# tangent-T/FACL

Measured on AMD Instinct MI355X. Metric: contrastive-step clips/sec (B=32,T=24,N=2048) at 1/2/4/8 MI355X, higher is better.
Workload: dtype f32

## Files before the change

### facl_amd/_lib.py

```python
import ctypes
import os

import torch

_HERE = os.path.dirname(os.path.abspath(__file__))
_LIB = None

c_p = ctypes.c_void_p
c_i = ctypes.c_int
c_f = ctypes.c_float
c_d = ctypes.c_double
c_l = ctypes.c_longlong

SIGNATURES = {
    "facl_version": [],
    "facl_fps_f32": [c_p, c_i, c_i, c_i, c_i, c_p, c_p, c_p],
    "facl_fps_f64": [c_p, c_i, c_i, c_i, c_i, c_p, c_p, c_p],
    "facl_fps_reorder": [c_p, c_i, c_i, c_i, c_p, c_i, c_p, c_p],
    "facl_group": [c_p, c_i, c_i, c_i, c_i, c_i, c_f, c_p, c_p, c_p, c_p],
    "facl_group_clips": [c_p, c_i, c_i, c_i, c_i, c_i, c_i, c_f, c_p, c_p, c_p, c_p],
    "facl_gather_rows": [c_p, c_i, c_i, c_i, c_i, c_p, c_i, c_p, c_p, c_i, c_i, c_p],
    "facl_scatter_rows": [c_p, c_i, c_i, c_i, c_i, c_i, c_p, c_i, c_p, c_p],
    "facl_sinkhorn": [c_p, c_i, c_i, c_i, c_p, c_p, c_p],
    "facl_kmeans": [c_p, c_i, c_i, c_i, c_i, c_p, c_p, c_p, c_p],
    "facl_adam_prep": [c_p, c_p, c_f, c_f, c_p, c_p],
    "facl_adam_apply": [c_i, c_p, c_p, c_p, c_p, c_p, c_p, c_f, c_f, c_f, c_p],
    "facl_ws_bytes": [],
    "facl_bn_finalize": [c_p, c_i, c_d, c_p, c_p, c_f, c_f, c_p, c_p, c_p, c_p, c_p, c_p],
    "facl_bn_finalize_after": [c_p, c_i, c_d, c_p, c_p, c_f, c_f, c_p, c_p, c_p, c_p, c_p, c_p, c_i, c_p],
    "facl_bn_eval_consts_after": [c_i, c_p, c_p, c_p, c_p, c_f, c_p, c_p, c_i, c_p],
    "facl_absmax": [c_p, c_l, c_p, c_p],
    "facl_rows_act_amax": [c_p, c_l, c_i, c_p, c_p, c_p, c_p],
    "facl_bn_eval_consts": [c_i, c_p, c_p, c_p, c_p, c_f, c_p, c_p],
    "facl_sa_x_moments": [c_p, c_l, c_i, c_p, c_p, c_p],
    "facl_bn1_sums_from_moments": [c_p, c_d, c_i, c_p, c_p, c_p, c_p],
    "facl_sa_bn1_chain": [c_p, c_d, c_i, c_p, c_p, c_p, c_p, c_f, c_f, c_p, c_p, c_p, c_p, c_p, c_p, c_p],
    "facl_sa_l1tab": [c_p, c_p, c_i, c_p, c_p, c_p, c_p, c_p, c_p],
    "facl_sa_fwd2": [c_p, c_l, c_i, c_p, c_p, c_p, c_p, c_p, c_p, c_p, c_p],
    "facl_sa_fwd3": [c_p, c_l, c_p, c_p, c_p, c_p, c_p, c_p, c_p, c_p, c_p, c_p],
    "facl_sa_fwd3_h3": [c_p, c_l, c_p, c_p, c_p, c_p, c_p, c_p, c_p, c_p, c_p, c_p, c_p],
    "facl_sa_fwd3_f16": [c_p, c_l, c_p, c_p, c_p, c_p, c_p, c_p, c_p, c_p, c_p, c_p],
    "facl_sa_pool": [c_p, c_l, c_i, c_p, c_p, c_p, c_p, c_p],
    "facl_sa_eval": [c_p, c_l, c_i] + [c_p] * 12,
    "facl_rows_stats": [c_p, c_l, c_i, c_p, c_p, c_p],
    "facl_rows_bn_relu": [c_p, c_l, c_i, c_p, c_p, c_p, c_p],
    "facl_rows_segmax": [c_p, c_l, c_i, c_i, c_p, c_p, c_p, c_p],
    "facl_rows_bwd_stats": [c_p, c_p, c_l, c_i, c_p, c_p, c_p, c_p],
    "facl_rows_bwd_apply": [c_p, c_p, c_l, c_i, c_p, c_p, c_p, c_p],
    "facl_rows_bwd_apply_amax": [c_p, c_p, c_l, c_i, c_p, c_p, c_p, c_p, c_p],
    "facl_segmax_bwd_stats": [c_p, c_p, c_p, c_p, c_l, c_i, c_i, c_p, c_p, c_p, c_p],
    "facl_segmax_bwd_stats_ymax": [c_p, c_p, c_p, c_l, c_i, c_p, c_p, c_p, c_p, c_i, c_p],
    "facl_segmax_bwd_apply": [c_p, c_p, c_p, c_p, c_l, c_i, c_i, c_p, c_p, c_p, c_p],
    "facl_segmax_bwd_apply_amax": [c_p, c_p, c_p, c_p, c_l, c_i, c_i, c_p, c_p, c_p, c_p, c_p],
    "facl_gemm_fwd": [c_p, c_l, c_i, c_p, c_i, c_i, c_p, c_p, c_p, c_p, c_p, c_i, c_p, c_p, c_p, c_p],
    "facl_gemm_fwd_segmax": [c_p, c_l, c_i, c_p, c_i, c_i, c_p, c_p, c_p, c_p, c_p, c_p, c_p, c_p],
    "facl_gemm_dgrad": [c_p, c_l, c_i, c_p, c_i, c_i, c_p, c_p],
    "facl_gemm_wgrad": [c_p, c_p, c_l, c_i, c_i, c_i, c_p, c_p, c_i, c_p],
    "facl_gemm_fwd_f16": [c_p, c_l, c_i, c_p, c_i, c_i, c_p, c_p, c_p, c_p, c_p, c_i, c_p, c_p, c_p, c_p],
    "facl_gemm_fwd_segmax_f16": [c_p, c_l, c_i, c_p, c_i, c_i, c_p, c_p, c_p, c_p, c_p, c_p, c_p, c_p],
    "facl_gemm_dgrad_f16": [c_p, c_l, c_i, c_p, c_i, c_i, c_p, c_p],
    "facl_gemm_wgrad_f16": [c_p, c_p, c_l, c_i, c_i, c_i, c_p, c_p, c_i, c_p],
    "facl_gemm_wgrad_pro": [c_p, c_p, c_l, c_i, c_i, c_i, c_p, c_p, c_p, c_p, c_i, c_p],
    "facl_gemm_wgrad_pro_x3": [c_p, c_p, c_l, c_i, c_i, c_i, c_p, c_p, c_p, c_p, c_i, c_p],
    "facl_gemm_wgrad_h3": [c_p, c_p, c_l, c_i, c_i, c_i, c_p, c_p, c_p, c_p, c_p, c_p, c_i, c_p],
    "facl_gemm_rs_wgrad_slices": [c_l, c_i, c_i],
    "facl_gemm_rs_wgrad": [c_p, c_p, c_l, c_i, c_i, c_p, c_p, c_p, c_p, c_p, c_p, c_p],
    "facl_gemm_rs_planes_bytes": [c_i, c_i, c_i],
    "facl_gemm_rs_planes": [c_p, c_i, c_i, c_i, c_i, c_p, c_i, c_i, c_p, c_p],
    "facl_gemm_rs_planes_multi": [c_i, c_p, c_p, c_p, c_p, c_p, c_p, c_p, c_p, c_p, c_p, c_l, c_p, c_p],
    "facl_gemm_rs_supported": [c_l, c_i, c_i],
    "facl_gemm_rs_fwd": [c_p, c_l, c_i, c_p, c_i, c_p, c_i, c_p, c_p, c_p, c_p, c_p, c_p, c_p, c_p, c_p, c_p, c_p],
    "facl_gemm_rs_dgrad": [c_p, c_l, c_i, c_p, c_i, c_p, c_i, c_p, c_p],
    "facl_gemm_rs_dgrad_bnstats": [c_p, c_l, c_i, c_p, c_i, c_p, c_i, c_p, c_p, c_p, c_p, c_p, c_p],
    "facl_gemm_fwd_x3": [c_p, c_l, c_i, c_p, c_i, c_i, c_p, c_p, c_p, c_p, c_p, c_i, c_p, c_p, c_p, c_p],
    "facl_gemm_fwd_segmax_x3": [c_p, c_l, c_i, c_p, c_i, c_i, c_p, c_p, c_p, c_p, c_p, c_p, c_p, c_p],
    "facl_gemm_dgrad_x3": [c_p, c_l, c_i, c_p, c_i, c_i, c_p, c_p],
    "facl_gemm_wgrad_x3": [c_p, c_p, c_l, c_i, c_i, c_i, c_p, c_p, c_i, c_p],
    "facl_sa_fwd3_x3": [c_p, c_l, c_p, c_p, c_p, c_p, c_p, c_p, c_p, c_p, c_p, c_p],
    "facl_contrast": [c_p, c_i, c_i, c_i, c_i, c_i, c_i, c_i, c_p, c_i, c_p, c_p, c_p, c_p],
    "facl_contrast_pair": [c_p, c_i, c_i, c_i, c_i, c_p, c_i, c_p, c_p, c_p, c_p],
    "facl_normalize_map": [c_p, c_l, c_i, c_p, c_i, c_p, c_p, c_p],
    "facl_scale_rows2": [c_p, c_p, c_l, c_l, c_i, c_p, c_p, c_p],
    "facl_build_views_f32": [c_p, c_l, c_i, c_p, c_p, c_p, c_i, c_p, c_p],
    "facl_build_views_f64": [c_p, c_l, c_i, c_p, c_p, c_p, c_i, c_p, c_p],
    "facl_views_temporal_rows_f32": [c_p, c_l, c_i, c_p, c_i, c_p, c_p, c_p, c_p],
    "facl_views_temporal_rows_f64": [c_p, c_l, c_i, c_p, c_i, c_p, c_p, c_p, c_p],
    "facl_build_views_philox_f32": [c_p, c_l, c_i, c_p, c_p, c_p, c_l, c_i, c_i, c_p, c_p, c_p],
    "facl_build_views_philox_f64": [c_p, c_l, c_i, c_p, c_p, c_p, c_l, c_i, c_i, c_p, c_p, c_p],
    "facl_build_views_philox_gp_f32": [c_p, c_l, c_i, c_p, c_p, c_p, c_l, c_i, c_i, c_i, c_i, c_p, c_p, c_p],
    "facl_build_views_philox_gp_f64": [c_p, c_l, c_i, c_p, c_p, c_p, c_l, c_i, c_i, c_i, c_i, c_p, c_p, c_p],
    "facl_resident_temporal_rows_f32": [c_p, c_p, c_p, c_i, c_i, c_p, c_p],
    "facl_resident_temporal_rows_f64": [c_p, c_p, c_p, c_i, c_i, c_p, c_p],
    "facl_build_views_resident_f32": [c_p, c_p, c_p, c_i, c_p, c_i, c_l, c_i, c_p, c_p, c_p, c_p],
    "facl_build_views_resident_f64": [c_p, c_p, c_p, c_i, c_p, c_i, c_l, c_i, c_p, c_p, c_p, c_p],
    "facl_build_views_resident_gp_f32": [c_p, c_p, c_p, c_i, c_p, c_i, c_i, c_i, c_l, c_i, c_p, c_p, c_p, c_p],
    "facl_build_views_resident_gp_f64": [c_p, c_p, c_p, c_i, c_p, c_i, c_i, c_i, c_l, c_i, c_p, c_p, c_p, c_p],
    "facl_build_views_philox_recipe_f32": [c_p, c_l, c_i, c_p, c_p, c_p, c_l, c_i, c_i, c_i, c_i, c_p, c_p, c_p, c_i, c_p, c_p],
    "facl_build_views_philox_recipe_f64": [c_p, c_l, c_i, c_p, c_p, c_p, c_l, c_i, c_i, c_i, c_i, c_p, c_p, c_p, c_i, c_p, c_p],
    "facl_build_views_resident_recipe_f32": [c_p, c_p, c_p, c_i, c_p, c_i, c_i, c_i, c_l, c_i, c_p, c_p, c_p, c_p, c_i, c_p, c_p],
    "facl_build_views_resident_recipe_f64": [c_p, c_p, c_p, c_i, c_p, c_i, c_i, c_i, c_l, c_i, c_p, c_p, c_p, c_p, c_i, c_p, c_p],
    "facl_view_recipe_table": [c_p, c_i, c_p, c_p],
    "facl_sa_bwd0": [c_p, c_p, c_l, c_p, c_p, c_p, c_p, c_p],
    "facl_sa_bwd1": [c_p, c_l, c_p, c_p, c_p, c_p, c_p, c_p, c_p, c_p, c_p, c_p, c_p],
    "facl_sa_bwd_w3": [c_p, c_l, c_p, c_p, c_p, c_p, c_p, c_p, c_p],
    "facl_sa_bwd2": [c_p, c_p, c_p, c_l, c_i, c_p, c_p, c_p, c_p, c_p, c_p, c_p],
    "facl_sa_bwd_consts3": [c_p, c_p, c_p, c_p, c_d, c_p, c_p, c_p],
    "facl_sa_bwd_consts2": [c_p, c_p, c_d, c_p, c_p],
    "facl_bn_bwd_consts": [c_p, c_p, c_i, c_d, c_p, c_p, c_p, c_p],
    "facl_rows_center_wgrad": [c_p, c_p, c_l, c_i, c_p, c_p, c_p],
    "facl_viewmax_fwd": [c_p, c_i, c_i, c_i, c_p, c_p, c_p],
    "facl_viewmax_bwd": [c_p, c_p, c_i, c_i, c_i, c_p, c_p],
    "facl_viewmax_bwd_add": [c_p, c_p, c_i, c_i, c_i, c_p, c_p],
    "facl_sa_bwd_final": [c_p] * 13 + [c_i, c_d] + [c_p] * 9 + [c_p],
    "facl_bn_bwd_consts_frozen": [c_p, c_p, c_i, c_p, c_p, c_p, c_p, c_p],
    "facl_sa_bwd_consts3_frozen": [c_p, c_p, c_p],
    "facl_sa_bwd_consts2_frozen": [c_p, c_p, c_p],
    "facl_sa_bwd_final_frozen": [c_p] * 9 + [c_i] + [c_p] * 12 + [c_p],
    "facl_viewmax_stack": [c_p, c_i, c_i, c_i, c_p, c_p, c_p],
    "facl_fc_bn_stats": [c_p, c_l, c_l, c_i, c_p, c_p, c_p],
    "facl_fc_bn_apply": [c_p, c_l, c_l, c_i, c_p, c_p, c_i, c_i, c_d, c_d, c_p, c_p, c_f, c_f, c_p, c_p, c_p, c_p, c_p],
    "facl_fc_bn_bwd_stats": [c_p, c_p, c_l, c_l, c_i, c_p, c_p, c_p, c_p],
    "facl_fc_bn_bwd_apply": [c_p, c_p, c_l, c_l, c_i, c_p, c_p, c_p, c_d, c_d, c_p, c_p, c_p, c_p, c_p],
    "facl_col_sums": [c_p, c_l, c_i, c_p, c_p],
    "facl_contrast_pair_sum": [c_p, c_i, c_i, c_i, c_i, c_p, c_i, c_p, c_p, c_p, c_p, c_p],
    "facl_gemm_wgrad_acc": [c_p, c_p, c_l, c_i, c_i, c_i, c_p, c_i, c_p],
    "facl_contrast_pair_sum_mask": [c_p, c_i, c_i, c_i, c_i, c_p, c_i, c_i, c_p, c_p, c_p, c_p, c_p],
    "facl_loss_rows_fwd": [c_p, c_l, c_i, c_i, c_f, c_p, c_p, c_p],
    "facl_loss_rows_bwd": [c_p, c_p, c_p, c_l, c_i, c_i, c_f, c_p, c_p],
    "facl_contrast_pair_queue": [c_p, c_p, c_i, c_i, c_i, c_i, c_i, c_p, c_i, c_i, c_p, c_p, c_p, c_p, c_p, c_p, c_p],
    "facl_queue_push": [c_p, c_i, c_i, c_p, c_i, c_p, c_p],
    "facl_ema_apply": [c_i, c_p, c_p, c_p, c_f, c_p],
    "facl_grad_sqnorm": [c_i, c_p, c_p, c_p, c_p],
    "facl_adam_prep_ex": [c_p, c_p, c_f, c_f, c_p, c_i, c_d, c_i, c_i, c_i, c_d, c_p, c_p],
    "facl_adamw_apply": [c_i, c_p, c_p, c_p, c_p, c_p, c_p, c_p, c_f, c_f, c_f, c_f, c_p],
    "facl_mailbox_bytes": [c_i, c_i],
    "facl_mailbox_alloc": [c_l, c_p, c_p],
    "facl_mailbox_open": [c_p, c_p],
    "facl_mailbox_close": [c_p],
    "facl_mailbox_free": [c_p],
    "facl_mailbox_allreduce": [c_p, c_p, c_i, c_i, c_p, c_i, c_i, c_p, c_p, c_p],
    "facl_gen3dv_frames": [c_p, c_i, c_i, c_i, c_p, c_p, c_p, c_p],
    "facl_gen3dv_voxelise": [c_p, c_i, c_i, c_i, c_p, c_p, c_p, c_p, c_i, c_i, c_i, c_l, c_l, c_d, c_p, c_p, c_p, c_p, c_p],
    "facl_gen3dv_volumes": [c_p, c_p, c_p, c_p, c_i, c_i, c_l, c_p, c_p, c_p],
    "facl_gen3dv_filter": [c_p, c_p, c_p, c_i, c_i, c_l, c_i, c_i, c_p, c_p, c_p],
    "facl_gen3dv_compact": [c_p, c_p, c_p, c_p, c_i, c_i, c_l, c_p, c_p, c_p],
    "facl_gen3dv_sample": [c_p, c_p, c_p, c_p, c_p, c_i, c_i, c_l, c_p, c_l, c_i, c_p, c_p, c_p, c_p, c_p, c_p],
    "facl_gen3dv_app": [c_p, c_i, c_i, c_i, c_p, c_p, c_p, c_l, c_p, c_i, c_p, c_l, c_i, c_p, c_p, c_p, c_i, c_i, c_l, c_d,
                        c_p, c_p, c_p, c_p, c_p],
    "facl_knn_ws_bytes": [c_i, c_i, c_i],
    "facl_knn_topk": [c_p, c_i, c_i, c_p, c_i, c_i, c_i, c_i, c_p, c_p, c_p, c_p, c_p],
    "facl_knn_vote": [c_p, c_p, c_p, c_i, c_i, c_i, c_i, c_f, c_p, c_p, c_p],
    "facl_cls_gather_norm_fwd": [c_p, c_i, c_i, c_i, c_p, c_p, c_p],
    "facl_cls_gather_norm_bwd": [c_p, c_p, c_p, c_i, c_i, c_i, c_p, c_p],
    "facl_softmax_ce": [c_p, c_i, c_p, c_i, c_i, c_p, c_p, c_p, c_p, c_p],
    "facl_cls_probs_acc": [c_p, c_i, c_i, c_i, c_p, c_i, c_p],
    "facl_cls_topk": [c_p, c_i, c_i, c_i, c_i, c_p, c_p, c_p, c_p, c_p],
}
RESTYPE_I64 = {"facl_ws_bytes", "facl_gemm_rs_planes_bytes", "facl_mailbox_bytes", "facl_knn_ws_bytes"}


def lib_path():
    return os.environ.get("FACL_LIB") or os.path.join(_HERE, "libfacl_hip.so")


def load_library():
    global _LIB
    if _LIB is not None:
        return _LIB
    path = lib_path()
    if not os.path.exists(path):
        raise RuntimeError(
            f"{path} not found: facl_amd has no CPU/eager fallback. Build it with "
            "`python -m facl_amd.build` (hipcc --offload-arch=gfx950).")
    lib = ctypes.CDLL(path)
    for name, argtypes in SIGNATURES.items():
        fn = getattr(lib, name)
        fn.argtypes = argtypes
        fn.restype = ctypes.c_longlong if name in RESTYPE_I64 else ctypes.c_int
    _LIB = lib
    return lib


_ERR = {-1: "unsupported shape", -2: "NULL pointer", -3: "misaligned pointer", -4: "unsupported configuration"}


def check(rc, what):
    if rc != 0:
        msg = _ERR.get(rc, f"hipError {rc}")
        raise RuntimeError(f"{what} failed: {msg} (code {rc})")


AMAX_WORDS = 2048

VIEW_KINDS = ("raw", "mirror", "key", "key_mirror", "rot", "t4", "t7", "res30", "res10", "jitter", "scale", "tilt_neg", "tilt_pos")
VIEW_POS_MAX = 12
VIEW_NSTRENGTH = 6
VIEW_TABLE_COLS = 8

SA_D_MIN, SA_D_MAX = 3, 8


def sa_l1_cols(D):
    return 8 if D <= 4 else 12


def sa_bwd2_out(D):
    return 64 * 64 + 64 * sa_l1_cols(D)


def amax_buffers(n, device, zero=True):
    if zero:
        return torch.zeros((n, AMAX_WORDS), dtype=torch.int32, device=device)
    return empty((n, AMAX_WORDS), dtype=torch.int32, device=device)


def ptr(t):
    return None if t is None else t.data_ptr()


def stream():
    return torch.cuda.current_stream().cuda_stream


SIDE_STREAM = os.environ.get("FACL_SIDE_STREAM", "0") != "0"
_SIDE = {}


class fork:

    def __init__(self, enabled=True):
        self.on = bool(enabled) and SIDE_STREAM
        self.joined = False

    def __enter__(self):
        if self.on:
            self.main = torch.cuda.current_stream()
            key = (self.main.device.index,)
            if key not in _SIDE:
                _SIDE[key] = torch.cuda.Stream(device=self.main.device)
            self.side = _SIDE[key]
            if self.side.cuda_stream == self.main.cuda_stream:
                self.on = False
                return self
            self.side.wait_stream(self.main)
            self._ctx = torch.cuda.stream(self.side)
            self._ctx.__enter__()
        return self

    def __exit__(self, *exc):
        if self.on:
            self._ctx.__exit__(*exc)
            if exc[0] is not None:
                self.main.wait_stream(self.side)
                self.joined = True
        return False

    def join(self, *tensors):
        if self.on and not self.joined:
            self.main.wait_stream(self.side)
            self.joined = True
            for t in tensors:
# ... 100 lines not shown
```

### facl_amd/csrc/finalize.hip

```cpp
#include "common.h"
#include <stdlib.h>

extern "C" int64_t facl_ws_bytes(void);

namespace {

template <typename T>
__global__ __launch_bounds__(1024) void k_reduce_rows_t1(const T* __restrict__ part, int rows, int V,
                                                         int rows_per_block, double* __restrict__ out) {
    __shared__ double red[16][64];
    const int col = threadIdx.x & 63, rg = threadIdx.x >> 6;
    const int v = blockIdx.x * 64 + col;
    const int r0 = blockIdx.y * rows_per_block;
    const int r1 = r0 + rows_per_block < rows ? r0 + rows_per_block : rows;
    double s0 = 0, s1 = 0;
    if (v < V) {
        int r = r0 + rg;
        for (; r + 16 < r1; r += 32) {
            s0 += (double)part[(size_t)r * V + v];
            s1 += (double)part[(size_t)(r + 16) * V + v];
        }
        if (r < r1) s0 += (double)part[(size_t)r * V + v];
    }
    red[rg][col] = s0 + s1;
// ... 380 lines not shown
    if (!mom || !W1 || !b1 || !sums) return FACL_E_NULL;
    if (D < FACL_SA_D_MIN || D > FACL_SA_D_MAX) return FACL_E_SHAPE;
    hipLaunchKernelGGL(k_bn1_sums_from_moments, dim3(1), dim3(64), 0, (hipStream_t)stream, mom, count, D, W1, b1, 64,
                       sums);
    return facl_launch_status();
}

extern "C" int facl_sa_bn1_chain(const double* mom, double count, int D, const float* W1, const float* b1, const float* gamma,
                                 const float* beta, float eps, float momentum, float* running_mean, float* running_var,
                                 double* sums, float* bnc, uint32_t* aamax, float* l1tab, void* stream) {
    if (!mom || !W1 || !b1 || !gamma || !beta || !sums || !bnc || !l1tab) return FACL_E_NULL;
    if (D < FACL_SA_D_MIN || D > FACL_SA_D_MAX || count < 1) return FACL_E_SHAPE;
    hipLaunchKernelGGL(k_sa_bn1_chain, dim3(1), dim3(64), 0, (hipStream_t)stream, mom, count, D, W1, b1, gamma, beta, eps, momentum,
                       running_mean, running_var, sums, bnc, aamax, l1tab);
    return facl_launch_status();
}

extern "C" int facl_sa_l1tab(const float* W1, const float* b1, int D, const float* scale, const float* shift,
                             float* l1tab, const uint32_t* xamax, uint32_t* a1amax, void* stream) {
    if (!W1 || !b1 || !l1tab || ((xamax == nullptr) != (a1amax == nullptr))) return FACL_E_NULL;
    if (D < FACL_SA_D_MIN || D > FACL_SA_D_MAX) return FACL_E_SHAPE;
    hipLaunchKernelGGL(k_l1tab, dim3(1), dim3(64), 0, (hipStream_t)stream, W1, b1, D, scale, shift, l1tab, xamax, a1amax);
    return facl_launch_status();
}

namespace {

__global__ __launch_bounds__(256) void k_sa_bwd_consts3(const double* __restrict__ sums0, const float* __restrict__ bnc3,
                                                        const float* __restrict__ W3, const float* __restrict__ b3,
                                                        double P, float* __restrict__ G3, float* __restrict__ h3) {
    __shared__ double g[256], hc[256];
    __shared__ double red[3][64];
    const int c = threadIdx.x;
    {
        const double mean = bnc3[c], inv = bnc3[256 + c], sc = bnc3[512 + c];
        const double gg = -(sc * sums0[2 * c + 1] * inv) / P;
        g[c] = gg;
        hc[c] = -(sc * sums0[2 * c]) / P + gg * ((double)b3[c] - mean);
    }
    __syncthreads();
    const int j = threadIdx.x & 63, qt = threadIdx.x >> 6;
    const int k = blockIdx.x;
    double s = 0;
    if (k < 64) {
#pragma unroll 8
        for (int cc = 64 * qt; cc < 64 * qt + 64; ++cc) s += g[cc] * (double)W3[cc * 64 + k] * (double)W3[cc * 64 + j];
    } else {
#pragma unroll 8
        for (int cc = 64 * qt; cc < 64 * qt + 64; ++cc) s += hc[cc] * (double)W3[cc * 64 + j];
    }
    if (qt) red[qt - 1][j] = s;
    __syncthreads();
    if (qt == 0) {
        s += red[0][j]; s += red[1][j]; s += red[2][j];
        if (k < 64) G3[k * 64 + j] = (float)s;
        else h3[j] = (float)s;
    }
}

__global__ void k_sa_bwd_consts2(const double* __restrict__ sums1, const float* __restrict__ bnc2, double P,
                                 float* __restrict__ bw2) {
    const int c = threadIdx.x;
    if (c >= 64) return;
    const double inv = bnc2[64 + c], sc = bnc2[128 + c];
    bw2[c] = (float)sc;
    bw2[64 + c] = (float)(-sc * sums1[2 * c] / P);
    bw2[128 + c] = (float)(-sc * inv * sums1[2 * c + 1] / P);
    bw2[192 + c] = bnc2[c];
}

__global__ __launch_bounds__(256) void k_sa_bwd_final(
    const double* __restrict__ out3, const double* __restrict__ sums0_g, const double* __restrict__ sums0_l,
    const float* __restrict__ bnc3, const float* __restrict__ W3, const float* __restrict__ b3,
    const double* __restrict__ out2, const double* __restrict__ sums1_l, const double* __restrict__ R1_g,
    const double* __restrict__ mom_l, const float* __restrict__ bnc1, const float* __restrict__ W1,
    const float* __restrict__ b1, int D, double P, float* __restrict__ dW3, float* __restrict__ dg3,
    float* __restrict__ dbe3, float* __restrict__ dW2, float* __restrict__ dg2, float* __restrict__ dbe2,
    float* __restrict__ dW1, float* __restrict__ dg1, float* __restrict__ dbe1) {
    const int o = blockIdx.x * 256 + threadIdx.x;
    const double* sparse3 = out3;
    const double* gram2 = out3 + 256 * 64;
    const double* s2 = out3 + 256 * 64 + 64 * 64;
    if (o < 16384) {
        const int c = o >> 6, k = o & 63;
        const double mean = bnc3[c], inv = bnc3[256 + c], sc = bnc3[512 + c];
        double wg = 0;
        for (int j = 0; j < 64; ++j) wg += (double)W3[c * 64 + j] * gram2[j * 64 + k];
        const double yhat_a2 = inv * (wg + ((double)b3[c] - mean) * s2[k]);
        dW3[o] = (float)(sparse3[o] - (sc / P) * (sums0_g[2 * c] * s2[k] + sums0_g[2 * c + 1] * yhat_a2));
        return;
    }
    int r = o - 16384;
    if (r < 256) { dbe3[r] = (float)sums0_l[2 * r]; dg3[r] = (float)sums0_l[2 * r + 1]; return; }
    r -= 256;
    if (r < 4096) { dW2[r] = (float)out2[r]; return; }
    r -= 4096;
    if (r < 64) { dbe2[r] = (float)sums1_l[2 * r]; dg2[r] = (float)sums1_l[2 * r + 1]; return; }
    r -= 64;
    if (r < 64) {
        const int c = r;
        const double* R1_l = out2 + 4096;
        const double mean = bnc1[c], inv = bnc1[64 + c], sc = bnc1[128 + c];
        const double bmm = (double)b1[c] - mean;
        double wr_l = 0, wr_g = 0;
        for (int d = 0; d < D; ++d) {
            wr_l += (double)W1[c * D + d] * R1_l[d * 64 + c];
            wr_g += (double)W1[c * D + d] * R1_g[d * 64 + c];
        }
        const double dbe_l = R1_l[D * 64 + c], dbe_g = R1_g[D * 64 + c];
        const double dg_l = inv * (wr_l + bmm * dbe_l), dg_g = inv * (wr_g + bmm * dbe_g);
        dbe1[c] = (float)dbe_l;
        dg1[c] = (float)dg_l;
        const double* sx = mom_l;
        const double* X2 = mom_l + D;
        for (int d = 0; d < D; ++d) {
            double wx = 0;
            for (int j = 0; j < D; ++j) wx += (double)W1[c * D + j] * X2[j * D + d];
            const double yhat_x = inv * (wx + bmm * sx[d]);
            dW1[c * D + d] = (float)(sc * (R1_l[d * 64 + c] - (dbe_g / P) * sx[d] - (dg_g / P) * yhat_x));
        }
    }
}

}

extern "C" int facl_sa_bwd_consts3(const double* sums0, const float* bnc3, const float* W3, const float* b3, double P,
                                   float* G3, float* h3, void* stream) {
    if (!sums0 || !bnc3 || !W3 || !b3 || !G3 || !h3) return FACL_E_NULL;
    if (P < 1) return FACL_E_SHAPE;
    hipLaunchKernelGGL(k_sa_bwd_consts3, dim3(65), dim3(256), 0, (hipStream_t)stream, sums0, bnc3, W3, b3, P, G3, h3);
    return facl_launch_status();
}

__global__ void k_bn_bwd_consts(const double* __restrict__ sums_l, const double* __restrict__ sums_g, int C, double P,
                                float* __restrict__ dbeta, float* __restrict__ dgamma, float* __restrict__ kk) {
    const int c = blockIdx.x * blockDim.x + threadIdx.x;
    if (c >= C) return;
    dbeta[c] = (float)sums_l[2 * c];
    dgamma[c] = (float)sums_l[2 * c + 1];
    const float inv = (float)(1.0 / P);
    kk[c] = (float)sums_g[2 * c] * inv;
    kk[C + c] = (float)sums_g[2 * c + 1] * inv;
}

extern "C" int facl_bn_bwd_consts(const double* sums_local, const double* sums_global, int C, double P, float* dbeta,
                                  float* dgamma, float* kk, void* stream) {
    if (!sums_local || !sums_global || !dbeta || !dgamma || !kk) return FACL_E_NULL;
    if (C < 1 || P < 1) return FACL_E_SHAPE;
    hipLaunchKernelGGL(k_bn_bwd_consts, dim3((C + 255) / 256), dim3(256), 0, (hipStream_t)stream, sums_local, sums_global,
                       C, P, dbeta, dgamma, kk);
    return facl_launch_status();
}

extern "C" int facl_sa_bwd_consts2(const double* sums1, const float* bnc2, double P, float* bw2, void* stream) {
    if (!sums1 || !bnc2 || !bw2) return FACL_E_NULL;
    if (P < 1) return FACL_E_SHAPE;
    hipLaunchKernelGGL(k_sa_bwd_consts2, dim3(1), dim3(64), 0, (hipStream_t)stream, sums1, bnc2, P, bw2);
    return facl_launch_status();
}

extern "C" int facl_sa_bwd_final(const double* out3, const double* sums0_g, const double* sums0_l, const float* bnc3,
                                 const float* W3, const float* b3, const double* out2, const double* sums1_l,
                                 const double* R1_g, const double* mom_l, const float* bnc1, const float* W1,
                                 const float* b1, int D, double P, float* dW3, float* dg3, float* dbe3, float* dW2,
                                 float* dg2, float* dbe2, float* dW1, float* dg1, float* dbe1, void* stream) {
    if (!out3 || !sums0_g || !sums0_l || !bnc3 || !W3 || !b3 || !out2 || !sums1_l || !R1_g || !mom_l || !bnc1 || !W1 ||
        !b1 || !dW3 || !dg3 || !dbe3 || !dW2 || !dg2 || !dbe2 || !dW1 || !dg1 || !dbe1)
        return FACL_E_NULL;
    if (D < FACL_SA_D_MIN || D > FACL_SA_D_MAX || P < 1) return FACL_E_SHAPE;
    const int total = 16384 + 256 + 4096 + 64 + 64;
    hipLaunchKernelGGL(k_sa_bwd_final, dim3((total + 255) / 256), dim3(256), 0, (hipStream_t)stream, out3, sums0_g,
                       sums0_l, bnc3, W3, b3, out2, sums1_l, R1_g, mom_l, bnc1, W1, b1, D, P, dW3, dg3, dbe3, dW2, dg2,
                       dbe2, dW1, dg1, dbe1);
    return facl_launch_status();
}

namespace {

__global__ void k_bn_bwd_consts_frozen(const double* __restrict__ sums, const float* __restrict__ bnc, int C,
                                       float* __restrict__ dbeta, float* __restrict__ dgamma, float* __restrict__ dbias,
                                       float* __restrict__ kk) {
    const int c = blockIdx.x * blockDim.x + threadIdx.x;
    if (c >= C) return;
    dbeta[c] = (float)sums[2 * c];
    dgamma[c] = (float)sums[2 * c + 1];
    dbias[c] = (float)((double)bnc[2 * C + c] * sums[2 * c]);
    kk[c] = 0.f;
    kk[C + c] = 0.f;
}

__global__ void k_sa_bwd_consts3_frozen(float* __restrict__ G3, float* __restrict__ h3) {
    const int o = blockIdx.x * 256 + threadIdx.x;
    if (o < 4096) G3[o] = 0.f;
    else if (o < 4096 + 64) h3[o - 4096] = 0.f;
}

__global__ void k_sa_bwd_consts2_frozen(const float* __restrict__ bnc2, float* __restrict__ bw2) {
    const int c = threadIdx.x;
    if (c >= 64) return;
    bw2[c] = bnc2[128 + c];
    bw2[64 + c] = 0.f;
    bw2[128 + c] = 0.f;
    bw2[192 + c] = bnc2[c];
}

__global__ __launch_bounds__(256) void k_sa_bwd_final_frozen(
    const double* __restrict__ out3, const double* __restrict__ sums0, const float* __restrict__ bnc3,
    const double* __restrict__ out2, const double* __restrict__ sums1, const float* __restrict__ bnc2,
    const float* __restrict__ bnc1, const float* __restrict__ W1, const float* __restrict__ b1, int D,
    float* __restrict__ dW3, float* __restrict__ dg3, float* __restrict__ dbe3, float* __restrict__ db3,
    float* __restrict__ dW2, float* __restrict__ dg2, float* __restrict__ dbe2, float* __restrict__ db2,
    float* __restrict__ dW1, float* __restrict__ dg1, float* __restrict__ dbe1, float* __restrict__ db1) {
    const int o = blockIdx.x * 256 + threadIdx.x;
    if (o < 16384) { dW3[o] = (float)out3[o]; return; }
    int r = o - 16384;
    if (r < 256) {
        dbe3[r] = (float)sums0[2 * r];
        dg3[r] = (float)sums0[2 * r + 1];
        db3[r] = (float)((double)bnc3[512 + r] * sums0[2 * r]);
        return;
    }
    r -= 256;
    if (r < 4096) { dW2[r] = (float)out2[r]; return; }
    r -= 4096;
    if (r < 64) {
        dbe2[r] = (float)sums1[2 * r];
        dg2[r] = (float)sums1[2 * r + 1];
        db2[r] = (float)((double)bnc2[128 + r] * sums1[2 * r]);
        return;
    }
    r -= 64;
    if (r < 64) {
        const int c = r;
        const double* R1 = out2 + 4096;
        const double mean = bnc1[c], inv = bnc1[64 + c], sc = bnc1[128 + c];
        double wr = 0;
        for (int d = 0; d < D; ++d) wr += (double)W1[c * D + d] * R1[d * 64 + c];
        const double dbe = R1[D * 64 + c];
        dbe1[c] = (float)dbe;
        dg1[c] = (float)(inv * (wr + ((double)b1[c] - mean) * dbe));
        db1[c] = (float)(sc * dbe);
        for (int d = 0; d < D; ++d) dW1[c * D + d] = (float)(sc * R1[d * 64 + c]);
    }
}

}

extern "C" int facl_bn_bwd_consts_frozen(const double* sums, const float* bnc, int C, float* dbeta, float* dgamma,
                                         float* dbias, float* kk, void* stream) {
    if (!sums || !bnc || !dbeta || !dgamma || !dbias || !kk) return FACL_E_NULL;
    if (C < 1) return FACL_E_SHAPE;
    hipLaunchKernelGGL(k_bn_bwd_consts_frozen, dim3((C + 255) / 256), dim3(256), 0, (hipStream_t)stream, sums, bnc, C,
                       dbeta, dgamma, dbias, kk);
    return facl_launch_status();
}

extern "C" int facl_sa_bwd_consts3_frozen(float* G3, float* h3, void* stream) {
    if (!G3 || !h3) return FACL_E_NULL;
    hipLaunchKernelGGL(k_sa_bwd_consts3_frozen, dim3((4096 + 64 + 255) / 256), dim3(256), 0, (hipStream_t)stream, G3, h3);
    return facl_launch_status();
}

extern "C" int facl_sa_bwd_consts2_frozen(const float* bnc2, float* bw2, void* stream) {
    if (!bnc2 || !bw2) return FACL_E_NULL;
    hipLaunchKernelGGL(k_sa_bwd_consts2_frozen, dim3(1), dim3(64), 0, (hipStream_t)stream, bnc2, bw2);
    return facl_launch_status();
}

extern "C" int facl_sa_bwd_final_frozen(const double* out3, const double* sums0, const float* bnc3, const double* out2,
                                        const double* sums1, const float* bnc2, const float* bnc1, const float* W1,
                                        const float* b1, int D, float* dW3, float* dg3, float* dbe3, float* db3, float* dW2,
                                        float* dg2, float* dbe2, float* db2, float* dW1, float* dg1, float* dbe1, float* db1,
                                        void* stream) {
    if (!out3 || !sums0 || !bnc3 || !out2 || !sums1 || !bnc2 || !bnc1 || !W1 || !b1 || !dW3 || !dg3 || !dbe3 || !db3 ||
        !dW2 || !dg2 || !dbe2 || !db2 || !dW1 || !dg1 || !dbe1 || !db1)
        return FACL_E_NULL;
    if (D < FACL_SA_D_MIN || D > FACL_SA_D_MAX) return FACL_E_SHAPE;
    const int total = 16384 + 256 + 4096 + 64 + 64;
    hipLaunchKernelGGL(k_sa_bwd_final_frozen, dim3((total + 255) / 256), dim3(256), 0, (hipStream_t)stream, out3, sums0, bnc3,
                       out2, sums1, bnc2, bnc1, W1, b1, D, dW3, dg3, dbe3, db3, dW2, dg2, dbe2, db2, dW1, dg1, dbe1, db1);
    return facl_launch_status();
}
```

### facl_amd/csrc/gemm_rs.hip

```cpp
#include "rows_common.h"

int facl_reduce_rows(const double* part, int rows, int V, double* out, hipStream_t st);
int facl_sum_slices(const float* slices, int nz, long long n4, float* out, bool par_ok, hipStream_t st);
extern "C" int64_t facl_ws_bytes(void);

namespace {

constexpr int RS_CT = 8;
constexpr int RS_WAVES = 4;
constexpr int RS_WPP = RS_CT * 3 / RS_WAVES;
constexpr int RS_WSLOT = RS_CT * 3 * 1024;
constexpr int RS_ASLOT = 32 * 128;
constexpr int RS_LDS_W = 2 * RS_WSLOT;
constexpr int RS_LDS_A = RS_WAVES * RS_ASLOT;
constexpr int RS_KMAX = 1024;
#ifndef RS_PREP_IN_ODD
#define RS_PREP_IN_ODD 1
#endif
#ifndef RS_H3_AHEAD2
#define RS_H3_AHEAD2 0
#endif
constexpr int RS_KPRO = 512;
constexpr int RS_LDS = RS_LDS_W + RS_LDS_A + 2 * RS_KPRO * 4;

struct RsArgs {
    const float* A = nullptr; int lda = 0; int M = 0; int K = 0;
    const uint4* Wp = nullptr; int NT = 0;
    int N = 0;
    const float* bias = nullptr;
    const float* pscale = nullptr; const float* pshift = nullptr;
    const float* centers = nullptr;
    float* C = nullptr; int ldc = 0;
    double* part = nullptr;
    const float* sgn = nullptr; float* smax = nullptr; int* sarg = nullptr;
    const float* by = nullptr; const float* bbnc = nullptr;
    int h3 = 0;
    const unsigned* amax = nullptr;
    const int* wse = nullptr;
    int phase_ticks = 0;
    int first_round = 0;
};



constexpr int RS_PL_ITEMS = 16;
__device__ __forceinline__ void rs_planes_tile(const float* __restrict__ W, long long so, long long sc, int NO, int NC,
                                               const float* __restrict__ xc, int ldxc, uint4* __restrict__ out, int half,
                                               int* __restrict__ hdr, int ot) {
    __shared__ float red[16];
    const int NT = NO >> 5, nks = NC >> 4, nitems = (nks + (xc ? 1 : 0)) * 64;
    float v[RS_PL_ITEMS][8];
    float m = 0.f;
#pragma unroll
    for (int t = 0; t < RS_PL_ITEMS; ++t) {
        const int item = threadIdx.x + 256 * t;
        const int ln = item & 63, ks = item >> 6;
        const int o = 32 * ot + (ln & 31), hh = ln >> 5;
        if (item < nitems) {
            if (ks < nks) {
#pragma unroll
                for (int j = 0; j < 8; ++j) v[t][j] = W[(long long)o * so + (long long)(16 * ks + 8 * hh + j) * sc];
            } else {
#pragma unroll
                for (int j = 0; j < 8; ++j) v[t][j] = (hh == 0 && j < 3) ? xc[(long long)o * ldxc + j] : 0.f;
            }
        } else {
#pragma unroll
            for (int j = 0; j < 8; ++j) v[t][j] = 0.f;
        }
    }
    float sw = 1.f;
    if (half) {
#pragma unroll
        for (int t = 0; t < RS_PL_ITEMS; ++t)
#pragma unroll
            for (int j = 0; j < 8; ++j) m = fmaxf(m, fabsf(v[t][j]));
#pragma unroll
        for (int o = 32; o > 0; o >>= 1) m = fmaxf(m, __shfl_xor(m, o, 64));
        if ((threadIdx.x & 63) == 0) red[threadIdx.x >> 6] = m;
        __syncthreads();
        m = fmaxf(fmaxf(red[0], red[1]), fmaxf(red[2], red[3]));
        const int se = h3_se(__float_as_uint(m));
        if (threadIdx.x == 0) hdr[ot] = se;
        sw = pow2_biased(se);
    }
#pragma unroll
    for (int t = 0; t < RS_PL_ITEMS; ++t) {
        const int item = threadIdx.x + 256 * t;
        if (item >= nitems) break;
        const int ln = item & 63, ks = item >> 6;
        unsigned hi[4], mi[4], lo[4];
        if (half) {
#pragma unroll
            for (int j = 0; j < 4; ++j) split_pair_h(v[t][2 * j] * sw, v[t][2 * j + 1] * sw, hi[j], lo[j]);
            uint4* d = out + ((long long)(ks * NT + ot) * 2) * 64 + ln;
            d[0] = make_uint4(hi[0], hi[1], hi[2], hi[3]);
            d[64] = make_uint4(lo[0], lo[1], lo[2], lo[3]);
            continue;
        }
#pragma unroll
        for (int j = 0; j < 4; ++j) split_pair(v[t][2 * j], v[t][2 * j + 1], hi[j], mi[j], lo[j]);
        uint4* d = out + ((long long)(ks * NT + ot) * 3) * 64 + ln;
        d[0] = make_uint4(hi[0], hi[1], hi[2], hi[3]);
        d[64] = make_uint4(mi[0], mi[1], mi[2], mi[3]);
        d[128] = make_uint4(lo[0], lo[1], lo[2], lo[3]);
    }
}

__device__ __forceinline__ void rs_absmax_block(const float* __restrict__ x, long long n, unsigned* __restrict__ amax, int b, int nb) {
    float m = 0.f;
    for (long long i = (long long)b * 256 + threadIdx.x; i < n; i += (long long)nb * 256) m = fmaxf(m, fabsf(x[i]));
#pragma unroll
    for (int o = 32; o > 0; o >>= 1) m = fmaxf(m, __shfl_xor(m, o, 64));
    if ((threadIdx.x & 63) == 0)
        atomicMax(amax + ((b * 4 + (threadIdx.x >> 6)) & (FACL_AMAX_SLOTS - 1)) * FACL_AMAX_STRIDE, __float_as_uint(m));
}

__global__ __launch_bounds__(256) void k_rs_planes(const float* __restrict__ W, long long so, long long sc, int NO, int NC,
                                                   const float* __restrict__ xc, int ldxc, uint4* __restrict__ out, int half,
                                                   int* __restrict__ hdr) {
    rs_planes_tile(W, so, sc, NO, NC, xc, ldxc, out, half, hdr, blockIdx.x);
}

constexpr int RS_MAXJOBS = 8;
struct RsPlaneJobs {
    int n;
    const float* W[RS_MAXJOBS]; long long so[RS_MAXJOBS]; long long sc[RS_MAXJOBS]; int NO[RS_MAXJOBS]; int NC[RS_MAXJOBS];
    const float* xc[RS_MAXJOBS]; int ldxc[RS_MAXJOBS]; uint4* out[RS_MAXJOBS]; int* hdr[RS_MAXJOBS]; int first[RS_MAXJOBS + 1];
    int half[RS_MAXJOBS];
    const float* ax; long long an; unsigned* aamax; int anb;
};
__global__ __launch_bounds__(256) void k_rs_planes_multi(RsPlaneJobs jb) {
    if ((int)blockIdx.x >= jb.first[jb.n]) {
        rs_absmax_block(jb.ax, jb.an, jb.aamax, (int)blockIdx.x - jb.first[jb.n], jb.anb);
        return;
    }
    int j = 0;
#pragma unroll
    for (int t = 1; t < RS_MAXJOBS; ++t) j += (t < jb.n && (int)blockIdx.x >= jb.first[t]) ? 1 : 0;
    rs_planes_tile(jb.W[j], jb.so[j], jb.sc[j], jb.NO[j], jb.NC[j], jb.xc[j], jb.ldxc[j], jb.out[j], jb.half[j], jb.hdr[j],
                   (int)blockIdx.x - jb.first[j]);
}

struct RsTile { int x, y; };
__device__ __forceinline__ RsTile rs_tile() {
    const int nbx = gridDim.x;
    const int L = facl_xcd_tile(blockIdx.x + nbx * blockIdx.y, nbx * gridDim.y);
    RsTile t;
    t.x = L % nbx; t.y = L / nbx;
    return t;
}

__device__ __forceinline__ void rs_dma16(const void* gsrc, unsigned lds_dst) {
    unsigned keep;
    asm volatile("s_mov_b32 %0, m0\n\ts_mov_b32 m0, %2\n\ts_nop 0\n\tglobal_load_lds_dwordx4 %1, off\n\ts_mov_b32 m0, %0"
                 : "=&s"(keep) : "v"(gsrc), "s"(lds_dst) : "memory");
}
__device__ __forceinline__ unsigned lds_addr(const void* p) {
    return (unsigned)(uintptr_t)(const __attribute__((address_space(3))) char*)p;
}

template <bool PRO, bool SEG, bool BST, bool H3 = false, int WV = RS_WAVES>
__global__ __launch_bounds__(64 * WV, WV == 8 ? 1 : 2) void k_gemm_rs(RsArgs g) {
    constexpr int NPL = H3 ? 2 : 3;
    constexpr int WPP = RS_CT * NPL / WV;
    extern __shared__ __attribute__((aligned(16))) char lds[];
    if ((int)(blockIdx.x + gridDim.x * blockIdx.y) < g.first_round) facl_phase_wait(g.phase_ticks);
    const int tid = threadIdx.x, lane = tid & 63, h = lane >> 5, q = lane & 31;
    const int wave = __builtin_amdgcn_readfirstlane(tid >> 6);
    char* const wring = lds;
    char* const abuf = lds + RS_LDS_W + wave * RS_ASLOT;
    float* const tab = reinterpret_cast<float*>(lds + RS_LDS_W + WV * RS_ASLOT);
    const unsigned wring_a = __builtin_amdgcn_readfirstlane(lds_addr(wring));
    const unsigned abuf_a = __builtin_amdgcn_readfirstlane(lds_addr(abuf));
    const RsTile tile = rs_tile();
    const int cb = tile.x;
    const int row0 = (tile.y * WV + wave) * 32;
    const int nks = g.K >> 4, nst = g.K >> 5;
    const int nks_all = nks + (g.centers ? 1 : 0);
    int seA = 127;
    if (H3) seA = h3_se_wide_of(g.amax);
    const float sA = pow2_biased(seA);


    const uint4* wsrc = g.Wp + ((size_t)(RS_CT * cb) * NPL + wave * WPP) * 64 + lane;
    const size_t wstep = (size_t)g.NT * NPL * 64;
    auto issueW = [&](int j) {
        if (j < nks_all) {
            const unsigned dst = wring_a + (j & 1) * RS_WSLOT + wave * WPP * 1024;
            const uint4* src = wsrc + (size_t)j * wstep;
#pragma unroll
            for (int p = 0; p < WPP; ++p) rs_dma16(src + p * 64, dst + p * 1024);
        }
    };
    const float* asrc[4];
#pragma unroll
    for (int i = 0; i < 4; ++i) {
        const int r = 8 * i + (lane >> 3);
        int gr = row0 + r;
        gr = gr < g.M ? gr : g.M - 1;
        asrc[i] = g.A + (size_t)gr * g.lda + 4 * ((lane & 7) ^ ((r >> 1) & 7));
    }
    auto issueA = [&](int s) {
        if (s < nst) {
#pragma unroll
            for (int i = 0; i < 4; ++i) rs_dma16(asrc[i] + 32 * s, abuf_a + i * 1024);
        }
    };
    const int akey = (q >> 1) & 7;
    auto read_stage = [&](float4 (&r)[4]) {
        const char* base = abuf + q * 128;
#pragma unroll
        for (int t = 0; t < 2; ++t) {
            const int c = 4 * t + 2 * h;
            r[2 * t] = *reinterpret_cast<const float4*>(base + ((c ^ akey) << 4));
            r[2 * t + 1] = *reinterpret_cast<const float4*>(base + (((c + 1) ^ akey) << 4));
        }
    };
    auto planes_half = [&](int j, const float4& r, unsigned (&pk)[12], int half) {
        float v[4] = {r.x, r.y, r.z, r.w};
        if (PRO) {
            const float4 s4 = *reinterpret_cast<const float4*>(tab + 16 * j + 8 * h + 4 * half);
            const float4 t4 = *reinterpret_cast<const float4*>(tab + RS_KPRO + 16 * j + 8 * h + 4 * half);
            v[0] = relu_nan(fmaf(s4.x, v[0], t4.x)); v[1] = relu_nan(fmaf(s4.y, v[1], t4.y));
            v[2] = relu_nan(fmaf(s4.z, v[2], t4.z)); v[3] = relu_nan(fmaf(s4.w, v[3], t4.w));
        }
        if (H3) {
            split_pair_h(v[0] * sA, v[1] * sA, pk[2 * half], pk[4 + 2 * half]);
            split_pair_h(v[2] * sA, v[3] * sA, pk[2 * half + 1], pk[4 + 2 * half + 1]);
        } else {
            split_pair(v[0], v[1], pk[2 * half], pk[4 + 2 * half], pk[8 + 2 * half]);
            split_pair(v[2], v[3], pk[2 * half + 1], pk[4 + 2 * half + 1], pk[8 + 2 * half + 1]);
        }
    };
    auto frag = [&](const unsigned (&pk)[12], int p) { return as_bf16x8(pk[4 * p], pk[4 * p + 1], pk[4 * p + 2], pk[4 * p + 3]); };

    f32x16 acc[RS_CT];
#pragma unroll
    for (int ct = 0; ct < RS_CT; ++ct)
#pragma unroll
        for (int r = 0; r < 16; ++r) acc[ct][r] = 0.f;
    constexpr int PA[6] = FACL_SB_PA, PB[6] = FACL_SB_PB;
    constexpr int HA[3] = FACL_H3_PA, HB[3] = FACL_H3_PB;
    auto mfma_group = [&](f32x16& c, const bf16x8 (&P)[3], const bf16x8 (&b)[3]) {
        if (H3) {
#pragma unroll
            for (int t = 0; t < 3; ++t)
                c = MFMA_F16(__builtin_bit_cast(f16x8h, P[HA[t]]), __builtin_bit_cast(f16x8h, b[HB[t]]), c);
        } else {
#pragma unroll
            for (int t = 0; t < 6; ++t) c = MFMA_BF16(P[PA[t]], b[PB[t]], c);
        }
    };
    auto mfma_step = [&](int j, const unsigned (&pk)[12], auto&& mid_a, auto&& mid_b) {
        const uint4* ws = reinterpret_cast<const uint4*>(wring + (j & 1) * RS_WSLOT) + lane;
        const bf16x8 P[3] = {frag(pk, 0), frag(pk, 1), frag(pk, H3 ? 1 : 2)};
        if (H3 && RS_H3_AHEAD2) {
            bf16x8 bq[3][3];
#pragma unroll
            for (int p = 0; p < NPL; ++p) { bq[0][p] = __builtin_bit_cast(bf16x8, ws[p * 64]); bq[1][p] = __builtin_bit_cast(bf16x8, ws[(NPL + p) * 64]); }
#pragma unroll
            for (int ct = 0; ct < RS_CT; ++ct) {
                if (ct + 2 < RS_CT) {
#pragma unroll
                    for (int p = 0; p < NPL; ++p) bq[(ct + 2) % 3][p] = __builtin_bit_cast(bf16x8, ws[((ct + 2) * NPL + p) * 64]);
                }
                __builtin_amdgcn_sched_barrier(0);
                if (ct == 2) mid_a();
                if (ct == 4) mid_b();
                mfma_group(acc[ct], P, bq[ct % 3]);
                __builtin_amdgcn_sched_barrier(0);
            }
            return;
        }
        bf16x8 b0[3], b1[3];
#pragma unroll
        for (int p = 0; p < NPL; ++p) b0[p] = __builtin_bit_cast(bf16x8, ws[p * 64]);
#pragma unroll
        for (int ct = 0; ct < RS_CT; ct += 2) {
#pragma unroll
            for (int p = 0; p < NPL; ++p) b1[p] = __builtin_bit_cast(bf16x8, ws[((ct + 1) * NPL + p) * 64]);
            __builtin_amdgcn_sched_barrier(0);
            if (ct == 2) mid_a();
            if (ct == 4) mid_b();
            mfma_group(acc[ct], P, b0);
            __builtin_amdgcn_sched_barrier(0);
            if (ct + 2 < RS_CT) {
#pragma unroll
                for (int p = 0; p < NPL; ++p) b0[p] = __builtin_bit_cast(bf16x8, ws[((ct + 2) * NPL + p) * 64]);
                __builtin_amdgcn_sched_barrier(0);
            }
            mfma_group(acc[ct + 1], P, b1);
            __builtin_amdgcn_sched_barrier(0);
        }
    };
    auto nop = []() {};

    issueA(0); issueW(0);
    if (PRO) {
        for (int i = tid; i < g.K; i += 64 * WV) { tab[i] = g.pscale[i]; tab[RS_KPRO + i] = g.pshift[i]; }
    }
    unsigned P0[12], P1[12];
    float4 raw[4];
    asm volatile("s_waitcnt vmcnt(0)" ::: "memory");
    __syncthreads();
    read_stage(raw);
    planes_half(0, raw[0], P0, 0);
    planes_half(0, raw[1], P0, 1);
    issueW(1);
    for (int j = 0; j + 2 < nks; j += 2) {
        asm volatile("s_waitcnt lgkmcnt(0)" ::: "memory");
        issueA((j >> 1) + 1);
        mfma_step(j, P0, [&]() { planes_half(j + 1, raw[2], P1, 0); }, [&]() { planes_half(j + 1, raw[3], P1, 1); });
        asm volatile("s_waitcnt vmcnt(4)" ::: "memory");
        __builtin_amdgcn_s_barrier();
        issueW(j + 2);
        if (RS_PREP_IN_ODD) {
            mfma_step(j + 1, P1,
                      [&]() { asm volatile("s_waitcnt vmcnt(%0)" :: "n"(WPP) : "memory"); read_stage(raw); },
                      [&]() { planes_half(j + 2, raw[0], P0, 0); planes_half(j + 2, raw[1], P0, 1); });
            asm volatile("s_waitcnt vmcnt(0)" ::: "memory");
            __builtin_amdgcn_s_barrier();
            issueW(j + 3);
            continue;
        }
        mfma_step(j + 1, P1, nop, nop);
        asm volatile("s_waitcnt vmcnt(0)" ::: "memory");
        __builtin_amdgcn_s_barrier();
        issueW(j + 3);
        read_stage(raw);
        planes_half(j + 2, raw[0], P0, 0);
        planes_half(j + 2, raw[1], P0, 1);
    }
    {
        const int j = nks - 2;
        mfma_step(j, P0, [&]() { planes_half(j + 1, raw[2], P1, 0); }, [&]() { planes_half(j + 1, raw[3], P1, 1); });
        asm volatile("s_waitcnt vmcnt(0)" ::: "memory");
        __builtin_amdgcn_s_barrier();
        issueW(j + 2);
        mfma_step(j + 1, P1, nop, nop);
    }
    if (g.centers) {
        float c0 = 0.f, c1 = 0.f, c2 = 0.f;
        if (h == 0) {
            int gr = row0 + q;
            gr = gr < g.M ? gr : g.M - 1;
            c0 = g.centers[(size_t)gr * 3]; c1 = g.centers[(size_t)gr * 3 + 1]; c2 = g.centers[(size_t)gr * 3 + 2];
        }
        unsigned hi[2], mi[2] = {0u, 0u}, lo[2];
        if (H3) {
            split_pair_h(c0 * sA, c1 * sA, hi[0], mi[0]);
            split_pair_h(c2 * sA, 0.f, hi[1], mi[1]);
            lo[0] = lo[1] = 0u;
        } else {
            split_pair(c0, c1, hi[0], mi[0], lo[0]);
            split_pair(c2, 0.f, hi[1], mi[1], lo[1]);
        }
        const unsigned Pc[12] = {hi[0], hi[1], 0u, 0u, mi[0], mi[1], 0u, 0u, lo[0], lo[1], 0u, 0u};
        asm volatile("s_waitcnt vmcnt(0)" ::: "memory");
        __builtin_amdgcn_s_barrier();
        mfma_step(nks, Pc, nop, nop);
    }

    float* const stg = reinterpret_cast<float*>(abuf);
    char* const freeslot = WV == 8 ? lds + RS_LDS_W + WV * RS_ASLOT + 2 * RS_KPRO * 4 : wring + (((nks_all - 1) & 1) ^ 1) * RS_WSLOT;
    float* const wstat = reinterpret_cast<float*>(freeslot + wave * 6144);
    float* const wbest = wstat + 512;
    float* const ystg = wstat + 512;
    const int srow = lane >> 3, schunk = lane & 7;
    float biasv[RS_CT], sgv[RS_CT], unsv[RS_CT];
#pragma unroll
    for (int ct = 0; ct < RS_CT; ++ct) {
        const int n = 256 * cb + 32 * ct + q;
        biasv[ct] = g.bias ? g.bias[n] : 0.f;
        sgv[ct] = SEG ? sgn_of(g.sgn[n]) : 1.f;
        unsv[ct] = H3 ? h3_unscale(seA, g.wse[RS_CT * cb + ct]) : 1.f;
    }
    struct YTile { float4 y0, y1, y2, y3; float mean, inv, sc, sh; };
    auto fetch_y = [&](int ct) -> YTile {
        YTile t;
        const int n_ = 256 * cb + 32 * ct + q;
        t.mean = g.bbnc[n_]; t.inv = g.bbnc[g.N + n_]; t.sc = g.bbnc[2 * g.N + n_]; t.sh = g.bbnc[3 * g.N + n_];
        const float* base = g.by + 256 * cb + 32 * ct + 4 * schunk;
        int r0_ = row0 + srow, r1_ = row0 + 8 + srow, r2_ = row0 + 16 + srow, r3_ = row0 + 24 + srow;
        r0_ = r0_ < g.M ? r0_ : g.M - 1; r1_ = r1_ < g.M ? r1_ : g.M - 1; r2_ = r2_ < g.M ? r2_ : g.M - 1; r3_ = r3_ < g.M ? r3_ : g.M - 1;
        t.y0 = *reinterpret_cast<const float4*>(base + (size_t)r0_ * g.N);
        t.y1 = *reinterpret_cast<const float4*>(base + (size_t)r1_ * g.N);
        t.y2 = *reinterpret_cast<const float4*>(base + (size_t)r2_ * g.N);
        t.y3 = *reinterpret_cast<const float4*>(base + (size_t)r3_ * g.N);
        return t;
    };
    YTile ycur = {}, ynxt = {};
    if (BST) ycur = fetch_y(0);
#pragma unroll
    for (int ct = 0; ct < RS_CT; ++ct) {
        const float bias = biasv[ct], sg = sgv[ct], uns = unsv[ct];
        float s = 0.f, sq = 0.f, best = 0.f;
        int bp = 0;
        float bmean = 0.f, binv = 0.f, bsc = 0.f, bsh = 0.f;
        if (BST) {
            bmean = ycur.mean; binv = ycur.inv; bsc = ycur.sc; bsh = ycur.sh;
            *reinterpret_cast<float4*>(ystg + (srow) * 32 + ((schunk ^ ((srow >> 1) & 7)) << 2)) = ycur.y0;
            *reinterpret_cast<float4*>(ystg + (8 + srow) * 32 + ((schunk ^ (((8 + srow) >> 1) & 7)) << 2)) = ycur.y1;
            *reinterpret_cast<float4*>(ystg + (16 + srow) * 32 + ((schunk ^ (((16 + srow) >> 1) & 7)) << 2)) = ycur.y2;
            *reinterpret_cast<float4*>(ystg + (24 + srow) * 32 + ((schunk ^ (((24 + srow) >> 1) & 7)) << 2)) = ycur.y3;
            asm volatile("s_waitcnt lgkmcnt(0)" ::: "memory");
            if (ct + 1 < RS_CT) ynxt = fetch_y(ct + 1);
        }
        float q4[4] = {0.f, 0.f, 0.f, 0.f}, g4[4] = {0.f, 0.f, 0.f, 0.f};
#pragma unroll
        for (int r = 0; r < 16; ++r) {
            const int p = rowmap(r, h);
            const float v = H3 ? fmaf(acc[ct][r], uns, bias) : acc[ct][r] + bias;
            stg[p * 32 + (((q >> 2) ^ ((p >> 1) & 7)) << 2) + (q & 3)] = v;
            if (row0 + p < g.M) {
                if (BST) {
                    const float yy = ystg[p * 32 + (((q >> 2) ^ ((p >> 1) & 7)) << 2) + (q & 3)];
                    const float d = bn_relu_dz(bsc, yy, bsh, v);
                    q4[r >> 2] += d;
                    g4[r >> 2] = fmaf(d, bn_yhat(yy, bmean, binv), g4[r >> 2]);
                } else {
                    s += v; sq = fmaf(v, v, sq);
                }
            }
            if (SEG) {
                const float sv = sg * v;
                if (r == 0 || sv > best) { best = sv; bp = rowmap(r, 0); }
            }
        }
        asm volatile("s_waitcnt lgkmcnt(0)" ::: "memory");
#pragma unroll
        for (int t = 0; t < 4; ++t) {
            const int row = 8 * t + srow;
            const float4 v4 = *reinterpret_cast<const float4*>(stg + row * 32 + ((schunk ^ ((row >> 1) & 7)) << 2));
            if (row0 + row < g.M)
                *reinterpret_cast<float4*>(g.C + (size_t)(row0 + row) * g.ldc + 256 * cb + 32 * ct + 4 * schunk) = v4;
        }
        asm volatile("" ::: "memory");
        if (BST) { s = (q4[0] + q4[1]) + (q4[2] + q4[3]); sq = (g4[0] + g4[1]) + (g4[2] + g4[3]); }
        if (g.part) {
            const float st = s + __shfl_xor(s, 32, 64), sqt = sq + __shfl_xor(sq, 32, 64);
            if (h == 0) { wstat[2 * (32 * ct + q)] = st; wstat[2 * (32 * ct + q) + 1] = sqt; }
        }
        if (SEG) {
            bp += 4 * h;
            const float ob = __shfl_xor(best, 32, 64);
            const int op = __shfl_xor(bp, 32, 64);
            if (ob > best || (ob == best && op < bp)) { best = ob; bp = op; }
            const float stp = s + __shfl_xor(s, 32, 64);
            best += stp - stp;
            if (wave & 1) {
                if (h == 0) { wbest[2 * (32 * ct + q)] = best; wbest[2 * (32 * ct + q) + 1] = __int_as_float(bp); }
            } else {
                acc[ct][0] = best; acc[ct][1] = __int_as_float(bp);
            }
        }
        if (BST) ycur = ynxt;
    }
    if (!g.part && !SEG) return;
    __syncthreads();
    if (SEG && !(wave & 1) && h == 0) {
        const float* pb = reinterpret_cast<const float*>(freeslot + (wave + 1) * 6144) + 512;
        const int cloud = row0 >> 6;
        if (row0 < g.M) {
#pragma unroll
            for (int ct = 0; ct < RS_CT; ++ct) {
                float best = acc[ct][0];
                int bp = __float_as_int(acc[ct][1]);
                const float ob = pb[2 * (32 * ct + q)];
                if (ob > best) { best = ob; bp = 32 + __float_as_int(pb[2 * (32 * ct + q) + 1]); }
                best += ob - ob;
                const size_t o = (size_t)cloud * g.N + 256 * cb + 32 * ct + q;
                g.smax[o] = best;
                g.sarg[o] = bp;
            }
        }
    }
    if (g.part && tid < 256) {
        double s = 0.0, sq = 0.0;
#pragma unroll
        for (int w = 0; w < WV; ++w) {
            const float* ps = reinterpret_cast<const float*>(freeslot + w * 6144);
            s += (double)ps[2 * tid]; sq += (double)ps[2 * tid + 1];
        }
        double* pr = g.part + ((size_t)tile.y * g.N + 256 * cb + tid) * 2;
        pr[0] = s; pr[1] = sq;
    }
}


constexpr int WG_WAVES = 8;
struct WgArgs {
    const float* dy; const float* y; int M, N, K;
    const float* pscale; const float* pshift;
    float* slices; int rows_per_slice;
    const unsigned* amax;
    const unsigned* amax_b;
};

constexpr int WG_TP = 68;
template <bool PRO, bool H3, bool WIDE = false>
__global__ __launch_bounds__(64 * WG_WAVES) void k_wgrad_rs(WgArgs g) {
    constexpr int NPL = H3 ? 2 : 3;
    constexpr int BRING_U4 = 2 * (2 * 4 * NPL * 64);
    constexpr int WSTG_F = WIDE ? 32 * WG_TP : 32 * 32;
    extern __shared__ __attribute__((aligned(16))) char wg_lds[];
    uint4 (*bring)[2 * 4 * NPL * 64] = reinterpret_cast<uint4 (*)[2 * 4 * NPL * 64]>(wg_lds);
    float* const stg_base = reinterpret_cast<float*>(wg_lds + BRING_U4 * 16);
    const int tid = threadIdx.x, lane = tid & 63, h = lane >> 5, q = lane & 31;
    const int wave = __builtin_amdgcn_readfirstlane(tid >> 6);
    const int gx = gridDim.x, gy = gridDim.y;
    const int L = facl_xcd_tile(blockIdx.x + gx * (blockIdx.y + gy * blockIdx.z), gx * gy * gridDim.z);
    const int bx = L % gx, by = (L / gx) % gy, bz = L / (gx * gy);
    const int k0 = bx * 128, n0 = by * 512 + wave * 64;
    const int p0 = bz * g.rows_per_slice;
    const int p1 = p0 + g.rows_per_slice < g.M ? p0 + g.rows_per_slice : g.M;
    const int nst = (p1 - p0 + 31) >> 5;
    float sD = 1.f, sB = 1.f, uns = 1.f;
    if (H3) {
        const int seD = h3_se_wide_of(g.amax), seB = h3_se_of(g.amax_b);
        sD = pow2_biased(seD); sB = pow2_biased(seB); uns = h3_unscale(seD, seB);
    }

    const int ks_b = tid >> 8, kt_b = (tid >> 6) & 3, lb = tid & 63;
    const int kb = k0 + 32 * kt_b + (lb & 31), hb = lb >> 5;
    const float ps = PRO ? g.pscale[kb] : 1.f, pt = PRO ? g.pshift[kb] : 0.f;
    const float* ysrc = g.y + kb;
    const float* dsrc = g.dy + n0 + q;
    auto load_b = [&](int s, float (&r)[8]) {
#pragma unroll
        for (int e = 0; e < 8; ++e) {
            int p = p0 + 32 * s + 16 * ks_b + 8 * hb + e;
            p = p < p1 ? p : p1 - 1;
            r[e] = ysrc[(size_t)p * g.K];
        }
    };
    auto store_b = [&](int s, const float (&r)[8]) {
        float v[8];
#pragma unroll
        for (int e = 0; e < 8; ++e) v[e] = PRO ? fmaxf(fmaf(ps, r[e], pt), 0.f) : r[e];
        unsigned hi[4], mi[4], lo[4];
        uint4* d = &bring[s & 1][((ks_b * 4 + kt_b) * NPL) * 64 + lb];
        if (H3) {
#pragma unroll
            for (int e = 0; e < 4; ++e) split_pair_h(v[2 * e] * sB, v[2 * e + 1] * sB, hi[e], mi[e]);
        } else {
#pragma unroll
            for (int e = 0; e < 4; ++e) split_pair(v[2 * e], v[2 * e + 1], hi[e], mi[e], lo[e]);
            d[128] = make_uint4(lo[0], lo[1], lo[2], lo[3]);
        }
        d[0] = make_uint4(hi[0], hi[1], hi[2], hi[3]);
        d[64] = make_uint4(mi[0], mi[1], mi[2], mi[3]);
    };
    auto load_a = [&](int s, float (&r)[2][2][8]) {
#pragma unroll
        for (int ks = 0; ks < 2; ++ks)
#pragma unroll
            for (int e = 0; e < 8; ++e) {
                const int p = p0 + 32 * s + 16 * ks + 8 * h + e;
                const bool in = p < p1;
                const size_t o = (size_t)(in ? p : p1 - 1) * g.N;
#pragma unroll
                for (int nt = 0; nt < 2; ++nt) {
                    const float v = dsrc[o + 32 * nt];
                    r[ks][nt][e] = in ? v : 0.f;
                }
            }
    };

    float* const dimg = stg_base + wave * WSTG_F;
    const float* dsrc4 = g.dy + n0 + 4 * (lane & 15);
    auto load_raw = [&](int s, float4 (&r)[8]) {
#pragma unroll
        for (int i = 0; i < 8; ++i) {
            const int p = p0 + 32 * s + 4 * i + (lane >> 4);
            const bool in = p < p1;
            const float4 v = *reinterpret_cast<const float4*>(dsrc4 + (size_t)(in ? p : p1 - 1) * g.N);
            r[i] = in ? v : make_float4(0.f, 0.f, 0.f, 0.f);
        }
    };
    auto raw_to_frags = [&](const float4 (&r)[8], float (&f)[2][2][8]) {
#pragma unroll
        for (int i = 0; i < 8; ++i)
            *reinterpret_cast<float4*>(dimg + (4 * i + (lane >> 4)) * WG_TP + 4 * (lane & 15)) = r[i];
        asm volatile("s_waitcnt lgkmcnt(0)" ::: "memory");
#pragma unroll
        for (int ks = 0; ks < 2; ++ks)
#pragma unroll
            for (int e = 0; e < 8; ++e)
#pragma unroll
                for (int nt = 0; nt < 2; ++nt) f[ks][nt][e] = dimg[(16 * ks + 8 * h + e) * WG_TP + 32 * nt + q];
    };

    f32x16 acc[2][4];
#pragma unroll
    for (int a = 0; a < 2; ++a)
#pragma unroll
        for (int b = 0; b < 4; ++b)
#pragma unroll
            for (int r = 0; r < 16; ++r) acc[a][b][r] = 0.f;
    constexpr int PA[6] = FACL_SB_PA, PB[6] = FACL_SB_PB;
    constexpr int HA[3] = FACL_H3_PA, HB[3] = FACL_H3_PB;

    float rb[8], ra[2][2][8];
    float4 raw[8];
    load_b(0, rb);
    if (WIDE) { load_raw(0, raw); raw_to_frags(raw, ra); }
    else load_a(0, ra);
    store_b(0, rb);
    if (nst > 1) load_b(1, rb);
    __syncthreads();
    for (int s = 0; s < nst; ++s) {
        float ran[2][2][8];
        if (s + 1 < nst) {
            if (WIDE) load_raw(s + 1, raw);
            else load_a(s + 1, ran);
        }
        const uint4* bs = &bring[s & 1][lane];
        auto split_a = [&](int ks, bf16x8 (&af)[2][NPL]) {
#pragma unroll
            for (int nt = 0; nt < 2; ++nt) {
                unsigned hi[4], mi[4], lo[4];
                if (H3) {
#pragma unroll
                    for (int e = 0; e < 4; ++e) split_pair_h(ra[ks][nt][2 * e] * sD, ra[ks][nt][2 * e + 1] * sD, hi[e], mi[e]);
                } else {
#pragma unroll
                    for (int e = 0; e < 4; ++e) split_pair(ra[ks][nt][2 * e], ra[ks][nt][2 * e + 1], hi[e], mi[e], lo[e]);
                    af[nt][NPL - 1] = as_bf16x8(lo[0], lo[1], lo[2], lo[3]);
                }
                af[nt][0] = as_bf16x8(hi[0], hi[1], hi[2], hi[3]);
                af[nt][1] = as_bf16x8(mi[0], mi[1], mi[2], mi[3]);
            }
        };
        auto mfma_ks = [&](int ks, const bf16x8 (&af)[2][NPL]) {
#pragma unroll
            for (int kt = 0; kt < 4; ++kt) {
                bf16x8 bf[NPL];
#pragma unroll
                for (int p = 0; p < NPL; ++p) bf[p] = __builtin_bit_cast(bf16x8, bs[((ks * 4 + kt) * NPL + p) * 64]);
                if (H3) {
#pragma unroll
                    for (int t = 0; t < 3; ++t) {
                        acc[0][kt] = MFMA_F16(__builtin_bit_cast(f16x8h, af[0][HA[t]]), __builtin_bit_cast(f16x8h, bf[HB[t]]), acc[0][kt]);
                        acc[1][kt] = MFMA_F16(__builtin_bit_cast(f16x8h, af[1][HA[t]]), __builtin_bit_cast(f16x8h, bf[HB[t]]), acc[1][kt]);
                    }
                } else {
#pragma unroll
                    for (int t = 0; t < 6; ++t) {
                        acc[0][kt] = MFMA_BF16(af[0][PA[t]], bf[PB[t]], acc[0][kt]);
                        acc[1][kt] = MFMA_BF16(af[1][PA[t]], bf[PB[t]], acc[1][kt]);
                    }
                }
            }
        };
        {
            bf16x8 af0[2][NPL], af1[2][NPL];
            split_a(0, af0);
            mfma_ks(0, af0);
            split_a(1, af1);
            if (WIDE && s + 1 < nst) raw_to_frags(raw, ra);
            mfma_ks(1, af1);
        }
        if (s + 1 < nst) {
            store_b(s + 1, rb);
            if (s + 2 < nst) load_b(s + 2, rb);
            if (!WIDE) {
#pragma unroll
                for (int ks = 0; ks < 2; ++ks)
#pragma unroll
                    for (int nt = 0; nt < 2; ++nt)
#pragma unroll
                        for (int e = 0; e < 8; ++e) ra[ks][nt][e] = ran[ks][nt][e];
            }
        }
        __syncthreads();
    }

    float* const stg = stg_base + wave * WSTG_F;
    float* const out = g.slices + (size_t)bz * g.N * g.K;
    const int srow = lane >> 3, schunk = lane & 7;
#pragma unroll
    for (int nt = 0; nt < 2; ++nt)
#pragma unroll
        for (int kt = 0; kt < 4; ++kt) {
#pragma unroll
            for (int r = 0; r < 16; ++r) {
                const int p = rowmap(r, h);
                stg[p * 32 + (((q >> 2) ^ ((p >> 1) & 7)) << 2) + (q & 3)] = H3 ? acc[nt][kt][r] * uns : acc[nt][kt][r];
            }
            asm volatile("s_waitcnt lgkmcnt(0)" ::: "memory");
#pragma unroll
            for (int t = 0; t < 4; ++t) {
                const int row = 8 * t + srow;
                const float4 v4 = *reinterpret_cast<const float4*>(stg + row * 32 + ((schunk ^ ((row >> 1) & 7)) << 2));
                *reinterpret_cast<float4*>(out + (size_t)(n0 + 32 * nt + row) * g.K + k0 + 32 * kt + 4 * schunk) = v4;
            }
            asm volatile("" ::: "memory");
        }
}

template <bool PRO, bool H3, bool WIDE>
int wg_launch_k(const WgArgs& g, dim3 grid, hipStream_t st) {
    constexpr int lds = 2 * (2 * 4 * (H3 ? 2 : 3) * 64) * 16 + WG_WAVES * 32 * (WIDE ? WG_TP : 32) * 4;
    return facl_launch_dynamic_lds<k_wgrad_rs<PRO, H3, WIDE>>(grid, dim3(64 * WG_WAVES), lds, st, g);
}

constexpr int RS_LDS8 = RS_LDS_W + 8 * RS_ASLOT + 2 * RS_KPRO * 4 + 8 * 6144;

int rs_waves(int h3) {
    static const int w8 = facl_env_int("FACL_RS_W8", 0);
    return (h3 && w8) ? 8 : RS_WAVES;
}

template <bool PRO, bool SEG, bool BST, bool H3, int WV>
int rs_launch_k(const RsArgs& g, hipStream_t st) {
    const dim3 grid(g.N / 256, (g.M + 32 * WV - 1) / (32 * WV));
    return facl_launch_dynamic_lds<k_gemm_rs<PRO, SEG, BST, H3, WV>>(grid, dim3(64 * WV), WV == 8 ? RS_LDS8 : RS_LDS, st, g);
}
template <bool H3, int WV>
int rs_launch_form(const RsArgs& g, hipStream_t st) {
    if (g.by) return rs_launch_k<false, false, true, H3, WV>(g, st);
    if (g.pscale && g.smax) return rs_launch_k<true, true, false, H3, WV>(g, st);
    if (g.pscale) return rs_launch_k<true, false, false, H3, WV>(g, st);
    if (g.smax) return rs_launch_k<false, true, false, H3, WV>(g, st);
    return rs_launch_k<false, false, false, H3, WV>(g, st);
}

int rs_launch(const RsArgs& g0, hipStream_t st) {
    RsArgs g = g0;
    {
        static const int per_ks = facl_env_int("FACL_RS_PHASE", 30);
        const long long wgs = (long long)(g.N / 256) * ((g.M + 32 * rs_waves(g.h3) - 1) / (32 * rs_waves(g.h3)));
        g.first_round = 512;
        g.phase_ticks = (per_ks > 0 && wgs > g.first_round && rs_waves(g.h3) == RS_WAVES) ? per_ks * (g.K >> 4) + 500 : 0;
    }
    if (rs_waves(g.h3) == 8) return rs_launch_form<true, 8>(g, st);
    return g.h3 ? rs_launch_form<true, RS_WAVES>(g, st) : rs_launch_form<false, RS_WAVES>(g, st);
}

}

static int64_t rs_planes_only_bytes(int N, int K, int with_centers) {
    return (int64_t)(K / 16 + (with_centers ? 1 : 0)) * (N / 32) * 3 * 64 * 16;
}
extern "C" int64_t facl_gemm_rs_planes_bytes(int N, int K, int with_centers) {
    if (N < 32 || K < 16) return 0;
    return rs_planes_only_bytes(N, K, with_centers) + (((int64_t)(N / 32) * 4 + 255) / 256) * 256;
}

extern "C" int facl_gemm_rs_planes(const float* W, int ldw, int N, int K, int transposed, const float* Wc, int ldwc,
                                   int half, void* planes, void* stream) {
    if (!W || !planes) return FACL_E_NULL;
    if (N < 1 || K < 1 || ldw < K) return FACL_E_SHAPE;
    const int NO = transposed ? K : N, NC = transposed ? N : K;
    if ((NO & 31) || (NC & 15) || (transposed && Wc) || NC / 16 + (Wc ? 1 : 0) > RS_PL_ITEMS * 4) return FACL_E_SHAPE;
    const long long so = transposed ? 1 : ldw, sc = transposed ? ldw : 1;
    int* hdr = (int*)((char*)planes + rs_planes_only_bytes(NO, NC, Wc ? 1 : 0));
    hipLaunchKernelGGL(k_rs_planes, dim3(NO / 32), dim3(256), 0, (hipStream_t)stream, W, so, sc, NO, NC, Wc, ldwc, (uint4*)planes,
                       half ? 1 : 0, hdr);
    return facl_launch_status();
}

extern "C" int facl_gemm_rs_planes_multi(int n, const float* const* W, const int* ldw, const int* N, const int* K,
                                         const int* transposed, const float* const* Wc, const int* ldwc, const int* half,
                                         void* const* planes, const float* absmax_x, int64_t absmax_n, uint32_t* absmax_amax,
                                         void* stream) {
    if (!W || !ldw || !N || !K || !transposed || !Wc || !ldwc || !half || !planes) return FACL_E_NULL;
    if ((absmax_x == nullptr) != (absmax_amax == nullptr)) return FACL_E_NULL;
    if (n < 1 || n > RS_MAXJOBS || (absmax_x && absmax_n < 1)) return FACL_E_SHAPE;
    RsPlaneJobs jb;
    jb.n = n;
    jb.first[0] = 0;
    for (int j = 0; j < RS_MAXJOBS; ++j) {
        if (j >= n) { jb.W[j] = nullptr; jb.xc[j] = nullptr; jb.out[j] = nullptr; jb.hdr[j] = nullptr; jb.so[j] = jb.sc[j] = 0; jb.NO[j] = jb.NC[j] = 32; jb.ldxc[j] = 0; jb.half[j] = 0; jb.first[j + 1] = jb.first[j]; continue; }
        if (!W[j] || !planes[j]) return FACL_E_NULL;
        if (N[j] < 1 || K[j] < 1 || ldw[j] < K[j]) return FACL_E_SHAPE;
        const int NO = transposed[j] ? K[j] : N[j], NC = transposed[j] ? N[j] : K[j];
        if ((NO & 31) || (NC & 15) || (transposed[j] && Wc[j]) || NC / 16 + (Wc[j] ? 1 : 0) > RS_PL_ITEMS * 4) return FACL_E_SHAPE;
        jb.W[j] = W[j]; jb.so[j] = transposed[j] ? 1 : ldw[j]; jb.sc[j] = transposed[j] ? ldw[j] : 1;
        jb.NO[j] = NO; jb.NC[j] = NC; jb.xc[j] = Wc[j]; jb.ldxc[j] = ldwc[j]; jb.out[j] = (uint4*)planes[j];
        jb.hdr[j] = (int*)((char*)planes[j] + rs_planes_only_bytes(NO, NC, Wc[j] ? 1 : 0));
        jb.half[j] = half[j] ? 1 : 0;
        jb.first[j + 1] = jb.first[j] + NO / 32;
    }
    jb.ax = absmax_x; jb.an = absmax_n; jb.aamax = absmax_amax;
    jb.anb = absmax_x ? (int)((absmax_n + 4095) / 4096 < 16 ? (absmax_n + 4095) / 4096 : 16) : 0;
    hipLaunchKernelGGL(k_rs_planes_multi, dim3(jb.first[n] + jb.anb), dim3(256), 0, (hipStream_t)stream, jb);
    return facl_launch_status();
}

extern "C" int facl_gemm_rs_supported(int64_t M, int K, int N) {
    return (M >= 2048 && M <= 0x7fffffff && K >= 64 && K <= RS_KMAX && !(K & 31) && N >= 256 && !(N & 255)) ? 1 : 0;
}

extern "C" int facl_gemm_rs_fwd(const float* a, int64_t M, int K, const void* planes, int half, const uint32_t* amax_a, int N,
                                const float* bias, const float* pscale, const float* pshift, const float* centers, float* y,
                                double* sums, const float* sgn, float* ymax, int32_t* arg, void* ws, void* stream) {
    if (!a || !planes || !y || (sums && !ws) || (half && !amax_a)) return FACL_E_NULL;
    if (!facl_gemm_rs_supported(M, K, N)) return FACL_E_SHAPE;
    if ((pscale == nullptr) != (pshift == nullptr)) return FACL_E_NULL;
    if (pscale && K > RS_KPRO) return FACL_E_SHAPE;
    if ((sgn == nullptr) != (ymax == nullptr) || (sgn == nullptr) != (arg == nullptr)) return FACL_E_NULL;
    if (sgn && (M & 63)) return FACL_E_SHAPE;
    if (((uintptr_t)a | (uintptr_t)planes) & 15) return FACL_E_ALIGN;
    const int rpw = 32 * rs_waves(half ? 1 : 0);
    const int prow = (int)((M + rpw - 1) / rpw);
    if (sums && (size_t)prow * N * 2 * sizeof(double) > ((size_t)facl_ws_bytes() - FACL_WS_TICKET_BYTES)) return FACL_E_SHAPE;
    hipStream_t st = (hipStream_t)stream;
    const int* wse = (const int*)((const char*)planes + rs_planes_only_bytes(N, K, centers ? 1 : 0));
    RsArgs g{a, K, (int)M, K, (const uint4*)planes, N / 32, N};
    g.C = y; g.ldc = N;
    g.bias = bias; g.pscale = pscale; g.pshift = pshift; g.centers = centers;
    g.part = sums ? (double*)ws : nullptr;
    g.sgn = sgn; g.smax = ymax; g.sarg = arg;
    g.h3 = half ? 1 : 0; g.amax = amax_a; g.wse = wse;
    int rc = rs_launch(g, st);
    if (rc || !sums) return rc;
    return facl_reduce_rows((const double*)ws, prow, 2 * N, sums, st);
}

extern "C" int facl_gemm_rs_dgrad(const float* dy, int64_t M, int N, const void* planes, int half, const uint32_t* amax,
                                  int K, float* da, void* stream) {
    if (!dy || !planes || !da || (half && !amax)) return FACL_E_NULL;
    if (!facl_gemm_rs_supported(M, N, K)) return FACL_E_SHAPE;
    if (((uintptr_t)dy | (uintptr_t)planes) & 15) return FACL_E_ALIGN;
    const int* wse = (const int*)((const char*)planes + rs_planes_only_bytes(K, N, 0));
    RsArgs g{dy, N, (int)M, N, (const uint4*)planes, K / 32, K};
    g.C = da; g.ldc = K;
    g.h3 = half ? 1 : 0; g.amax = amax; g.wse = wse;
    return rs_launch(g, (hipStream_t)stream);
}

extern "C" int facl_gemm_rs_dgrad_bnstats(const float* dy, int64_t M, int N, const void* planes, int half,
                                          const uint32_t* amax, int K, float* da, const float* y, const float* bnc,
                                          double* sums, void* ws, void* stream) {
    if (!dy || !planes || !da || !y || !bnc || !sums || !ws || (half && !amax)) return FACL_E_NULL;
    if (!facl_gemm_rs_supported(M, N, K)) return FACL_E_SHAPE;
    if (((uintptr_t)dy | (uintptr_t)planes) & 15) return FACL_E_ALIGN;
    const int rpw = 32 * rs_waves(half ? 1 : 0);
    const int prow = (int)((M + rpw - 1) / rpw);
    if ((size_t)prow * K * 2 * sizeof(double) > ((size_t)facl_ws_bytes() - FACL_WS_TICKET_BYTES)) return FACL_E_SHAPE;
    hipStream_t st = (hipStream_t)stream;
    const int* wse = (const int*)((const char*)planes + rs_planes_only_bytes(K, N, 0));
    RsArgs g{dy, N, (int)M, N, (const uint4*)planes, K / 32, K};
    g.C = da; g.ldc = K;
    g.part = (double*)ws; g.by = y; g.bbnc = bnc;
    g.h3 = half ? 1 : 0; g.amax = amax; g.wse = wse;
    int rc = rs_launch(g, st);
    if (rc) return rc;
    return facl_reduce_rows((const double*)ws, prow, 2 * K, sums, st);
}

extern "C" int facl_gemm_rs_wgrad_slices(int64_t M, int N, int K) {
    if (M < 4096 || N < 512 || (N & 511) || K < 128 || (K & 127)) return 0;
    const int tiles = (N / 512) * (K / 128);
    if (tiles < 8) return 0;
    int nz = 256 / tiles;
    if (nz < 1) nz = 1;
    int rps = (int)((M + nz - 1) / nz);
    rps = (rps + 31) / 32 * 32;
    return (int)((M + rps - 1) / rps);
}
extern "C" int facl_gemm_rs_wgrad(const float* dy, const float* y, int64_t M, int N, int K, const float* pscale,
                                  const float* pshift, const uint32_t* amax, const uint32_t* amax_b, float* dW, float* slices,
                                  void* stream) {
    if (!dy || !y || !dW || !slices || (amax && !amax_b)) return FACL_E_NULL;
    if ((pscale == nullptr) != (pshift == nullptr)) return FACL_E_NULL;
    if (M > 0x7fffffff) return FACL_E_SHAPE;
    const int nz = facl_gemm_rs_wgrad_slices(M, N, K);
    if (nz < 1) return FACL_E_CONFIG;
    if (((uintptr_t)slices | (uintptr_t)dW) & 15) return FACL_E_ALIGN;
    const int tiles = (N / 512) * (K / 128);
    int nz0 = 256 / tiles;
    if (nz0 < 1) nz0 = 1;
    int rps = (int)((M + nz0 - 1) / nz0);
    rps = (rps + 31) / 32 * 32;
    hipStream_t st = (hipStream_t)stream;
    WgArgs g{dy, y, (int)M, N, K, pscale, pshift, slices, rps, amax, amax_b};
    const dim3 grid(K / 128, N / 512, nz);
    static const int wide_env = facl_env_int("FACL_WGRAD_WIDE", 1);
    const int wide = wide_env && !(((uintptr_t)dy) & 15);
    int rc;
    if (pscale && amax && wide) rc = wg_launch_k<true, true, true>(g, grid, st);
    else if (amax && wide) rc = wg_launch_k<false, true, true>(g, grid, st);
    else if (pscale && amax) rc = wg_launch_k<true, true, false>(g, grid, st);
    else if (pscale) rc = wg_launch_k<true, false, false>(g, grid, st);
    else if (amax) rc = wg_launch_k<false, true, false>(g, grid, st);
    else rc = wg_launch_k<false, false, false>(g, grid, st);
    if (rc) return rc;
    return facl_sum_slices(slices, nz, (long long)N * K / 4, dW, false, st);
}
```

### facl_amd/csrc/rows.hip

```cpp
#include "rows_common.h"
#include <algorithm>

int facl_reduce_rows(const double* part, int rows, int V, double* out, hipStream_t st);

namespace {

constexpr int ROWS_BLOCKS = 1024;


__global__ __launch_bounds__(256) void k_rows_stats(const float* __restrict__ y, int R, int C,
                                                    double* __restrict__ part) {
    const int c = blockIdx.x * 256 + threadIdx.x;
    if (c >= C) return;
    double s = 0, q = 0;
    for (int r = blockIdx.y; r < R; r += gridDim.y) {
        const float v = y[(size_t)r * C + c];
        s += (double)v;
        q += (double)v * (double)v;
    }
    part[(size_t)blockIdx.y * 2 * C + 2 * c] = s;
    part[(size_t)blockIdx.y * 2 * C + 2 * c + 1] = q;
}

__global__ void k_rows_bn_relu(const float* __restrict__ y, long long n4, int C4, const float* __restrict__ scale,
                               const float* __restrict__ shift, float* __restrict__ out) {
    const long long stride = (long long)gridDim.x * blockDim.x;
    const long long i0 = (long long)blockIdx.x * blockDim.x + threadIdx.x;
    int c4 = (int)(i0 % C4);
    const int dc = (int)(stride % C4);
    for (long long i = i0; i < n4; i += stride, c4 = c4 + dc >= C4 ? c4 + dc - C4 : c4 + dc)
        reinterpret_cast<float4*>(out)[i] = lane_map<4>(bn_relu, reinterpret_cast<const float4*>(scale)[c4],
                                                        reinterpret_cast<const float4*>(y)[i], reinterpret_cast<const float4*>(shift)[c4]);
}

__global__ __launch_bounds__(256) void k_rows_segmax(const float* __restrict__ y, int S, int C,
                                                     const float* __restrict__ bnc, float* __restrict__ out,
                                                     int* __restrict__ arg) {
    const int c = blockIdx.x * 256 + threadIdx.x;
    const int m = blockIdx.y;
    if (c >= C) return;
    const float scale = bnc[2 * C + c], shift = bnc[3 * C + c], sgn = bnc[4 * C + c];
    const float* base = y + (size_t)m * S * C + c;
    float best = sgn * base[0];
    int bi = 0;
    for (int s = 1; s < S; ++s) first_max_wins(best, bi, sgn * base[(size_t)s * C], s);
    out[(size_t)m * C + c] = bn_relu(fabsf(scale), best, shift);
    arg[(size_t)m * C + c] = bi;
}

__global__ __launch_bounds__(256) void k_rows_bwd_stats(const float* __restrict__ dout, const float* __restrict__ y,
                                                        int R, int C, const float* __restrict__ bnc,
                                                        double* __restrict__ part) {
    const int c = blockIdx.x * 256 + threadIdx.x;
    if (c >= C) return;
    double acc[2] = {};
    bn_bwd_stats_rows<1>(dout, y, C, c, bnc, blockIdx.y, R, gridDim.y, acc);
    part[(size_t)blockIdx.y * 2 * C + 2 * c] = acc[0];
    part[(size_t)blockIdx.y * 2 * C + 2 * c + 1] = acc[1];
}

__global__ __launch_bounds__(256) void k_rows_bwd_stats4(const float* __restrict__ dout, const float* __restrict__ y,
                                                         int R, int C4, const float* __restrict__ bnc,
                                                         double* __restrict__ part) {
    __shared__ double red[3][64][8];
    const int lane = threadIdx.x & 63, ph = threadIdx.x >> 6;
    const int c4 = blockIdx.x * 64 + lane;
    const int C = 4 * C4;
    double acc[8] = {0, 0, 0, 0, 0, 0, 0, 0};
    if (c4 < C4) {
        const BnLanes<4> q = bn_lanes<4>(bnc, C, c4);
        for (int r = blockIdx.y * 4 + ph; r < R; r += gridDim.y * 4) {
            const size_t o = (size_t)r * C4 + c4;
            const float4 v = reinterpret_cast<const float4*>(y)[o], g = reinterpret_cast<const float4*>(dout)[o];
            const float d0 = bn_relu_dz(q.scale.x, v.x, q.shift.x, g.x), d1 = bn_relu_dz(q.scale.y, v.y, q.shift.y, g.y);
            const float d2 = bn_relu_dz(q.scale.z, v.z, q.shift.z, g.z), d3 = bn_relu_dz(q.scale.w, v.w, q.shift.w, g.w);
            acc[0] += (double)d0; acc[1] += (double)d0 * (double)bn_yhat(v.x, q.mean.x, q.inv.x);
            acc[2] += (double)d1; acc[3] += (double)d1 * (double)bn_yhat(v.y, q.mean.y, q.inv.y);
            acc[4] += (double)d2; acc[5] += (double)d2 * (double)bn_yhat(v.z, q.mean.z, q.inv.z);
            acc[6] += (double)d3; acc[7] += (double)d3 * (double)bn_yhat(v.w, q.mean.w, q.inv.w);
        }
    }
    if (phase_sum(acc, red, lane, ph, c4 < C4)) {
        double* pr = part + (size_t)blockIdx.y * 2 * C + 8 * c4;
#pragma unroll
        for (int e = 0; e < 8; ++e) pr[e] = acc[e];
    }
}

__global__ void k_rows_bwd_apply(const float* __restrict__ dout, const float* __restrict__ y, long long n, int C,
                                 const float* __restrict__ bnc, const float* __restrict__ kk,
                                 float* __restrict__ dy) {
    const long long stride = (long long)gridDim.x * blockDim.x;
    const long long i0 = (long long)blockIdx.x * blockDim.x + threadIdx.x;
    int c = (int)(i0 % C);
    const int dc = (int)(stride % C);
    for (long long i = i0; i < n; i += stride, c = c + dc >= C ? c + dc - C : c + dc)
        dy[i] = bn_relu_bwd(dout[i], y[i], bnc[c], bnc[C + c], bnc[2 * C + c], bnc[3 * C + c], kk[c], kk[C + c]);
}

__global__ __launch_bounds__(256) void k_rows_bwd_apply4(const float* __restrict__ dout, const float* __restrict__ y,
                                                         int R, int C4, const float* __restrict__ bnc,
                                                         const float* __restrict__ kk, float* __restrict__ dy,
                                                         unsigned* __restrict__ amax) {
    const int c4 = blockIdx.x * 256 + threadIdx.x;
    if (c4 >= C4) return;
    float mx = 0.f;
    unsigned* const slot = amax ? abs_max_slot(amax) : nullptr;
    const unsigned seen = amax ? *slot : 0u;
    const BnLanes<4> q = bn_lanes<4>(bnc, 4 * C4, c4);
    const KkLanes<4> k = kk_lanes<4>(kk, 4 * C4, c4);
    for (int r = blockIdx.y; r < R; r += gridDim.y) {
        const size_t o = (size_t)r * C4 + c4;
        const float4 out = lane_map<4>(bn_relu_bwd, reinterpret_cast<const float4*>(dout)[o], reinterpret_cast<const float4*>(y)[o],
                                       q.mean, q.inv, q.scale, q.shift, k.k1, k.k2);
        reinterpret_cast<float4*>(dy)[o] = out;
        mx = abs_max4(mx, out);
    }
    if (amax) publish_abs_max(slot, seen, mx);
}

__global__ __launch_bounds__(256) void k_segmax_bwd_stats(const float* __restrict__ dxpre, const float* __restrict__ xpre,
                                                          const float* __restrict__ y, const int* __restrict__ arg,
                                                          int Mrows, int S, int C, const float* __restrict__ bnc,
                                                          double* __restrict__ part) {
    const int c = blockIdx.x * 256 + threadIdx.x;
    if (c >= C) return;
    const float mean = bnc[c], inv = bnc[C + c];
    double s = 0, g = 0;
    for (int m = blockIdx.y; m < Mrows; m += gridDim.y) {
        const size_t o = (size_t)m * C + c;
        const float d = xpre[o] > 0.f ? dxpre[o] : 0.f;
        const float v = y[((size_t)m * S + arg[o]) * C + c];
        s += (double)d;
        g += (double)d * (double)bn_yhat(v, mean, inv);
    }
    part[(size_t)blockIdx.y * 2 * C + 2 * c] = s;
    part[(size_t)blockIdx.y * 2 * C + 2 * c + 1] = g;
}

__global__ __launch_bounds__(256) void k_segmax_bwd_stats_ymax(const float* __restrict__ dxpre, const float* __restrict__ xpre,
                                                               const float* __restrict__ ymax, int Mrows, int C,
                                                               const float* __restrict__ bnc, double* __restrict__ part,
                                                               unsigned* __restrict__ zamax, int zwords) {
    if (zamax && blockIdx.x == 0 && blockIdx.y == 0)
        for (int i = threadIdx.x; i < zwords; i += 256) zamax[i] = 0u;
    const int c = blockIdx.x * 256 + threadIdx.x;
    if (c >= C) return;
    const float mean = bnc[c], inv = bnc[C + c], sg = bnc[4 * C + c];
    double s = 0, g = 0;
    for (int m = blockIdx.y; m < Mrows; m += gridDim.y) {
        const size_t o = (size_t)m * C + c;
        const float d = xpre[o] > 0.f ? dxpre[o] : 0.f;
        s += (double)d;
        g += (double)d * (double)bn_yhat(sg * ymax[o], mean, inv);
    }
    part[(size_t)blockIdx.y * 2 * C + 2 * c] = s;
    part[(size_t)blockIdx.y * 2 * C + 2 * c + 1] = g;
}

template <int W>
__global__ __launch_bounds__(256) void k_segmax_bwd_apply(const float* __restrict__ dxpre, const float* __restrict__ xpre,
                                                          const float* __restrict__ y, const int* __restrict__ arg,
                                                          int S, int CW, const float* __restrict__ bnc,
                                                          const float* __restrict__ kk, float* __restrict__ dy,
                                                          unsigned* __restrict__ amax) {
    using F = typename lanes<W>::F;
    const int cw = blockIdx.x * 256 + threadIdx.x;
    const int m = blockIdx.y;
    if (cw >= CW) return;
    float mx = 0.f;
    unsigned* const slot = amax ? abs_max_slot(amax) : nullptr;
    const unsigned seen = amax ? *slot : 0u;
    const BnLanes<W> q = bn_lanes<W>(bnc, W * CW, cw);
    const KkLanes<W> k = kk_lanes<W>(kk, W * CW, cw);
    const size_t o = (size_t)m * CW + cw;
    const F d = lane_map<W>([](float xp, float dx) { return xp > 0.f ? dx : 0.f; }, reinterpret_cast<const F*>(xpre)[o],
                            reinterpret_cast<const F*>(dxpre)[o]);
    const typename lanes<W>::I a = reinterpret_cast<const typename lanes<W>::I*>(arg)[o];
    const F* yb = reinterpret_cast<const F*>(y) + (size_t)m * S * CW + cw;
    F* db = reinterpret_cast<F*>(dy) + (size_t)m * S * CW + cw;
    for (int s = 0; s < S; ++s) {
        const F out = lane_map<W>([s](int a, float d, float v, float mean, float inv, float scale, float k1, float k2) {
            return bn_bwd_dy(scale, s == a ? d : 0.f, k1, bn_yhat(v, mean, inv), k2);
        }, a, d, yb[(size_t)s * CW], q.mean, q.inv, q.scale, k.k1, k.k2);
        db[(size_t)s * CW] = out;
        if constexpr (W == 4) mx = abs_max4(mx, out);
    }
    if (amax) publish_abs_max(slot, seen, mx);
}

__global__ __launch_bounds__(256) void k_rows_center_wgrad(const float* __restrict__ dy, const float* __restrict__ ctr,
                                                           int R, int C4, double* __restrict__ part) {
    __shared__ double red[3][64][12];
    const int lane = threadIdx.x & 63, ph = threadIdx.x >> 6;
    const int c4 = blockIdx.x * 64 + lane;
    double acc[12] = {};
    if (c4 < C4) {
        for (int r = blockIdx.y * 4 + ph; r < R; r += gridDim.y * 4) {
            const float x0 = ctr[(size_t)r * 3], x1 = ctr[(size_t)r * 3 + 1], x2 = ctr[(size_t)r * 3 + 2];
            lane_each<4>([&](int e, float g) {
                acc[3 * e] += (double)g * (double)x0;
                acc[3 * e + 1] += (double)g * (double)x1;
                acc[3 * e + 2] += (double)g * (double)x2;
            }, reinterpret_cast<const float4*>(dy)[(size_t)r * C4 + c4]);
        }
    }
    if (phase_sum(acc, red, lane, ph, c4 < C4)) {
        double* pr = part + (size_t)blockIdx.y * 12 * C4 + 12 * c4;
#pragma unroll
        for (int e = 0; e < 12; ++e) pr[e] = acc[e];
    }
}

__global__ __launch_bounds__(256) void k_viewmax_fwd(const float* __restrict__ x, int G, int B, int C4,
                                                     float* __restrict__ out, int* __restrict__ arg) {
    const int i = blockIdx.x * 256 + threadIdx.x;
    if (i >= B * C4) return;
    const int b = i / C4, c4 = i - b * C4;
    float4 best = reinterpret_cast<const float4*>(x)[(size_t)b * C4 + c4];
    int4 bi = make_int4(0, 0, 0, 0);
    for (int g = 1; g < G; ++g) first_max_wins(best, bi, reinterpret_cast<const float4*>(x)[((size_t)g * B + b) * C4 + c4], g);
    reinterpret_cast<float4*>(out)[i] = best;
    reinterpret_cast<int4*>(arg)[i] = bi;
}

__global__ __launch_bounds__(256) void k_viewmax_bwd(const float* __restrict__ dout, const int* __restrict__ arg, int G,
                                                     int B, int C4, float* __restrict__ dx) {
    const int i = blockIdx.x * 256 + threadIdx.x;
    if (i >= B * C4) return;
    const int b = i / C4, c4 = i - b * C4;
    const float4 d = reinterpret_cast<const float4*>(dout)[i];
    const int4 a = reinterpret_cast<const int4*>(arg)[i];
    for (int g = 0; g < G; ++g)
        reinterpret_cast<float4*>(dx)[((size_t)g * B + b) * C4 + c4] =
            make_float4(a.x == g ? d.x : 0.f, a.y == g ? d.y : 0.f, a.z == g ? d.z : 0.f, a.w == g ? d.w : 0.f);
}

__global__ __launch_bounds__(256) void k_normalize_map(const float* __restrict__ x, int C, const float* __restrict__ Wm,
                                                       int K, float* __restrict__ xn, float* __restrict__ code) {
    __shared__ __attribute__((aligned(16))) float row[4096];
    __shared__ float red[4];
    const size_t m = blockIdx.x;
    const float4* xr = reinterpret_cast<const float4*>(x + m * C);
    const int C4 = C >> 2;
    float ss = 0.f;
    for (int i = threadIdx.x; i < C4; i += 256) {
        const float4 v = xr[i];
        reinterpret_cast<float4*>(row)[i] = v;
        ss = fmaf(v.x, v.x, ss); ss = fmaf(v.y, v.y, ss); ss = fmaf(v.z, v.z, ss); ss = fmaf(v.w, v.w, ss);
    }
    ss = wave_sum_f32(ss);
    if (lane_id() == 0) red[threadIdx.x >> 6] = ss;
    __syncthreads();
    const float nrm = sqrtf((red[0] + red[1]) + (red[2] + red[3]));
    const float inv = 1.f / fmaxf(nrm, 1e-12f);
    float4* xo = reinterpret_cast<float4*>(xn + m * C);
    for (int i = threadIdx.x; i < C4; i += 256) {
        float4 v = reinterpret_cast<float4*>(row)[i];
        v.x *= inv; v.y *= inv; v.z *= inv; v.w *= inv;
        reinterpret_cast<float4*>(row)[i] = v;
        xo[i] = v;
    }
    __syncthreads();
    const int qtr = threadIdx.x & 3, q4 = C4 >> 2;
    for (int k = threadIdx.x >> 2; k < K; k += 64) {
        const float4* w = reinterpret_cast<const float4*>(Wm + (size_t)k * C) + qtr * q4;
        const float4* r = reinterpret_cast<const float4*>(row) + qtr * q4;
        float acc = 0.f;
        for (int i = 0; i < q4; ++i) {
            const float4 a = r[i], b = w[i];
            acc = fmaf(a.x, b.x, acc); acc = fmaf(a.y, b.y, acc); acc = fmaf(a.z, b.z, acc); acc = fmaf(a.w, b.w, acc);
        }
        acc += __shfl_xor(acc, 1, 64);
        acc += __shfl_xor(acc, 2, 64);
        if (qtr == 0) code[m * K + k] = acc;
    }
}

template <int KPW, int NI>
__global__ __launch_bounds__(256) void k_normalize_map4(const float* __restrict__ x, int M, const float* __restrict__ Wm,
                                                        float* __restrict__ xn, float* __restrict__ code) {
    static_assert(KPW * 4 == 64, "the butterfly leaves one total per lane");
    constexpr int K = 4 * KPW, C4 = 64 * NI, C = 4 * C4;
    __shared__ __attribute__((aligned(16))) float rows[4][C];
    const int wave = threadIdx.x >> 6, lane = threadIdx.x & 63;
    const int m0 = blockIdx.x * 4;
    const float4* w4 = reinterpret_cast<const float4*>(Wm) + (size_t)wave * C4 + lane;
    float4 b[NI][KPW];
#pragma unroll
    for (int t = 0; t < NI; ++t)
#pragma unroll
        for (int kk = 0; kk < KPW; ++kk) b[t][kk] = w4[(size_t)(4 * kk) * C4 + 64 * t];
    {
        const int m = m0 + wave;
        float4 v[NI];
        float ss = 0.f;
#pragma unroll
        for (int t = 0; t < NI; ++t) {
            const int i = lane + 64 * t;
            v[t] = make_float4(0.f, 0.f, 0.f, 0.f);
            if (m < M && i < C4) v[t] = reinterpret_cast<const float4*>(x + (size_t)m * C)[i];
            ss = fmaf(v[t].x, v[t].x, ss); ss = fmaf(v[t].y, v[t].y, ss); ss = fmaf(v[t].z, v[t].z, ss); ss = fmaf(v[t].w, v[t].w, ss);
        }
        ss = wave_sum_f32(ss);
        const float inv = 1.f / fmaxf(sqrtf(ss), 1e-12f);
#pragma unroll
        for (int t = 0; t < NI; ++t) {
            const int i = lane + 64 * t;
            if (i < C4) {
                const float4 o = make_float4(v[t].x * inv, v[t].y * inv, v[t].z * inv, v[t].w * inv);
                reinterpret_cast<float4*>(rows[wave])[i] = o;
                if (m < M) reinterpret_cast<float4*>(xn + (size_t)m * C)[i] = o;
            }
        }
    }
    __syncthreads();
    float a[64];
#pragma unroll
    for (int j = 0; j < 64; ++j) a[j] = 0.f;
#pragma unroll
    for (int t = 0; t < NI; ++t) {
        float4 r[4];
#pragma unroll
        for (int q = 0; q < 4; ++q) r[q] = reinterpret_cast<const float4*>(rows[q])[lane + 64 * t];
#pragma unroll
        for (int kk = 0; kk < KPW; ++kk)
#pragma unroll
            for (int q = 0; q < 4; ++q) {
                float u = a[4 * kk + q];
                u = fmaf(r[q].x, b[t][kk].x, u); u = fmaf(r[q].y, b[t][kk].y, u); u = fmaf(r[q].z, b[t][kk].z, u); u = fmaf(r[q].w, b[t][kk].w, u);
                a[4 * kk + q] = u;
            }
    }
#pragma unroll
    for (int o = 32; o > 0; o >>= 1) {
        const bool hi = (lane & o) != 0;
#pragma unroll
        for (int j = 0; j < o; ++j) {
            const float keep = hi ? a[j + o] : a[j], send = hi ? a[j] : a[j + o];
            a[j] = keep + __shfl_xor(send, o, 64);
        }
    }
    const int kk = lane >> 2, q = lane & 3;
    if (m0 + q < M) code[(size_t)(m0 + q) * K + wave + 4 * kk] = a[0];
}

__global__ __launch_bounds__(256) void k_viewmax_bwd_add(const float* __restrict__ dout, const int* __restrict__ arg,
                                                         int B, int C4, float* __restrict__ dx) {
    const int i = blockIdx.x * 256 + threadIdx.x;
    if (i >= B * C4) return;
    const int b = i / C4, c4 = i - b * C4;
    const float4 d = reinterpret_cast<const float4*>(dout)[i];
    const int4 a = reinterpret_cast<const int4*>(arg)[i];
    const size_t C = (size_t)C4 * 4, col = (size_t)c4 * 4;
    dx[((size_t)a.x * B + b) * C + col + 0] += d.x;
    dx[((size_t)a.y * B + b) * C + col + 1] += d.y;
    dx[((size_t)a.z * B + b) * C + col + 2] += d.z;
    dx[((size_t)a.w * B + b) * C + col + 3] += d.w;
}

dim3 rows_grid(int64_t R, int C) {
    const int gx = (C + 255) / 256;
    return dim3(gx, (int)std::max<int64_t>(1, std::min<int64_t>(ROWS_BLOCKS / gx, R)));
}
dim3 phase_grid(int64_t R, int CW) {
    const int gx = (CW + 63) / 64;
    return dim3(gx, (int)std::max<int64_t>(1, std::min<int64_t>(ROWS_BLOCKS / gx, (R + 3) / 4)));
}

template <class... KA, class... A>
int launch_partials(void (*kern)(KA...), dim3 grid, int V, double* out, void* ws, hipStream_t st, A... args) {
    hipLaunchKernelGGL(kern, grid, dim3(256), 0, st, args...);
    if (int rc = facl_launch_status()) return rc;
    return facl_reduce_rows((const double*)ws, (int)grid.y, V, out, st);
}

}

extern "C" int facl_rows_stats(const float* y, int64_t R, int C, double* sums, void* ws, void* stream) {
    if (!y || !sums || !ws) return FACL_E_NULL;
    if (R < 1 || R > 0x7fffffff || C < 1 || 2 * C > 4608) return FACL_E_SHAPE;
    return launch_partials(k_rows_stats, rows_grid(R, C), 2 * C, sums, ws, (hipStream_t)stream, y, (int)R, C, (double*)ws);
}

extern "C" int facl_rows_bn_relu(const float* y, int64_t R, int C, const float* scale, const float* shift, float* out,
                                 void* stream) {
    if (!y || !scale || !shift || !out) return FACL_E_NULL;
    if (R < 1 || C < 4 || (C & 3)) return FACL_E_SHAPE;
    const long long n4 = R * (long long)(C / 4);
    const int grid = (int)((n4 + 255) / 256 < 4096 ? (n4 + 255) / 256 : 4096);
    hipLaunchKernelGGL(k_rows_bn_relu, dim3(grid), dim3(256), 0, (hipStream_t)stream, y, n4, C / 4, scale, shift, out);
    return facl_launch_status();
}

extern "C" int facl_rows_segmax(const float* y, int64_t M, int S, int C, const float* bnc, float* out, int32_t* arg,
                                void* stream) {
    if (!y || !bnc || !out || !arg) return FACL_E_NULL;
    if (M < 1 || M > 65535 || S < 1 || C < 1) return FACL_E_SHAPE;
    hipLaunchKernelGGL(k_rows_segmax, dim3((C + 255) / 256, (int)M), dim3(256), 0, (hipStream_t)stream, y, S, C, bnc,
                       out, arg);
    return facl_launch_status();
}

extern "C" int facl_rows_bwd_stats(const float* dout, const float* y, int64_t R, int C, const float* bnc, double* sums,
                                   void* ws, void* stream) {
    if (!dout || !y || !bnc || !sums || !ws) return FACL_E_NULL;
    if (R < 1 || R > 0x7fffffff || C < 1 || 2 * C > 4608) return FACL_E_SHAPE;
    const bool quads = !(C & 3) && aligned16(dout, y, bnc);
    return launch_partials(quads ? k_rows_bwd_stats4 : k_rows_bwd_stats, quads ? phase_grid(R, C / 4) : rows_grid(R, C), 2 * C, sums, ws,
                           (hipStream_t)stream, dout, y, (int)R, quads ? C / 4 : C, bnc, (double*)ws);
}

extern "C" int facl_rows_bwd_apply(const float* dout, const float* y, int64_t R, int C, const float* bnc,
                                   const float* kk, float* dy, void* stream) {
    return facl_rows_bwd_apply_amax(dout, y, R, C, bnc, kk, dy, nullptr, stream);
}

extern "C" int facl_rows_bwd_apply_amax(const float* dout, const float* y, int64_t R, int C, const float* bnc,
                                        const float* kk, float* dy, uint32_t* amax, void* stream) {
    if (!dout || !y || !bnc || !kk || !dy) return FACL_E_NULL;
    if (R < 1 || C < 1) return FACL_E_SHAPE;
    if (!(C & 3) && R <= 0x7fffffff && aligned16(dout, y, dy, bnc, kk)) {
        const int gx = (C / 4 + 255) / 256;
        int gy = 4096 / gx;
        if (gy > R) gy = (int)R;
        hipLaunchKernelGGL(k_rows_bwd_apply4, dim3(gx, gy), dim3(256), 0, (hipStream_t)stream, dout, y, (int)R, C / 4, bnc, kk, dy, amax);
        return facl_launch_status();
    }
    if (amax) return FACL_E_ALIGN;
    const long long n = R * (long long)C;
    const int grid = (int)((n + 255) / 256 < 8192 ? (n + 255) / 256 : 8192);
    hipLaunchKernelGGL(k_rows_bwd_apply, dim3(grid), dim3(256), 0, (hipStream_t)stream, dout, y, n, C, bnc, kk, dy);
    return facl_launch_status();
}

extern "C" int facl_segmax_bwd_stats(const float* dxpre, const float* xpre, const float* y, const int32_t* arg,
                                     int64_t M, int S, int C, const float* bnc, double* sums, void* ws, void* stream) {
    if (!dxpre || !xpre || !y || !arg || !bnc || !sums || !ws) return FACL_E_NULL;
    if (M < 1 || M > 0x7fffffff || S < 1 || C < 1 || 2 * C > 4608) return FACL_E_SHAPE;
    return launch_partials(k_segmax_bwd_stats, rows_grid(M, C), 2 * C, sums, ws, (hipStream_t)stream, dxpre, xpre, y, arg, (int)M, S,
                           C, bnc, (double*)ws);
}

extern "C" int facl_segmax_bwd_stats_ymax(const float* dxpre, const float* xpre, const float* ymax, int64_t M, int C,
                                          const float* bnc, double* sums, void* ws, uint32_t* zamax, int zwords, void* stream) {
    if (!dxpre || !xpre || !ymax || !bnc || !sums || !ws) return FACL_E_NULL;
    if (M < 1 || M > 0x7fffffff || C < 1 || 2 * C > 4608 || zwords < 0) return FACL_E_SHAPE;
    return launch_partials(k_segmax_bwd_stats_ymax, rows_grid(M, C), 2 * C, sums, ws, (hipStream_t)stream, dxpre, xpre, ymax, (int)M,
                           C, bnc, (double*)ws, zamax, zwords);
}

extern "C" int facl_segmax_bwd_apply(const float* dxpre, const float* xpre, const float* y, const int32_t* arg,
                                     int64_t M, int S, int C, const float* bnc, const float* kk, float* dy,
                                     void* stream) {
    return facl_segmax_bwd_apply_amax(dxpre, xpre, y, arg, M, S, C, bnc, kk, dy, nullptr, stream);
}

extern "C" int facl_segmax_bwd_apply_amax(const float* dxpre, const float* xpre, const float* y, const int32_t* arg,
                                          int64_t M, int S, int C, const float* bnc, const float* kk, float* dy,
                                          uint32_t* amax, void* stream) {
    if (!dxpre || !xpre || !y || !arg || !bnc || !kk || !dy) return FACL_E_NULL;
    if (M < 1 || M > 65535 || S < 1 || C < 1) return FACL_E_SHAPE;
    const bool quads = !(C & 3) && aligned16(dxpre, xpre, y, arg, dy, bnc, kk);
    if (!quads && amax) return FACL_E_ALIGN;
    const int CW = quads ? C / 4 : C;
    hipLaunchKernelGGL(quads ? k_segmax_bwd_apply<4> : k_segmax_bwd_apply<1>, dim3((CW + 255) / 256, (int)M), dim3(256), 0,
                       (hipStream_t)stream, dxpre, xpre, y, arg, S, CW, bnc, kk, dy, amax);
    return facl_launch_status();
}

extern "C" int facl_rows_center_wgrad(const float* dy, const float* centers, int64_t R, int C, double* dWc, void* ws,
                                      void* stream) {
    if (!dy || !centers || !dWc || !ws) return FACL_E_NULL;
    if (R < 1 || R > 0x7fffffff || C < 4 || (C & 3) || 3 * C > 4608) return FACL_E_SHAPE;
    if (!aligned16(dy)) return FACL_E_ALIGN;
    return launch_partials(k_rows_center_wgrad, phase_grid(R, C / 4), 3 * C, dWc, ws, (hipStream_t)stream, dy, centers, (int)R, C / 4,
                           (double*)ws);
}

extern "C" int facl_viewmax_fwd(const float* x, int G, int B, int C, float* out, int32_t* arg, void* stream) {
    if (!x || !out || !arg) return FACL_E_NULL;
    if (G < 1 || B < 1 || C < 4 || (C & 3)) return FACL_E_SHAPE;
    if (!aligned16(x, out, arg)) return FACL_E_ALIGN;
    const int n = B * (C / 4);
    hipLaunchKernelGGL(k_viewmax_fwd, dim3((n + 255) / 256), dim3(256), 0, (hipStream_t)stream, x, G, B, C / 4, out, arg);
    return facl_launch_status();
}

extern "C" int facl_viewmax_bwd(const float* dout, const int32_t* arg, int G, int B, int C, float* dx, void* stream) {
    if (!dout || !arg || !dx) return FACL_E_NULL;
    if (G < 1 || B < 1 || C < 4 || (C & 3)) return FACL_E_SHAPE;
    if (!aligned16(dout, dx, arg)) return FACL_E_ALIGN;
    const int n = B * (C / 4);
    hipLaunchKernelGGL(k_viewmax_bwd, dim3((n + 255) / 256), dim3(256), 0, (hipStream_t)stream, dout, arg, G, B, C / 4, dx);
    return facl_launch_status();
}

extern "C" int facl_normalize_map(const float* x, int64_t M, int C, const float* Wm, int K, float* x_nor, float* code,
                                  void* stream) {
    if (!x || !Wm || !x_nor || !code) return FACL_E_NULL;
    if (M < 0 || M > 0x7fffffff || C < 16 || (C & 15) || C > 4096 || K < 1 || K > 256) return FACL_E_SHAPE;
    if (!aligned16(x, Wm, x_nor)) return FACL_E_ALIGN;
    if (M == 0) return 0;
    static const int four = facl_env_int("FACL_NORMMAP4", 1);
    if (four && C == 512 && K == 64)
        hipLaunchKernelGGL((k_normalize_map4<16, 2>), dim3((unsigned)((M + 3) / 4)), dim3(256), 0, (hipStream_t)stream, x, (int)M, Wm,
                           x_nor, code);
    else if (four && C == 256 && K == 64)
        hipLaunchKernelGGL((k_normalize_map4<16, 1>), dim3((unsigned)((M + 3) / 4)), dim3(256), 0, (hipStream_t)stream, x, (int)M, Wm,
                           x_nor, code);
    else
        hipLaunchKernelGGL(k_normalize_map, dim3((unsigned)M), dim3(256), 0, (hipStream_t)stream, x, C, Wm, K, x_nor, code);
    return facl_launch_status();
}

extern "C" int facl_viewmax_bwd_add(const float* dout, const int32_t* arg, int G, int B, int C, float* dx, void* stream) {
    if (!dout || !arg || !dx) return FACL_E_NULL;
    if (G < 1 || B < 1 || C < 4 || (C & 3)) return FACL_E_SHAPE;
    if (!aligned16(dout, arg)) return FACL_E_ALIGN;
    const int n = B * (C / 4);
    hipLaunchKernelGGL(k_viewmax_bwd_add, dim3((n + 255) / 256), dim3(256), 0, (hipStream_t)stream, dout, arg, B, C / 4, dx);
    return facl_launch_status();
}
```

### facl_amd/tail.py

```python
import os
import threading

import torch

from . import _lib
from .sa_mlp import BN_EPS, BN_MOMENTUM, _Workspace, _bn_eval, _bn_finalize, act_amax_eval


PRECISIONS = ("f32", "f16", "x3", "x3b")
_SUFFIX = {"f32": "", "f16": "_f16", "x3": "_x3", "x3b": ""}
_LABEL = {"f32": "", "f16": " f16", "x3": " x3", "x3b": ""}
_SCOPE = threading.local()


class precision:

    def __init__(self, p):
        if p not in PRECISIONS:
            raise ValueError("precision must be one of %s" % (PRECISIONS,))
        self.p = p

    def __enter__(self):
        stack = _SCOPE.__dict__.setdefault("stack", [])
        stack.append(self.p)
        return self

    def __exit__(self, *exc):
        _SCOPE.stack.pop()
        return False


def current_precision():
    stack = getattr(_SCOPE, "stack", None)
    return stack[-1] if stack else "f32"


def backward_precision(p):
    return "x3" if p == "x3b" else p


def _fn(lib, name, prec):
    return getattr(lib, name + _SUFFIX[prec])


def _env_on(name, default="1"):
    return os.environ.get(name, default) != "0"


def gemm_fwd(a, W, bias, want_stats=False, centers=None, Wc=None, prec=None):
    lib = _lib.load_library()
    M, K = a.shape
    N = W.shape[0]
    y = _lib.empty((M, N), dtype=torch.float32, device=a.device)
    sums = _lib.empty((N, 2), dtype=torch.float64, device=a.device) if want_stats else None
    ws = _Workspace.get(a.device)
    prec = current_precision() if prec is None else prec
    with _lib.timed("facl_gemm_fwd %dx%dx%d%s" % (M, K, N, _LABEL[prec])):
        _lib.check(_fn(lib, "facl_gemm_fwd", prec)(_lib.ptr(a), M, K, _lib.ptr(W), W.stride(0), N, _lib.ptr(bias), None, None,
                                     _lib.ptr(centers), _lib.ptr(Wc), 3 if Wc is not None else 0, _lib.ptr(y),
                                     _lib.ptr(sums), _lib.ptr(ws), _lib.stream()), "facl_gemm_fwd")
    return y, sums


def gemm_dgrad(dy, W, prec=None):
    lib = _lib.load_library()
    M, N = dy.shape
    K = W.shape[1]
    da = _lib.empty((M, K), dtype=torch.float32, device=dy.device)
    prec = current_precision() if prec is None else prec
    with _lib.timed("facl_gemm_dgrad %dx%dx%d%s" % (M, N, K, _LABEL[prec])):
        _lib.check(_fn(lib, "facl_gemm_dgrad", prec)(_lib.ptr(dy), M, N, W.data_ptr(), W.stride(0), K, _lib.ptr(da), _lib.stream()),
                   "facl_gemm_dgrad")
    return da


def _wgrad_slices(M, N, K):
    tiles = ((N + 127) // 128) * ((K + 127) // 128)
    return max(1, min((M + 255) // 256, 512 // tiles))


def _wgrad_h3(dy, a, bnc, amax, amax_b, dW, slices, nz):
    lib = _lib.load_library()
    M, N = dy.shape
    K = a.shape[1]
    ps, pt = (bnc[2], bnc[3]) if bnc is not None else (None, None)
    with _lib.timed("facl_gemm_wgrad %dx%dx%d h3" % (M, N, K)):
        rc = lib.facl_gemm_wgrad_h3(_lib.ptr(dy), _lib.ptr(a), M, N, K, a.stride(0), _lib.ptr(ps), _lib.ptr(pt), _lib.ptr(amax),
                                    _lib.ptr(amax_b), _lib.ptr(dW), _lib.ptr(slices), nz, _lib.stream())
    if rc == -4:
        return False
    _lib.check(rc, "facl_gemm_wgrad_h3")
    return True


def gemm_wgrad(dy, a, prec=None, amax=None, amax_b=None):
    lib = _lib.load_library()
    M, N = dy.shape
    K = a.shape[1]
    nz = _wgrad_slices(M, N, K)
    dW = _lib.empty((N, K), dtype=torch.float32, device=dy.device)
    slices = _lib.empty(nz * N * K, dtype=torch.float32, device=dy.device)
    prec = current_precision() if prec is None else prec
    if amax is not None and amax_b is not None and prec == "f32" and _wgrad_h3(dy, a, None, amax, amax_b, dW, slices, nz):
        return dW
    with _lib.timed("facl_gemm_wgrad %dx%dx%d%s" % (M, N, K, _LABEL[prec])):
        _lib.check(_fn(lib, "facl_gemm_wgrad", prec)(_lib.ptr(dy), _lib.ptr(a), M, N, K, a.stride(0), _lib.ptr(dW), _lib.ptr(slices), nz,
                                       _lib.stream()), "facl_gemm_wgrad")
    return dW


def _stats(y, ws):
    lib = _lib.load_library()
    R, C = y.shape
    sums = _lib.empty((C, 2), dtype=torch.float64, device=y.device)
    _lib.check(lib.facl_rows_stats(_lib.ptr(y), R, C, _lib.ptr(sums), _lib.ptr(ws), _lib.stream()), "facl_rows_stats")
    return sums


def _bn_bwd_consts(sums, C, count, reduce_fn):
    lib = _lib.load_library()
    f32 = dict(dtype=torch.float32, device=sums.device)
    dbeta, dgamma, kk = _lib.empty(C, **f32), _lib.empty(C, **f32), _lib.empty((2, C), **f32)
    sums_g = reduce_fn(sums.clone()) if reduce_fn is not None else sums
    _lib.check(lib.facl_bn_bwd_consts(_lib.ptr(sums), _lib.ptr(sums_g), C, float(count), _lib.ptr(dbeta), _lib.ptr(dgamma),
                                      _lib.ptr(kk), _lib.stream()), "facl_bn_bwd_consts")
    return dbeta, dgamma, kk


def _bn_bwd_consts_mode(sums, bnc, C, count, reduce_fn, training):
    if training:
        return _bn_bwd_consts(sums, C, count, reduce_fn) + (None,)
    lib = _lib.load_library()
    f32 = dict(dtype=torch.float32, device=sums.device)
    dbeta, dgamma, dbias, kk = _lib.empty(C, **f32), _lib.empty(C, **f32), _lib.empty(C, **f32), _lib.empty((2, C), **f32)
    _lib.check(lib.facl_bn_bwd_consts_frozen(_lib.ptr(sums), _lib.ptr(bnc), C, _lib.ptr(dbeta), _lib.ptr(dgamma), _lib.ptr(dbias),
                                             _lib.ptr(kk), _lib.stream()), "facl_bn_bwd_consts_frozen")
    return dbeta, dgamma, kk, dbias


def _bn_relu_backward(da, y, bnc, count, reduce_fn, ws, sums=None, amax=None, training=True):
    lib = _lib.load_library()
    R, C = y.shape
    if sums is None:
        sums = _lib.empty((C, 2), dtype=torch.float64, device=y.device)
        _lib.check(lib.facl_rows_bwd_stats(_lib.ptr(da), _lib.ptr(y), R, C, _lib.ptr(bnc), _lib.ptr(sums), _lib.ptr(ws),
                                           _lib.stream()), "facl_rows_bwd_stats")
    dbeta, dgamma, kk, dbias = _bn_bwd_consts_mode(sums, bnc, C, count, reduce_fn, training)
    dy = _lib.empty_like(y)
    _lib.check(lib.facl_rows_bwd_apply_amax(_lib.ptr(da), _lib.ptr(y), R, C, _lib.ptr(bnc), _lib.ptr(kk), _lib.ptr(dy),
                                            _lib.ptr(amax), _lib.stream()), "facl_rows_bwd_apply_amax")
    return dy, dgamma, dbeta, dbias


def _first_layer_wgrad(dy, h, centers, ws, prec, amax=None, amax_b=None):
    lib = _lib.load_library()
    R, C = dy.shape
    dWh = gemm_wgrad(dy, h, prec=prec, amax=amax, amax_b=amax_b)
    dWc = _lib.empty((C, 3), dtype=torch.float64, device=dy.device)
    _lib.check(lib.facl_rows_center_wgrad(_lib.ptr(dy), _lib.ptr(centers), R, C, _lib.ptr(dWc), _lib.ptr(ws), _lib.stream()),
               "facl_rows_center_wgrad")
    return torch.cat((dWc.float(), dWh), dim=1)


def _forward_bn_consts(y, bn, training, reduce_fn, ws, sums=None, aamax=None):
    R, C = y.shape
    if not training:
        bnc = _bn_eval(C, bn.weight.detach(), bn.bias.detach(), bn.running_mean, bn.running_var)
        if aamax is not None:
            act_amax_eval(y, bnc, aamax)
        return bnc, float(R)
    if sums is None:
        sums = _stats(y, ws)
    count = float(R)
    if reduce_fn is not None:
        reduce_fn(sums)
        count = count * reduce_fn.world_size
    bnc = _bn_finalize(sums, C, count, bn.weight.detach(), bn.bias.detach(), bn.running_mean, bn.running_var, aamax=aamax)
    bn.count_batch()
    return bnc, count


class _LinearBNReLU(torch.autograd.Function):

    @staticmethod
    def forward(ctx, h, W, b, gamma, beta, bn, training, reduce_fn, centers=None):
        ctx.prec = current_precision()
        lib = _lib.load_library()
        _lib.require_cuda(h)
        ws = _Workspace.get(h.device)
        h = h.contiguous()
        if centers is not None:
            Wc, Wh = W[:, :3].contiguous(), W[:, 3:].contiguous()
            centers = centers.contiguous()
        else:
            Wc, Wh = None, W.contiguous()
        y, sums = gemm_fwd(h, Wh, b, want_stats=training, centers=centers, Wc=Wc, prec=ctx.prec)
        bnc, count = _forward_bn_consts(y, bn, training, reduce_fn, ws, sums)
        ctx.centers = centers
        ctx.Wh = Wh
        R, C = y.shape
        a = _lib.empty_like(y)
        _lib.check(lib.facl_rows_bn_relu(_lib.ptr(y), R, C, _lib.ptr(bnc[2]), _lib.ptr(bnc[3]), _lib.ptr(a),
                                         _lib.stream()), "facl_rows_bn_relu")
        _lib.tap_relu("relu_t%d" % (1 if centers is not None else 2), a=a)
        ctx.save_for_backward(h, W, y, bnc)
        ctx.count, ctx.reduce_fn, ctx.training = count, reduce_fn, training
        return a

    @staticmethod
    def backward(ctx, da):
        bp = backward_precision(ctx.prec)
        h, W, y, bnc = ctx.saved_tensors
        ws = _Workspace.get(y.device)
        dy, dgamma, dbeta, db = _bn_relu_backward(da.contiguous(), y, bnc, ctx.count, ctx.reduce_fn, ws, training=ctx.training)
        dW = gemm_wgrad(dy, h, prec=bp) if ctx.centers is None else _first_layer_wgrad(dy, h, ctx.centers, ws, bp)
        dh = gemm_dgrad(dy, ctx.Wh, prec=bp) if ctx.needs_input_grad[0] else None
        return dh, dW, db, dgamma, dbeta, None, None, None, None


class _LinearBNSegmax(torch.autograd.Function):

    @staticmethod
    def forward(ctx, h, W, b, gamma, beta, bn, training, reduce_fn, S):
        ctx.prec = current_precision()
        lib = _lib.load_library()
        _lib.require_cuda(h)
        ws = _Workspace.get(h.device)
        h = h.contiguous()
        W = W.contiguous()
        R, C = h.shape[0], W.shape[0]
        M = R // S
        xpre = _lib.empty((M, C), dtype=torch.float32, device=h.device)
        arg = _lib.empty((M, C), dtype=torch.int32, device=h.device)
        fused = False
        if S == 64 and R % 64 == 0:
            sgn = gamma.detach()
            y = _lib.empty((R, C), dtype=torch.float32, device=h.device)
            sums = _lib.empty((C, 2), dtype=torch.float64, device=h.device) if training else None
            ymax = _lib.empty((M, C), dtype=torch.float32, device=h.device)
            with _lib.timed("facl_gemm_fwd %dx%dx%d%s" % (R, h.shape[1], C, _LABEL[ctx.prec])):
                rc = _fn(lib, "facl_gemm_fwd_segmax", ctx.prec)(_lib.ptr(h), R, h.shape[1], _lib.ptr(W), W.stride(0), C, _lib.ptr(b),
                                              _lib.ptr(sgn), _lib.ptr(y), _lib.ptr(sums), _lib.ptr(ymax), _lib.ptr(arg),
                                              _lib.ptr(ws), _lib.stream())
            if rc == 0:
                fused = True
                bnc, count = _forward_bn_consts(y, bn, training, reduce_fn, ws, sums)
                _lib.check(lib.facl_sa_pool(_lib.ptr(ymax), M, C, _lib.ptr(bnc[2]), _lib.ptr(bnc[3]), _lib.ptr(xpre), None,
                                            _lib.stream()), "facl_sa_pool")
            elif rc != -4:
                _lib.check(rc, "facl_gemm_fwd_segmax")
        if not fused:
            y, sums = gemm_fwd(h, W, b, want_stats=training, prec=ctx.prec)
            bnc, count = _forward_bn_consts(y, bn, training, reduce_fn, ws, sums)
            _lib.check(lib.facl_rows_segmax(_lib.ptr(y), M, S, C, _lib.ptr(bnc), _lib.ptr(xpre), _lib.ptr(arg),
                                            _lib.stream()), "facl_rows_segmax")
        _lib.tap("seg_arg", arg)
        _lib.tap_relu("relu_t3", a=xpre)
        ctx.save_for_backward(h, W, y, bnc, xpre, arg)
        ctx.count, ctx.reduce_fn, ctx.training, ctx.S = count, reduce_fn, training, S
        ctx.mark_non_differentiable(arg)
        return xpre, arg

    @staticmethod
    def backward(ctx, dxpre, _darg):
        bp = backward_precision(ctx.prec)
        lib = _lib.load_library()
        h, W, y, bnc, xpre, arg = ctx.saved_tensors
        ws = _Workspace.get(y.device)
        R, C = y.shape
        S = ctx.S
        M = R // S
        dxpre = dxpre.contiguous()
        sums = _lib.empty((C, 2), dtype=torch.float64, device=y.device)
        _lib.check(lib.facl_segmax_bwd_stats(_lib.ptr(dxpre), _lib.ptr(xpre), _lib.ptr(y), _lib.ptr(arg), M, S, C,
                                             _lib.ptr(bnc), _lib.ptr(sums), _lib.ptr(ws), _lib.stream()),
                   "facl_segmax_bwd_stats")
        dbeta, dgamma, kk, db = _bn_bwd_consts_mode(sums, bnc, C, ctx.count, ctx.reduce_fn, ctx.training)
        dy = _lib.empty_like(y)
        _lib.check(lib.facl_segmax_bwd_apply(_lib.ptr(dxpre), _lib.ptr(xpre), _lib.ptr(y), _lib.ptr(arg), M, S, C,
                                             _lib.ptr(bnc), _lib.ptr(kk), _lib.ptr(dy), _lib.stream()),
                   "facl_segmax_bwd_apply")
        dW = gemm_wgrad(dy, h, prec=bp)
        dh = gemm_dgrad(dy, W, prec=bp)
        return dh, dW, db, dgamma, dbeta, None, None, None, None


def linear_bn_relu(h, affine, bn, training, reduce_fn=None, centers=None):
    W = affine.weight.view(affine.weight.shape[0], -1)
    return _LinearBNReLU.apply(h, W, affine.bias, bn.weight, bn.bias, bn, training, reduce_fn, centers)


class _Linear(torch.autograd.Function):

    @staticmethod
    def forward(ctx, h, W, b):
        ctx.prec = current_precision()
        h, W = h.contiguous(), W.contiguous()
        y, _ = gemm_fwd(h, W, b, prec=ctx.prec)
        ctx.save_for_backward(h, W)
        return y

    @staticmethod
    def backward(ctx, dy):
        bp = backward_precision(ctx.prec)
        h, W = ctx.saved_tensors
        dy = dy.contiguous()
        return gemm_dgrad(dy, W, prec=bp), gemm_wgrad(dy, h, prec=bp), dy.sum(0)


_FC_FUSED = _env_on("FACL_FC_FUSED")


class _FCHead(torch.autograd.Function):

    @staticmethod
    def forward(ctx, x_pre, G, W1, b1, gamma, beta, bn, W2, b2, training, reduce_fn):
        ctx.prec = current_precision()
        lib = _lib.load_library()
        _lib.require_cuda(x_pre)
        ws = _Workspace.get(x_pre.device)
        x_pre = x_pre.contiguous()
        M, Cin = x_pre.shape
        B = M // G
        h = _lib.empty((M + B, Cin), dtype=torch.float32, device=x_pre.device)
        arg = _lib.empty((B, Cin), dtype=torch.int32, device=x_pre.device)
        _lib.check(lib.facl_viewmax_stack(_lib.ptr(x_pre), G, B, Cin, _lib.ptr(h), _lib.ptr(arg), _lib.stream()), "facl_viewmax_stack")
        _lib.tap("view_arg", arg)
        W1, W2 = W1.contiguous(), W2.contiguous()
        R, C = M + B, W1.shape[0]
        segs = ((0, M), (M, R))
# ... 106 lines not shown
                    part = (dbe[i], dga[i], kk[i], None)
                _lib.check(lib.facl_rows_bwd_apply(_lib.ptr(dact[r0:r1]), _lib.ptr(y[r0:r1]), r1 - r0, C, _lib.ptr(bnc),
                                                   _lib.ptr(part[2]), _lib.ptr(dy[r0:r1]), _lib.stream()), "facl_rows_bwd_apply")
                parts.append(part)
            dgamma, dbeta = parts[0][1] + parts[1][1], parts[0][0] + parts[1][0]
            if frozen:
                db1 = parts[0][3] + parts[1][3]
        with _lib.fork(enabled=side) as f1:
            dW1 = gemm_wgrad(dy, h, prec=bp)
        dh = gemm_dgrad(dy, W1, prec=bp)
        _lib.check(lib.facl_viewmax_bwd_add(dh[M:].data_ptr(), _lib.ptr(arg), ctx.G, B, dh.shape[1], _lib.ptr(dh), _lib.stream()),
                   "facl_viewmax_bwd_add")
        f2.join(dW2, db2)
        f1.join(dW1)
        return dh[:M], None, dW1, db1, dgamma, dbeta, None, dW2, db2, None, None


def fc_head(x_pre, G, affine1, bn, affine2, training, reduce_fn=None):
    return _FCHead.apply(x_pre, G, affine1.weight, affine1.bias, bn.weight, bn.bias, bn, affine2.weight, affine2.bias,
                         training, reduce_fn)


class _NormalizeMap(torch.autograd.Function):

    @staticmethod
    def forward(ctx, x, Wm, lazy=False):
        lib = _lib.load_library()
        _lib.require_cuda(x)
        x, Wm = x.contiguous(), Wm.contiguous()
        M, C = x.shape
        K = Wm.shape[0]
        xn = _lib.empty_like(x)
        code = _lib.empty((M, K), dtype=torch.float32, device=x.device)
        with _lib.fork(enabled=lazy) as f:
            _lib.check(lib.facl_normalize_map(_lib.ptr(x), M, C, _lib.ptr(Wm), K, _lib.ptr(xn), _lib.ptr(code), _lib.stream()),
                       "facl_normalize_map")
        if f.on:
            _lib._PENDING.append((f, (xn, code)))
        ctx.save_for_backward(x, xn, Wm)
        return xn, code

    @staticmethod
    def backward(ctx, dxn, dcode):
        x, xn, Wm = ctx.saved_tensors
        dxn_t = dcode @ Wm if dxn is None else dxn + dcode @ Wm
        dWm = dcode.t() @ xn
        nrm = x.norm(dim=1, keepdim=True).clamp_min(1e-12)
        dx = (dxn_t - xn * (dxn_t * xn).sum(1, keepdim=True)) / nrm
        return dx, dWm, None


def normalize_map(x, mapping_weight, lazy=False):
    return _NormalizeMap.apply(x, mapping_weight, lazy)


class _ViewMax(torch.autograd.Function):

    @staticmethod
    def forward(ctx, x_pre, G):
        lib = _lib.load_library()
        _lib.require_cuda(x_pre)
        x_pre = x_pre.contiguous()
        B, C = x_pre.shape[0] // G, x_pre.shape[1]
        out = _lib.empty((B, C), dtype=torch.float32, device=x_pre.device)
        arg = _lib.empty((B, C), dtype=torch.int32, device=x_pre.device)
        _lib.check(lib.facl_viewmax_fwd(_lib.ptr(x_pre), G, B, C, _lib.ptr(out), _lib.ptr(arg), _lib.stream()), "facl_viewmax_fwd")
        ctx.save_for_backward(arg)
        ctx.G = G
        return out

    @staticmethod
    def backward(ctx, dout):
        lib = _lib.load_library()
        arg, = ctx.saved_tensors
        B, C = arg.shape
        dout = dout.contiguous()
        dx = _lib.empty((ctx.G * B, C), dtype=torch.float32, device=dout.device)
        _lib.check(lib.facl_viewmax_bwd(_lib.ptr(dout), _lib.ptr(arg), ctx.G, B, C, _lib.ptr(dx), _lib.stream()), "facl_viewmax_bwd")
        return dx, None


def view_max(x_pre, G):
    return _ViewMax.apply(x_pre, G)


def linear(h, affine):
    return _Linear.apply(h, affine.weight, affine.bias)


def linear_bn_relu_segmax(h, affine, bn, training, S, reduce_fn=None):
    W = affine.weight.view(affine.weight.shape[0], -1)
    xpre, _ = _LinearBNSegmax.apply(h, W, affine.bias, bn.weight, bn.bias, bn, training, reduce_fn, S)
    return xpre


def rs_planes(W, transposed, centers_cols=None, half=False):
    lib = _lib.load_library()
    N, K = W.shape
    nb = lib.facl_gemm_rs_planes_bytes(K if transposed else N, N if transposed else K, 0 if centers_cols is None else 1)
    planes = _lib.empty(nb, dtype=torch.uint8, device=W.device)
    _lib.check(lib.facl_gemm_rs_planes(W.data_ptr(), W.stride(0), N, K, 1 if transposed else 0,
                                       None if centers_cols is None else centers_cols.data_ptr(),
                                       0 if centers_cols is None else centers_cols.stride(0), 1 if half else 0,
                                       _lib.ptr(planes), _lib.stream()), "facl_gemm_rs_planes")
    return planes


def rs_planes_multi(jobs, absmax=None):
    jobs = [(j + (False,))[:4] for j in jobs]
    import ctypes
    lib = _lib.load_library()
    n = len(jobs)
    outs = []
    for W, tr, xc, _h in jobs:
        N, K = W.shape
        nb = lib.facl_gemm_rs_planes_bytes(K if tr else N, N if tr else K, 0 if xc is None else 1)
        outs.append(_lib.empty(nb, dtype=torch.uint8, device=W.device))
    vp, ip = ctypes.c_void_p * n, ctypes.c_int * n
    _lib.check(lib.facl_gemm_rs_planes_multi(
        n, vp(*[j[0].data_ptr() for j in jobs]), ip(*[j[0].stride(0) for j in jobs]), ip(*[j[0].shape[0] for j in jobs]),
        ip(*[j[0].shape[1] for j in jobs]), ip(*[1 if j[1] else 0 for j in jobs]),
        vp(*[None if j[2] is None else j[2].data_ptr() for j in jobs]),
        ip(*[0 if j[2] is None else j[2].stride(0) for j in jobs]), ip(*[1 if j[3] else 0 for j in jobs]),
        vp(*[o.data_ptr() for o in outs]), None if absmax is None else _lib.ptr(absmax[0]),
        0 if absmax is None else absmax[0].numel(), None if absmax is None else _lib.ptr(absmax[1]), _lib.stream()),
        "facl_gemm_rs_planes_multi")
    return outs


FWD_H3 = _env_on("FACL_FWD_H3")
BWD_H3 = _env_on("FACL_BWD_H3")


def _rs_fwd(a, planes, N, bias, pro, centers, want_stats, seg_sgn, ws, half=False, amax_a=None):
    lib = _lib.load_library()
    M, K = a.shape
    y = _lib.empty((M, N), dtype=torch.float32, device=a.device)
    sums = _lib.empty((N, 2), dtype=torch.float64, device=a.device) if want_stats else None
    ymax = arg = None
    if seg_sgn is not None:
        ymax = _lib.empty((M // 64, N), dtype=torch.float32, device=a.device)
        arg = _lib.empty((M // 64, N), dtype=torch.int32, device=a.device)
    ps, pt = (pro[2], pro[3]) if pro is not None else (None, None)
    with _lib.timed("facl_gemm_rs_fwd %dx%dx%d%s" % (M, K, N, " h3" if half else "")):
        _lib.check(lib.facl_gemm_rs_fwd(_lib.ptr(a), M, K, _lib.ptr(planes), 1 if half else 0, _lib.ptr(amax_a), N, _lib.ptr(bias), _lib.ptr(ps), _lib.ptr(pt),
                                        _lib.ptr(centers), _lib.ptr(y), _lib.ptr(sums), _lib.ptr(seg_sgn), _lib.ptr(ymax),
                                        _lib.ptr(arg), _lib.ptr(ws), _lib.stream()), "facl_gemm_rs_fwd")
    return y, sums, ymax, arg


_FUSE_BNSTATS = _env_on("FACL_RS_BNSTATS")


def _rs_dgrad(dy, W, prec, planes=None, bn_y=None, bn_c=None, ws=None, amax=None):
    if prec != "f32":
        return gemm_dgrad(dy, W, prec=prec), None
    lib = _lib.load_library()
    M, N = dy.shape
    K = W.shape[1]
    half = 0 if amax is None else 1
    if planes is None:
        planes = rs_planes(W, True, half=bool(half))
    da = _lib.empty((M, K), dtype=torch.float32, device=dy.device)
    sums = None
    with _lib.timed("facl_gemm_rs_dgrad %dx%dx%d%s" % (M, N, K, " h3" if half else "")):
        if bn_y is not None and _FUSE_BNSTATS:
            sums = _lib.empty((K, 2), dtype=torch.float64, device=dy.device)
            _lib.check(lib.facl_gemm_rs_dgrad_bnstats(_lib.ptr(dy), M, N, _lib.ptr(planes), half, _lib.ptr(amax), K, _lib.ptr(da),
                                                      _lib.ptr(bn_y), _lib.ptr(bn_c), _lib.ptr(sums), _lib.ptr(ws), _lib.stream()),
                       "facl_gemm_rs_dgrad_bnstats")
        else:
            _lib.check(lib.facl_gemm_rs_dgrad(_lib.ptr(dy), M, N, _lib.ptr(planes), half, _lib.ptr(amax), K, _lib.ptr(da),
                                              _lib.stream()), "facl_gemm_rs_dgrad")
    return da, sums


_WGRAD_RS = _env_on("FACL_WGRAD_RS")


def _wgrad_pro(dy, y, bnc, prec, amax=None, amax_b=None):
    lib = _lib.load_library()
    M, N = dy.shape
    K = y.shape[1]
    dW = _lib.empty((N, K), dtype=torch.float32, device=dy.device)
    nzr = lib.facl_gemm_rs_wgrad_slices(M, N, K) if (prec == "f32" and _WGRAD_RS and y.is_contiguous()) else 0
    if nzr > 0:
        slices = _lib.empty(nzr * N * K, dtype=torch.float32, device=dy.device)
        with _lib.timed("facl_gemm_rs_wgrad %dx%dx%d%s" % (M, N, K, "" if amax is None else " h3")):
            _lib.check(lib.facl_gemm_rs_wgrad(_lib.ptr(dy), _lib.ptr(y), M, N, K, _lib.ptr(bnc[2]), _lib.ptr(bnc[3]),
                                              _lib.ptr(amax), _lib.ptr(amax_b), _lib.ptr(dW), _lib.ptr(slices), _lib.stream()),
                       "facl_gemm_rs_wgrad")
        return dW
    nz = _wgrad_slices(M, N, K)
    slices = _lib.empty(nz * N * K, dtype=torch.float32, device=dy.device)
    if amax is not None and prec == "f32" and _wgrad_h3(dy, y, bnc, amax, amax_b, dW, slices, nz):
        return dW
    fn = lib.facl_gemm_wgrad_pro_x3 if prec == "x3" else lib.facl_gemm_wgrad_pro
    with _lib.timed("facl_gemm_wgrad %dx%dx%d%s" % (M, N, K, _LABEL[prec])):
        rc = fn(_lib.ptr(dy), _lib.ptr(y), M, N, K, y.stride(0), _lib.ptr(bnc[2]), _lib.ptr(bnc[3]), _lib.ptr(dW),
                _lib.ptr(slices), nz, _lib.stream())
    if rc == -4:
        a = _lib.empty_like(y)
        _lib.check(lib.facl_rows_bn_relu(_lib.ptr(y), M, K, _lib.ptr(bnc[2]), _lib.ptr(bnc[3]), _lib.ptr(a), _lib.stream()),
                   "facl_rows_bn_relu")
        return gemm_wgrad(dy, a, prec=prec)
    _lib.check(rc, "facl_gemm_wgrad_pro")
    return dW


def net3dv3_supported(P, widths, S, prec):
    if not _env_on("FACL_TAIL_RS") or prec not in ("f32", "x3b") or S != 64 or P % 64:
        return False
    lib = _lib.load_library()
    c0, c1, c2, c3 = widths
    return all(lib.facl_gemm_rs_supported(P, k, n) == 1 for k, n in ((c0, c1), (c1, c2), (c2, c3))) and max(c1, c2) <= 512 \
        and all(lib.facl_gemm_rs_supported(P, n, k) == 1 for k, n in ((c0, c1), (c1, c2), (c2, c3)))


class _Net3DV3(torch.autograd.Function):

    @staticmethod
    def forward(ctx, pooled, centers, S, training, reduce_fn, bns, pooled_amax, W1, b1, g1, be1, W2, b2, g2, be2, W3, b3, g3, be3):
        ctx.prec = current_precision()
        lib = _lib.load_library()
        _lib.require_cuda(pooled)
        ws = _Workspace.get(pooled.device)
        pooled, centers = pooled.contiguous(), centers.contiguous()
        W1, W2, W3 = W1.contiguous(), W2.contiguous(), W3.contiguous()
        P = pooled.shape[0]
        h3 = FWD_H3
        jobs = [(W1[:, 3:], False, W1[:, :3], h3), (W2, False, None, h3), (W3, False, None, h3)]
        want_bwd = (training or any(ctx.needs_input_grad)) and backward_precision(ctx.prec) == "f32"
        if want_bwd:
            jobs += [(W3, True, None, BWD_H3), (W2, True, None, BWD_H3), (W1[:, 3:], True, None, BWD_H3)]
        amax = _lib.amax_buffers(3, pooled.device, zero=(not training) or pooled_amax is None)
        if pooled_amax is not None:
            a0 = pooled_amax
        else:
            a0 = amax[0]
            _lib.check(lib.facl_absmax(_lib.ptr(pooled), pooled.numel(), _lib.ptr(a0), _lib.stream()), "facl_absmax")
        pl = rs_planes_multi(jobs, absmax=(centers, a0))
        ctx.bwd_planes = pl[3:] if want_bwd else None
        ctx.bwd_h3 = want_bwd and BWD_H3
        y1, sums1, _, _ = _rs_fwd(pooled, pl[0], W1.shape[0], b1, None, centers, training, None, ws, h3, a0)
        bnc1, count = _forward_bn_consts(y1, bns[0], training, reduce_fn, ws, sums1, aamax=amax[1])
        y2, sums2, _, _ = _rs_fwd(y1, pl[1], W2.shape[0], b2, bnc1, None, training, None, ws, h3, amax[1])
        bnc2, _ = _forward_bn_consts(y2, bns[1], training, reduce_fn, ws, sums2, aamax=amax[2])
        y3, sums3, ymax, arg = _rs_fwd(y2, pl[2], W3.shape[0], b3, bnc2, None, training, g3.detach(), ws, h3, amax[2])
        ctx.act_amax = (a0, amax[1], amax[2])
        bnc3, _ = _forward_bn_consts(y3, bns[2], training, reduce_fn, ws, sums3)
        M, C = P // S, W3.shape[0]
        xpre = _lib.empty((M, C), dtype=torch.float32, device=pooled.device)
        _lib.check(lib.facl_sa_pool(_lib.ptr(ymax), M, C, _lib.ptr(bnc3[2]), _lib.ptr(bnc3[3]), _lib.ptr(xpre), None, _lib.stream()),
                   "facl_sa_pool")
        _lib.tap("seg_arg", arg)
        _lib.tap_relu("relu_t1", y1, bnc1[2], bnc1[3])
        _lib.tap_relu("relu_t2", y2, bnc2[2], bnc2[3])
        _lib.tap_relu("relu_t3", a=xpre)
        ctx.save_for_backward(pooled, centers, W1, W2, W3, y1, y2, y3, bnc1, bnc2, bnc3, xpre, arg, ymax)
        ctx.count, ctx.reduce_fn, ctx.training, ctx.S = count, reduce_fn, training, S
        return xpre

    @staticmethod
    def backward(ctx, dxpre):
        bp = backward_precision(ctx.prec)
        lib = _lib.load_library()
        pooled, centers, W1, W2, W3, y1, y2, y3, bnc1, bnc2, bnc3, xpre, arg, ymax = ctx.saved_tensors
        ws = _Workspace.get(y1.device)
        st = _lib.stream()
        P, S = y1.shape[0], ctx.S
        M = P // S
        f64 = dict(dtype=torch.float64, device=y1.device)
        C3 = y3.shape[1]
        dxpre = dxpre.contiguous()
        sums = _lib.empty((C3, 2), **f64)
        h3 = ctx.bwd_h3 and bp == "f32"
        amax = _lib.empty((3, _lib.AMAX_WORDS), dtype=torch.int32, device=y1.device) if h3 else None
        _lib.check(lib.facl_segmax_bwd_stats_ymax(_lib.ptr(dxpre), _lib.ptr(xpre), _lib.ptr(ymax), M, C3, _lib.ptr(bnc3),
                                                  _lib.ptr(sums), _lib.ptr(ws), _lib.ptr(amax), 3 * _lib.AMAX_WORDS if h3 else 0, st),
                   "facl_segmax_bwd_stats")
        dbe3, dga3, kk, db3 = _bn_bwd_consts_mode(sums, bnc3, C3, ctx.count, ctx.reduce_fn, ctx.training)
        dy = _lib.empty_like(y3)
        am = (lambda i: amax[i]) if h3 else (lambda i: None)
        _lib.check(lib.facl_segmax_bwd_apply_amax(_lib.ptr(dxpre), _lib.ptr(xpre), _lib.ptr(y3), _lib.ptr(arg), M, S, C3,
                                                  _lib.ptr(bnc3), _lib.ptr(kk), _lib.ptr(dy), _lib.ptr(am(0)), st),
                   "facl_segmax_bwd_apply")
        bpl = ctx.bwd_planes if ctx.bwd_planes is not None else (None, None, None)
        a0b, a1b, a2b = ctx.act_amax
        dW3 = _wgrad_pro(dy, y2, bnc2, bp, am(0), a2b)
        da, sums = _rs_dgrad(dy, W3, bp, bpl[0], y2, bnc2, ws, am(0))
        grads = []
        for li, (y, bnc, yin, bnc_in, W) in enumerate(((y2, bnc2, y1, bnc1, W2), (y1, bnc1, None, None, W1)), 1):
            dy, dga, dbe, db = _bn_relu_backward(da, y, bnc, ctx.count, ctx.reduce_fn, ws, sums, am(li), training=ctx.training)
            if yin is not None:
                dW = _wgrad_pro(dy, yin, bnc_in, bp, am(li), a1b)
                da, sums = _rs_dgrad(dy, W, bp, bpl[1], yin, bnc_in, ws, am(li))
            else:
                dW = _first_layer_wgrad(dy, pooled, centers, ws, bp, am(li), a0b)
                da = _rs_dgrad(dy, W[:, 3:], bp, bpl[2], amax=am(li))[0] if ctx.needs_input_grad[0] else None
            grads.append((dW, db, dga, dbe))
        (dW2, db2, dga2, dbe2), (dW1, db1, dga1, dbe1) = grads
        return (da, None, None, None, None, None, None, dW1, db1, dga1, dbe1, dW2, db2, dga2, dbe2, dW3, db3, dga3, dbe3)


def net3dv3(pooled, centers, net, training, S, reduce_fn=None, pooled_amax=None):
    view = lambda a: a.weight.view(a.weight.shape[0], -1)
    return _Net3DV3.apply(pooled, centers, S, training, reduce_fn, (net[1], net[4], net[7]), pooled_amax,
                          view(net[0]), net[0].bias, net[1].weight, net[1].bias,
                          view(net[3]), net[3].bias, net[4].weight, net[4].bias,
                          view(net[6]), net[6].bias, net[7].weight, net[7].bias)
```

### include/facl_hip.h

```cpp
#ifndef FACL_HIP_H
#define FACL_HIP_H

#include <stdint.h>

#ifdef __cplusplus
extern "C" {
#endif

#define FACL_E_SHAPE  (-1)
#define FACL_E_NULL   (-2)
#define FACL_E_ALIGN  (-3)
#define FACL_E_CONFIG (-4)

int facl_version(void);

int facl_fps_f32(const float* xyz, int M, int N, int ld, int m, const int32_t* start,
                 int32_t* out_idx, void* stream);
int facl_fps_f64(const double* xyz, int M, int N, int ld, int m, const int32_t* start,
                 int32_t* out_idx, void* stream);

int facl_fps_reorder(const float* points, int M, int N, int D, const int32_t* picks, int m,
                     float* out, void* stream);

int facl_group(const float* points, int M, int N, int D, int S, int K, float r2,
               int32_t* idx, float* xt, float* yt, void* stream);
int facl_group_clips(const float* clips, int B, int G, int N, int D, int S, int K, float r2, int32_t* idx,
                     float* xt, float* yt, void* stream);

int64_t facl_ws_bytes(void);
int facl_bn_finalize(const double* sums, int C, double count, const float* gamma, const float* beta,
                     float eps, float momentum, float* running_mean, float* running_var, float* bnc,
                     uint32_t* aamax, uint32_t* zamax, void* stream);
int facl_bn_eval_consts(int C, const float* gamma, const float* beta, const float* running_mean,
                        const float* running_var, float eps, float* bnc, void* stream);
int facl_bn_finalize_after(const double* sums, int C, double count, const float* gamma, const float* beta,
                           float eps, float momentum, float* running_mean, float* running_var, float* bnc,
                           uint32_t* aamax, uint32_t* zamax, const float* prev, int nprev, void* stream);
int facl_bn_eval_consts_after(int C, const float* gamma, const float* beta, const float* running_mean,
                              const float* running_var, float eps, float* bnc, const float* prev, int nprev, void* stream);

#define FACL_SA_D_MIN 3
#define FACL_SA_D_MAX 8
#define FACL_SA_L1_COLS(D) ((D) <= 4 ? 8 : 12)
#define FACL_SA_BWD2_OUT(D) (64 * 64 + 64 * FACL_SA_L1_COLS(D))
int facl_sa_x_moments(const float* x, int64_t P, int D, double* mom, void* ws, void* stream);
int facl_bn1_sums_from_moments(const double* mom, double count, int D, const float* W1, const float* b1,
                               double* sums, void* stream);
int facl_sa_bn1_chain(const double* mom, double count, int D, const float* W1, const float* b1, const float* gamma,
                      const float* beta, float eps, float momentum, float* running_mean, float* running_var,
                      double* sums, float* bnc, uint32_t* aamax, float* l1tab, void* stream);
int facl_sa_l1tab(const float* W1, const float* b1, int D, const float* scale, const float* shift,
                  float* l1tab, const uint32_t* xamax, uint32_t* a1amax, void* stream);
int facl_sa_fwd2(const float* x, int64_t nunits, int D, const float* l1tab, const float* W2,
                 const float* b2, float* y2f, double* sums2, void* ws, const uint32_t* a1amax, void* stream);
int facl_sa_fwd3(const float* y2f, int64_t nunits, const float* scale2, const float* shift2,
                 const float* W3, const float* b3, const float* sgn3, float* ymax, uint8_t* arg,
                 double* sums3, void* ws, void* stream);
int facl_sa_fwd3_f16(const float* y2f, int64_t nunits, const float* scale2, const float* shift2, const float* W3,
                     const float* b3, const float* sgn3, float* ymax, uint8_t* arg, double* sums3, void* ws,
                     void* stream);
int facl_sa_fwd3_h3(const float* y2f, int64_t nunits, const float* scale2, const float* shift2, const float* W3,
                    const float* b3, const float* sgn3, float* ymax, uint8_t* arg, double* sums3, void* ws,
                    const uint32_t* a2amax, void* stream);
int facl_sa_pool(const float* ymax, int64_t rows, int C, const float* scale, const float* shift,
                 float* pooled, uint32_t* amax, void* stream);
int facl_sa_eval(const float* x, int64_t nunits, int D, const float* l1tab, const float* W2, const float* b2,
                 const float* scale2, const float* shift2, const float* W3, const float* b3, const float* scale3,
                 const float* shift3, float* pooled, const uint32_t* a1amax, void* stream);
int facl_absmax(const float* x, int64_t n, uint32_t* amax, void* stream);
int facl_rows_act_amax(const float* y, int64_t R, int C, const float* scale, const float* shift, uint32_t* amax, void* stream);

int facl_sa_bwd0(const float* dpooled, const float* ymax, int64_t rows, const float* bnc3, float* coef,
                 double* sums, void* ws, void* stream);
int facl_sa_bwd1(const float* y2f, int64_t nunits, const float* bnc2, const float* G3, const float* h3,
                 const float* W3, const float* coef, const uint8_t* arg, float* dz2f, double* sums,
                 void* ws, const uint32_t* a2amax, void* stream);
int facl_sa_bwd_w3(const float* y2f, int64_t nunits, const float* bnc2, const float* coef,
                   const uint8_t* arg, double* out, void* ws, const uint32_t* a2amax, void* stream);
int facl_sa_bwd2(const float* dz2f, const float* y2f, const float* x, int64_t nunits, int D,
                 const float* bw2, const float* W2, const float* l1tab, double* out, void* ws,
                 const uint32_t* a1amax, void* stream);
int facl_bn_bwd_consts(const double* sums_local, const double* sums_global, int C, double P, float* dbeta,
                       float* dgamma, float* kk, void* stream);
int facl_sa_bwd_consts3(const double* sums0, const float* bnc3, const float* W3, const float* b3, double P,
                        float* G3, float* h3, void* stream);
int facl_sa_bwd_consts2(const double* sums1, const float* bnc2, double P, float* bw2, void* stream);
int facl_sa_bwd_final(const double* out3, const double* sums0_g, const double* sums0_l, const float* bnc3,
                      const float* W3, const float* b3, const double* out2, const double* sums1_l,
                      const double* R1_g, const double* mom_l, const float* bnc1, const float* W1,
                      const float* b1, int D, double P, float* dW3, float* dg3, float* dbe3, float* dW2,
                      float* dg2, float* dbe2, float* dW1, float* dg1, float* dbe1, void* stream);
int facl_bn_bwd_consts_frozen(const double* sums, const float* bnc, int C, float* dbeta, float* dgamma, float* dbias,
                              float* kk, void* stream);
int facl_sa_bwd_consts3_frozen(float* G3, float* h3, void* stream);
int facl_sa_bwd_consts2_frozen(const float* bnc2, float* bw2, void* stream);
int facl_sa_bwd_final_frozen(const double* out3, const double* sums0, const float* bnc3, const double* out2,
                             const double* sums1, const float* bnc2, const float* bnc1, const float* W1, const float* b1,
                             int D, float* dW3, float* dg3, float* dbe3, float* db3, float* dW2, float* dg2, float* dbe2,
                             float* db2, float* dW1, float* dg1, float* dbe1, float* db1, void* stream);

int facl_rows_stats(const float* y, int64_t R, int C, double* sums, void* ws, void* stream);
int facl_rows_bn_relu(const float* y, int64_t R, int C, const float* scale, const float* shift, float* out,
                      void* stream);
int facl_rows_segmax(const float* y, int64_t M, int S, int C, const float* bnc, float* out, int32_t* arg,
                     void* stream);
int facl_rows_bwd_stats(const float* dout, const float* y, int64_t R, int C, const float* bnc, double* sums,
                        void* ws, void* stream);
int facl_viewmax_fwd(const float* x, int G, int B, int C, float* out, int32_t* arg, void* stream);
int facl_viewmax_bwd(const float* dout, const int32_t* arg, int G, int B, int C, float* dx, void* stream);
int facl_viewmax_bwd_add(const float* dout, const int32_t* arg, int G, int B, int C, float* dx, void* stream);
int facl_viewmax_stack(const float* x, int G, int B, int C, float* h, int32_t* arg, void* stream);

int facl_fc_bn_stats(const float* y, int64_t M, int64_t R, int C, double* sums2, void* ws, void* stream);
int facl_fc_bn_apply(const float* y, int64_t M, int64_t R, int C, const double* sums2, const double* part, int nslices_a,
                     int nslices_b, double count_a, double count_b, const float* gamma, const float* beta, float eps,
                     float momentum, float* running_mean, float* running_var, float* bnc2, float* a_out, void* stream);
int facl_fc_bn_bwd_stats(const float* dact, const float* y, int64_t M, int64_t R, int C, const float* bnc2, double* sums2,
                         void* ws, void* stream);
int facl_fc_bn_bwd_apply(const float* dact, const float* y, int64_t M, int64_t R, int C, const float* bnc2,
                         const double* sums2_g, const void* ws, double count_a, double count_b, float* dgamma, float* dbeta,
                         float* kk2, float* dy, void* stream);
int facl_col_sums(const float* x, int64_t R, int C, float* out, void* stream);
int facl_rows_center_wgrad(const float* dy, const float* centers, int64_t R, int C, double* dWc, void* ws,
                           void* stream);
int facl_rows_bwd_apply(const float* dout, const float* y, int64_t R, int C, const float* bnc,
                        const float* kk, float* dy, void* stream);
int facl_segmax_bwd_stats(const float* dxpre, const float* xpre, const float* y, const int32_t* arg,
                          int64_t M, int S, int C, const float* bnc, double* sums, void* ws, void* stream);
int facl_segmax_bwd_stats_ymax(const float* dxpre, const float* xpre, const float* ymax, int64_t M, int C,
                               const float* bnc, double* sums, void* ws, uint32_t* zamax, int zwords, void* stream);
int facl_segmax_bwd_apply(const float* dxpre, const float* xpre, const float* y, const int32_t* arg,
                          int64_t M, int S, int C, const float* bnc, const float* kk, float* dy, void* stream);
#define FACL_AMAX_WORDS 2048
int facl_rows_bwd_apply_amax(const float* dout, const float* y, int64_t R, int C, const float* bnc, const float* kk,
                             float* dy, uint32_t* amax, void* stream);
int facl_segmax_bwd_apply_amax(const float* dxpre, const float* xpre, const float* y, const int32_t* arg, int64_t M, int S,
                               int C, const float* bnc, const float* kk, float* dy, uint32_t* amax, void* stream);

int facl_gemm_fwd(const float* a, int64_t M, int K, const float* W, int ldw, int N, const float* bias,
                  const float* pscale, const float* pshift, const float* centers, const float* Wc,
                  int ldwc, float* y, double* sums, void* ws, void* stream);
int facl_gemm_fwd_segmax(const float* a, int64_t M, int K, const float* W, int ldw, int N, const float* bias,
                         const float* sgn, float* y, double* sums, float* ymax, int32_t* arg, void* ws,
                         void* stream);
int facl_gemm_dgrad(const float* dy, int64_t M, int N, const float* W, int ldw, int K, float* da,
                    void* stream);
int facl_gemm_wgrad(const float* dy, const float* a, int64_t M, int N, int K, int lda, float* dW,
                    float* slices, int nz, void* stream);
int facl_gemm_wgrad_acc(const float* dy, const float* a, int64_t M, int N, int K, int lda, float* dW, int prec, void* stream);
int facl_gemm_fwd_f16(const float* a, int64_t M, int K, const float* W, int ldw, int N, const float* bias,
                      const float* pscale, const float* pshift, const float* centers, const float* Wc, int ldwc,
                      float* y, double* sums, void* ws, void* stream);
int facl_gemm_fwd_segmax_f16(const float* a, int64_t M, int K, const float* W, int ldw, int N, const float* bias,
                             const float* sgn, float* y, double* sums, float* ymax, int32_t* arg, void* ws,
                             void* stream);
int facl_gemm_dgrad_f16(const float* dy, int64_t M, int N, const float* W, int ldw, int K, float* da,
                        void* stream);
int facl_gemm_wgrad_f16(const float* dy, const float* a, int64_t M, int N, int K, int lda, float* dW,
                        float* slices, int nz, void* stream);
int facl_gemm_wgrad_pro(const float* dy, const float* y, int64_t M, int N, int K, int ldy, const float* pscale,
                        const float* pshift, float* dW, float* slices, int nz, void* stream);
int facl_gemm_wgrad_pro_x3(const float* dy, const float* y, int64_t M, int N, int K, int ldy, const float* pscale,
                           const float* pshift, float* dW, float* slices, int nz, void* stream);
int facl_gemm_wgrad_h3(const float* dy, const float* y, int64_t M, int N, int K, int ldy, const float* pscale,
                       const float* pshift, const uint32_t* amax, const uint32_t* amax_b, float* dW, float* slices, int nz,
                       void* stream);
int facl_gemm_rs_wgrad_slices(int64_t M, int N, int K);
int facl_gemm_rs_wgrad(const float* dy, const float* y, int64_t M, int N, int K, const float* pscale, const float* pshift,
                       const uint32_t* amax, const uint32_t* amax_b, float* dW, float* slices, void* stream);
int64_t facl_gemm_rs_planes_bytes(int N, int K, int with_centers);
int facl_gemm_rs_planes(const float* W, int ldw, int N, int K, int transposed, const float* Wc, int ldwc, int half,
                        void* planes, void* stream);
int facl_gemm_rs_planes_multi(int n, const float* const* W, const int* ldw, const int* N, const int* K,
                              const int* transposed, const float* const* Wc, const int* ldwc, const int* half,
                              void* const* planes, const float* absmax_x, int64_t absmax_n, uint32_t* absmax_amax,
                              void* stream);
int facl_gemm_rs_supported(int64_t M, int K, int N);
int facl_gemm_rs_fwd(const float* a, int64_t M, int K, const void* planes, int half, const uint32_t* amax_a, int N,
                     const float* bias, const float* pscale, const float* pshift, const float* centers, float* y, double* sums,
                     const float* sgn, float* ymax, int32_t* arg, void* ws, void* stream);
int facl_gemm_rs_dgrad(const float* dy, int64_t M, int N, const void* planes, int half, const uint32_t* amax, int K,
                       float* da, void* stream);
int facl_gemm_rs_dgrad_bnstats(const float* dy, int64_t M, int N, const void* planes, int half, const uint32_t* amax, int K,
                               float* da, const float* y, const float* bnc, double* sums, void* ws, void* stream);
int facl_gemm_fwd_x3(const float* a, int64_t M, int K, const float* W, int ldw, int N, const float* bias,
                     const float* pscale, const float* pshift, const float* centers, const float* Wc, int ldwc,
                     float* y, double* sums, void* ws, void* stream);
int facl_gemm_fwd_segmax_x3(const float* a, int64_t M, int K, const float* W, int ldw, int N, const float* bias,
                            const float* sgn, float* y, double* sums, float* ymax, int32_t* arg, void* ws,
                            void* stream);
int facl_gemm_dgrad_x3(const float* dy, int64_t M, int N, const float* W, int ldw, int K, float* da,
                       void* stream);
int facl_gemm_wgrad_x3(const float* dy, const float* a, int64_t M, int N, int K, int lda, float* dW,
                       float* slices, int nz, void* stream);
int facl_sa_fwd3_x3(const float* y2f, int64_t nunits, const float* scale2, const float* shift2, const float* W3,
                    const float* b3, const float* sgn3, float* ymax, uint8_t* arg, double* sums3, void* ws,
                    void* stream);

int facl_gather_rows(const float* feat, int ldf, int M, int S1, int C, const int32_t* idx, int rows_per_cloud,
                     const float* xyz, float* out, int ldo, int col_off, void* stream);
int facl_scatter_rows(const float* drows, int ldd, int col_off, int M, int S1, int C, const int32_t* idx,
                      int rows_per_cloud, float* dfeat, void* stream);

int facl_contrast(const float* sim, int R, int J, int B, int Bk, int nA, int nS, int slot_rows,
                  const int32_t* poscol, int clip_offset, float* dsim, double* loss, void* ws, void* stream);
int facl_contrast_pair(const float* sim, int G, int B, int Bk, int J, const int64_t* order, int clip_offset,
                       float* dsim, double* losses, void* ws, void* stream);
int facl_contrast_pair_sum(const float* sim, int G, int B, int Bk, int J, const int64_t* order, int clip_offset,
                           float* dsim, double* losses, float* losses32, void* ws, void* stream);
int facl_contrast_pair_sum_mask(const float* sim, int G, int B, int Bk, int J, const int64_t* order, int clip_offset,
                                int mask_mode, float* dsim, double* losses, float* losses32, void* ws, void* stream);
int facl_loss_rows_fwd(const float* x, int64_t R, int C, int normalize, float s, float* n, float* inv_norm, void* stream);
int facl_loss_rows_bwd(const float* dn, const float* n, const float* inv_norm, int64_t R, int C, int normalize, float s,
                       float* dx, void* stream);
int facl_contrast_pair_queue(const float* sim, const float* sim_q, int G, int B, int Bk, int J, int L, const int64_t* order,
                             int clip_offset, int mask_mode, const int32_t* qstate, float* dsim, float* dsim_q, double* losses,
                             float* losses32, void* ws, void* stream);
int facl_queue_push(const float* rows, int P, int C, float* queue, int L, int32_t* qstate, void* stream);
int facl_scale_rows2(const float* src, float* dst, int64_t R1, int64_t R, int J, const float* g1, const float* g2,
                     void* stream);

int facl_normalize_map(const float* x, int64_t M, int C, const float* Wm, int K, float* x_nor, float* code,
                       void* stream);

int64_t facl_mailbox_bytes(int R, int n_max);
int facl_mailbox_alloc(int64_t bytes, void** ptr, void* handle64);
int facl_mailbox_open(const void* handle64, void** ptr);
int facl_mailbox_close(void* ptr);
int facl_mailbox_free(void* ptr);
int facl_mailbox_allreduce(const double* in, double* out, int n, int n_max, void* const* boxes, int rank, int R, uint64_t* seq,
                           uint32_t* err, void* stream);

int facl_adam_prep(const float* lr, float* step, float b1, float b2, float* consts, void* stream);
int facl_adam_apply(int nt, float* const* p, const float* const* g, float* const* m, float* const* v, const int* n,
                    const float* consts, float b1, float b2, float eps, void* stream);
int facl_ema_apply(int nt, float* const* pk, const float* const* p, const int* n, float m, void* stream);

#define FACL_LR_STEP   0
#define FACL_LR_COSINE 1
int facl_grad_sqnorm(int nt, const float* const* g, const int* n, double* partial, void* stream);
int facl_adam_prep_ex(const float* lr, float* step, float b1, float b2, const double* partial, int npartial, double max_norm,
                      int schedule, int warmup_steps, int decay_steps, double lr_min, float* consts, void* stream);
int facl_adamw_apply(int nt, float* const* p, const float* const* g, float* const* m, float* const* v, const int* n,
                     const int* decay, const float* consts, float b1, float b2, float eps, float wd, void* stream);

int facl_sinkhorn(const float* Q, int R, int C, int iters, float* scratch, float* out, void* stream);
int facl_kmeans(const float* x, int N, int D, int K, int iters, int32_t* labels, float* cent, int32_t* counts,
                void* stream);

int facl_build_views_f32(const float* src, int64_t rows, int C, const int32_t* idx, const double* noise,
                         const double* cossin, int B, float* out, void* stream);
int facl_build_views_f64(const double* src, int64_t rows, int C, const int32_t* idx, const double* noise,
                         const double* cossin, int B, float* out, void* stream);

int facl_views_temporal_rows_f32(const float* src, int64_t rows, int C, const int32_t* meta, int B, int32_t* list,
                                 int32_t* counts, int32_t* err, void* stream);
int facl_views_temporal_rows_f64(const double* src, int64_t rows, int C, const int32_t* meta, int B, int32_t* list,
                                 int32_t* counts, int32_t* err, void* stream);
int facl_build_views_philox_f32(const float* src, int64_t rows, int C, const int32_t* meta, const int32_t* list,
                                const int32_t* counts, int64_t seed, int epoch, int B, float* out, int32_t* idx_out,
                                void* stream);
int facl_build_views_philox_f64(const double* src, int64_t rows, int C, const int32_t* meta, const int32_t* list,
                                const int32_t* counts, int64_t seed, int epoch, int B, float* out, int32_t* idx_out,
                                void* stream);
int facl_build_views_philox_gp_f32(const float* src, int64_t rows, int C, const int32_t* meta, const int32_t* list,
                                   const int32_t* counts, int64_t seed, int epoch, int B, int G, int P, float* out,
                                   int32_t* idx_out, void* stream);
int facl_build_views_philox_gp_f64(const double* src, int64_t rows, int C, const int32_t* meta, const int32_t* list,
                                   const int32_t* counts, int64_t seed, int epoch, int B, int G, int P, float* out,
                                   int32_t* idx_out, void* stream);

#define FACL_RESIDENT_REC 12
int facl_resident_temporal_rows_f32(const float* src, int64_t* table, int32_t* lists, int first, int count, int32_t* err,
                                    void* stream);
int facl_resident_temporal_rows_f64(const double* src, int64_t* table, int32_t* lists, int first, int count, int32_t* err,
                                    void* stream);
int facl_build_views_resident_f32(const float* src, const int64_t* table, const int32_t* lists, int n_clips,
                                  const int32_t* sel, int B, int64_t seed, int epoch, float* out, int64_t* idx_out,
                                  int32_t* err, void* stream);
int facl_build_views_resident_f64(const double* src, const int64_t* table, const int32_t* lists, int n_clips,
                                  const int32_t* sel, int B, int64_t seed, int epoch, float* out, int64_t* idx_out,
                                  int32_t* err, void* stream);
int facl_build_views_resident_gp_f32(const float* src, const int64_t* table, const int32_t* lists, int n_clips,
                                     const int32_t* sel, int B, int G, int P, int64_t seed, int epoch, float* out,
                                     int64_t* idx_out, int32_t* err, void* stream);
int facl_build_views_resident_gp_f64(const double* src, const int64_t* table, const int32_t* lists, int n_clips,
                                     const int32_t* sel, int B, int G, int P, int64_t seed, int epoch, float* out,
                                     int64_t* idx_out, int32_t* err, void* stream);

#define FACL_VIEW_RAW        0
#define FACL_VIEW_MIRROR     1
#define FACL_VIEW_KEY        2
#define FACL_VIEW_KEY_MIRROR 3
#define FACL_VIEW_ROT        4
#define FACL_VIEW_T4         5
#define FACL_VIEW_T7         6
#define FACL_VIEW_RES30      7
#define FACL_VIEW_RES10      8
#define FACL_VIEW_JITTER     9
#define FACL_VIEW_SCALE      10
#define FACL_VIEW_TILT_NEG   11
#define FACL_VIEW_TILT_POS   12
#define FACL_VIEW_NKINDS     13
#define FACL_VIEW_POS_MAX    12
#define FACL_VIEW_NSTRENGTH  6
#define FACL_VIEW_TABLE_COLS 8
int facl_build_views_philox_recipe_f32(const float* src, int64_t rows, int C, const int32_t* meta, const int32_t* list,
                                       const int32_t* counts, int64_t seed, int epoch, int B, int G, int P, float* out,
                                       int32_t* idx_out, const int32_t* kinds, int n_kinds, const double* strengths,
                                       void* stream);
int facl_build_views_philox_recipe_f64(const double* src, int64_t rows, int C, const int32_t* meta, const int32_t* list,
                                       const int32_t* counts, int64_t seed, int epoch, int B, int G, int P, float* out,
                                       int32_t* idx_out, const int32_t* kinds, int n_kinds, const double* strengths,
                                       void* stream);
int facl_build_views_resident_recipe_f32(const float* src, const int64_t* table, const int32_t* lists, int n_clips,
                                         const int32_t* sel, int B, int G, int P, int64_t seed, int epoch, float* out,
                                         int64_t* idx_out, int32_t* err, const int32_t* kinds, int n_kinds,
                                         const double* strengths, void* stream);
int facl_build_views_resident_recipe_f64(const double* src, const int64_t* table, const int32_t* lists, int n_clips,
                                         const int32_t* sel, int B, int G, int P, int64_t seed, int epoch, float* out,
                                         int64_t* idx_out, int32_t* err, const int32_t* kinds, int n_kinds,
                                         const double* strengths, void* stream);
int facl_view_recipe_table(const int32_t* kinds, int n_kinds, int32_t* table, int32_t* stride);

#define FACL_GEN3DV_MAX_FRAMES        64
#define FACL_GEN3DV_MAX_FRAMES_TOTAL  (1 << 16)
#define FACL_GEN3DV_MAX_PIXELS        (1 << 22)
#define FACL_GEN3DV_MAX_CLIPS         4096
#define FACL_GEN3DV_MAX_VOXELS        (1 << 24)
#define FACL_GEN3DV_MAX_VOXELS_TOTAL  (1 << 27)
int facl_gen3dv_frames(const uint16_t* frames, int NF, int H, int W, int32_t* fbox, int32_t* fcount, double* fext,
                       void* stream);
int facl_gen3dv_voxelise(const uint16_t* frames, int NF, int H, int W, const int32_t* fbox, const int32_t* fmeta,
                         const double* cmin, const int32_t* cgrid, int B, int maxF, int maxvox, int64_t NV, int64_t NP,
                         double voxel, uint64_t* occ, uint64_t* mocc, int32_t* pix, int32_t* err, void* stream);
int facl_gen3dv_volumes(const uint64_t* occ, const uint64_t* mocc, const int32_t* wtab, const int32_t* cgrid, int B,
                        int maxvox, int64_t NV, int32_t* vol, int32_t* key, void* stream);
// ... 38 lines not shown
```

Measured before the change: 10970.

## Fuse segmax BN backward apply into the layer-3 dgrad and wgrad GEMM prologues

Removes the separate segmax backward apply kernel that wrote a full dy tensor for the last SA layer. The dgrad and wgrad GEMMs now rebuild dy on the fly from y3 as an affine per-channel term plus a sparse routed term, using per-cloud routing words (sd, arg) held in LDS or registers. The fp16x3 amax bound for the split is computed analytically in a new consts kernel, with forward-time absmax tracking added for it. This saves a full M×C write and reread of dy. In exchange it adds extra ALU work and LDS pressure in the GEMM inner loops and relies on a conservative amax bound.

```diff
diff --git a/facl_amd/_lib.py b/facl_amd/_lib.py
--- a/facl_amd/_lib.py
+++ b/facl_amd/_lib.py
@@ -50,6 +50,7 @@
     "facl_rows_bwd_apply_amax": [c_p, c_p, c_l, c_i, c_p, c_p, c_p, c_p, c_p],
     "facl_segmax_bwd_stats": [c_p, c_p, c_p, c_p, c_l, c_i, c_i, c_p, c_p, c_p, c_p],
     "facl_segmax_bwd_stats_ymax": [c_p, c_p, c_p, c_l, c_i, c_p, c_p, c_p, c_p, c_i, c_p],
+    "facl_segmax_bwd_stats_ymax_dmax": [c_p, c_p, c_p, c_l, c_i, c_p, c_p, c_p, c_p, c_i, c_p, c_p],
     "facl_segmax_bwd_apply": [c_p, c_p, c_p, c_p, c_l, c_i, c_i, c_p, c_p, c_p, c_p],
     "facl_segmax_bwd_apply_amax": [c_p, c_p, c_p, c_p, c_l, c_i, c_i, c_p, c_p, c_p, c_p, c_p],
     "facl_gemm_fwd": [c_p, c_l, c_i, c_p, c_i, c_i, c_p, c_p, c_p, c_p, c_p, c_i, c_p, c_p, c_p, c_p],
@@ -72,6 +73,8 @@
     "facl_gemm_rs_fwd": [c_p, c_l, c_i, c_p, c_i, c_p, c_i, c_p, c_p, c_p, c_p, c_p, c_p, c_p, c_p, c_p, c_p, c_p],
     "facl_gemm_rs_dgrad": [c_p, c_l, c_i, c_p, c_i, c_p, c_i, c_p, c_p],
     "facl_gemm_rs_dgrad_bnstats": [c_p, c_l, c_i, c_p, c_i, c_p, c_i, c_p, c_p, c_p, c_p, c_p, c_p],
+    "facl_gemm_rs_dgrad_dz3_bnstats": [c_p, c_l, c_i, c_p, c_p, c_p, c_p, c_p, c_i, c_p, c_p, c_p, c_p, c_p, c_p],
+    "facl_gemm_rs_wgrad_dz3": [c_p, c_p, c_l, c_i, c_i, c_p, c_p, c_p, c_p, c_p, c_p, c_p, c_p, c_p, c_p],
     "facl_gemm_fwd_x3": [c_p, c_l, c_i, c_p, c_i, c_i, c_p, c_p, c_p, c_p, c_p, c_i, c_p, c_p, c_p, c_p],
     "facl_gemm_fwd_segmax_x3": [c_p, c_l, c_i, c_p, c_i, c_i, c_p, c_p, c_p, c_p, c_p, c_p, c_p, c_p],
     "facl_gemm_dgrad_x3": [c_p, c_l, c_i, c_p, c_i, c_i, c_p, c_p],
@@ -107,6 +110,7 @@
     "facl_sa_bwd_consts3": [c_p, c_p, c_p, c_p, c_d, c_p, c_p, c_p],
     "facl_sa_bwd_consts2": [c_p, c_p, c_d, c_p, c_p],
     "facl_bn_bwd_consts": [c_p, c_p, c_i, c_d, c_p, c_p, c_p, c_p],
+    "facl_bn_bwd_consts_dz3": [c_p, c_p, c_i, c_d, c_p, c_p, c_p, c_p, c_p, c_p, c_l, c_p, c_p, c_p, c_p, c_p],
     "facl_rows_center_wgrad": [c_p, c_p, c_l, c_i, c_p, c_p, c_p],
     "facl_viewmax_fwd": [c_p, c_i, c_i, c_i, c_p, c_p, c_p],
     "facl_viewmax_bwd": [c_p, c_p, c_i, c_i, c_i, c_p, c_p],
diff --git a/facl_amd/csrc/finalize.hip b/facl_amd/csrc/finalize.hip
--- a/facl_amd/csrc/finalize.hip
+++ b/facl_amd/csrc/finalize.hip
@@ -556,6 +556,56 @@
     return facl_launch_status();
 }
 
+static __global__ __launch_bounds__(256) void k_bn_bwd_consts_dz3(const double* __restrict__ sums_l, const double* __restrict__ sums_g, int C,
+                                                           double P, float* __restrict__ dbeta, float* __restrict__ dgamma,
+                                                           float* __restrict__ kk, const float* __restrict__ bnc,
+                                                           const float* __restrict__ dxpre, const float* __restrict__ xpre, int M,
+                                                           const unsigned* __restrict__ dmax, float* __restrict__ dzc,
+                                                           float* __restrict__ sd, unsigned* __restrict__ amax) {
+    const int c = blockIdx.x * 256 + threadIdx.x;
+    const bool live = c < C;
+    const float scale = live ? bnc[2 * C + c] : 0.f;
+    if (live)
+        for (int m = blockIdx.y; m < M; m += gridDim.y) {
+            const size_t o = (size_t)m * C + c;
+            sd[o] = scale * (xpre[o] > 0.f ? dxpre[o] : 0.f);
+        }
+    if (blockIdx.y) return;
+    unsigned bb = 0u;
+    if (live) {
+        dbeta[c] = (float)sums_l[2 * c];
+        dgamma[c] = (float)sums_l[2 * c + 1];
+        const float inv = (float)(1.0 / P);
+        kk[c] = (float)sums_g[2 * c] * inv;
+        kk[C + c] = (float)sums_g[2 * c + 1] * inv;
+        const double k1 = sums_g[2 * c] / P, k2 = sums_g[2 * c + 1] / P, s = scale, is = bnc[C + c];
+        const double cb = -s * is * k2;
+        dzc[c] = (float)(-s * k1 - cb * (double)bnc[c]);
+        dzc[C + c] = (float)cb;
+        unsigned db = 0u;
+        for (int i = 0; i < FACL_AMAX_SLOTS; ++i) { const unsigned t = dmax[i * FACL_AMAX_STRIDE]; db = db > t ? db : t; }
+        const double D = (double)__uint_as_float(db);
+        const double bd = fabs(s) * (D + fabs(k1) + fabs(k2) * sqrt(P > 1 ? P - 1 : 1)) * 1.001;
+        bb = __float_as_uint(fabsf((float)bd));
+    }
+#pragma unroll
+    for (int o = 32; o > 0; o >>= 1) { const unsigned t = (unsigned)__shfl_xor((int)bb, o, 64); bb = bb > t ? bb : t; }
+    atomicMax(amax + (threadIdx.x & (FACL_AMAX_SLOTS - 1)) * FACL_AMAX_STRIDE, bb);
+}
+
+extern "C" int facl_bn_bwd_consts_dz3(const double* sums_local, const double* sums_global, int C, double P, float* dbeta,
+                                      float* dgamma, float* kk, const float* bnc, const float* dxpre, const float* xpre, int64_t M,
+                                      const uint32_t* dmax, float* dzc, float* sd, uint32_t* amax, void* stream) {
+    if (!sums_local || !sums_global || !dbeta || !dgamma || !kk || !bnc || !dxpre || !xpre || !dmax || !dzc || !sd || !amax)
+        return FACL_E_NULL;
+    if (C < 1 || P < 1 || M < 1 || M > 0x7fffffff) return FACL_E_SHAPE;
+    const int gx = (C + 255) / 256;
+    const int gy = (int)(M < 64 ? M : 64);
+    hipLaunchKernelGGL(k_bn_bwd_consts_dz3, dim3(gx, gy), dim3(256), 0, (hipStream_t)stream, sums_local, sums_global, C, P, dbeta,
+                       dgamma, kk, bnc, dxpre, xpre, (int)M, dmax, dzc, sd, amax);
+    return facl_launch_status();
+}
+
 extern "C" int facl_sa_bwd_consts2(const double* sums1, const float* bnc2, double P, float* bw2, void* stream) {
     if (!sums1 || !bnc2 || !bw2) return FACL_E_NULL;
     if (P < 1) return FACL_E_SHAPE;
diff --git a/facl_amd/csrc/gemm_rs.hip b/facl_amd/csrc/gemm_rs.hip
--- a/facl_amd/csrc/gemm_rs.hip
+++ b/facl_amd/csrc/gemm_rs.hip
@@ -22,6 +22,10 @@
 #endif
 constexpr int RS_KPRO = 512;
 constexpr int RS_LDS = RS_LDS_W + RS_LDS_A + 2 * RS_KPRO * 4;
+constexpr int RS_KDZ = 1024;
+constexpr int RS_LDS_DZ = RS_LDS_W + RS_LDS_A + 2 * RS_KDZ * 4;
+constexpr int RS_DZ_HOLE = RS_CT * 2 * 1024;
+static_assert(RS_WSLOT - RS_DZ_HOLE >= 2 * RS_KDZ * 4, "a cloud's routing words fit the tail of a ring slot");
 
 struct RsArgs {
     const float* A = nullptr; int lda = 0; int M = 0; int K = 0;
@@ -34,6 +38,7 @@
     double* part = nullptr;
     const float* sgn = nullptr; float* smax = nullptr; int* sarg = nullptr;
     const float* by = nullptr; const float* bbnc = nullptr;
+    const float* dzc = nullptr; const float* dsd = nullptr; const int* darg = nullptr;
     int h3 = 0;
     const unsigned* amax = nullptr;
     const int* wse = nullptr;
@@ -160,8 +165,9 @@
     return (unsigned)(uintptr_t)(const __attribute__((address_space(3))) char*)p;
 }
 
-template <bool PRO, bool SEG, bool BST, bool H3 = false, int WV = RS_WAVES>
+template <bool PRO, bool SEG, bool BST, bool H3 = false, int WV = RS_WAVES, bool DZ = false>
 __global__ __launch_bounds__(64 * WV, WV == 8 ? 1 : 2) void k_gemm_rs(RsArgs g) {
+    static_assert(!DZ || (H3 && WV == RS_WAVES && !PRO && !SEG), "dz3 form: fp16x3 dgrad on 4-wave workgroups (two clouds each)");
     constexpr int NPL = H3 ? 2 : 3;
     constexpr int WPP = RS_CT * NPL / WV;
     extern __shared__ __attribute__((aligned(16))) char lds[];
@@ -217,8 +223,21 @@
             r[2 * t + 1] = *reinterpret_cast<const float4*>(base + (((c + 1) ^ akey) << 4));
         }
     };
+    const char* const dzhole = wring + (wave >> 1) * RS_WSLOT + RS_DZ_HOLE;
+    const int dzrow = 32 * (wave & 1) + q;
     auto planes_half = [&](int j, const float4& r, unsigned (&pk)[12], int half) {
         float v[4] = {r.x, r.y, r.z, r.w};
+        if (DZ) {
+            const int kb = 16 * j + 8 * h + 4 * half;
+            const float4 a4 = *reinterpret_cast<const float4*>(tab + kb);
+            const float4 b4 = *reinterpret_cast<const float4*>(tab + RS_KDZ + kb);
+            const float4 s4 = *reinterpret_cast<const float4*>(dzhole + 4 * kb);
+            const int4 g4 = *reinterpret_cast<const int4*>(dzhole + 4 * (RS_KDZ + kb));
+            v[0] = fmaf(v[0], b4.x, a4.x) + (g4.x == dzrow ? s4.x : 0.f);
+            v[1] = fmaf(v[1], b4.y, a4.y) + (g4.y == dzrow ? s4.y : 0.f);
+            v[2] = fmaf(v[2], b4.z, a4.z) + (g4.z == dzrow ? s4.z : 0.f);
+            v[3] = fmaf(v[3], b4.w, a4.w) + (g4.w == dzrow ? s4.w : 0.f);
+        }
         if (PRO) {
             const float4 s4 = *reinterpret_cast<const float4*>(tab + 16 * j + 8 * h + 4 * half);
             const float4 t4 = *reinterpret_cast<const float4*>(tab + RS_KPRO + 16 * j + 8 * h + 4 * half);
@@ -299,6 +318,20 @@
     issueA(0); issueW(0);
     if (PRO) {
         for (int i = tid; i < g.K; i += 64 * WV) { tab[i] = g.pscale[i]; tab[RS_KPRO + i] = g.pshift[i]; }
+    }
+    if (DZ) {
+        const int ncl = g.M >> 6;
+        for (int i = tid; i < g.K; i += 64 * WV) {
+            tab[i] = g.dzc[i]; tab[RS_KDZ + i] = g.dzc[g.K + i];
+#pragma unroll
+            for (int c = 0; c < 2; ++c) {
+                int cl = tile.y * 2 + c;
+                cl = cl < ncl ? cl : ncl - 1;
+                char* const hole = wring + c * RS_WSLOT + RS_DZ_HOLE;
+                reinterpret_cast<float*>(hole)[i] = g.dsd[(size_t)cl * g.K + i];
+                reinterpret_cast<int*>(hole)[RS_KDZ + i] = g.darg[(size_t)cl * g.K + i];
+            }
+        }
     }
     unsigned P0[12], P1[12];
     float4 raw[4];
@@ -496,11 +529,13 @@
     float* slices; int rows_per_slice;
     const unsigned* amax;
     const unsigned* amax_b;
+    const float* dzc = nullptr; const float* dsd = nullptr; const int* darg = nullptr;
 };
 
 constexpr int WG_TP = 68;
-template <bool PRO, bool H3, bool WIDE = false>
+template <bool PRO, bool H3, bool WIDE = false, bool DZ = false>
 __global__ __launch_bounds__(64 * WG_WAVES) void k_wgrad_rs(WgArgs g) {
+    static_assert(!DZ || H3, "dz3 form: fp16x3 only");
     constexpr int NPL = H3 ? 2 : 3;
     constexpr int BRING_U4 = 2 * (2 * 4 * NPL * 64);
     constexpr int WSTG_F = WIDE ? 32 * WG_TP : 32 * 32;
@@ -568,6 +603,28 @@
             }
     };
 
+    float dza[2] = {0.f, 0.f}, dzb[2] = {0.f, 0.f};
+    if (DZ && !WIDE) {
+#pragma unroll
+        for (int nt = 0; nt < 2; ++nt) { dza[nt] = g.dzc[n0 + q + 32 * nt]; dzb[nt] = g.dzc[g.N + n0 + q + 32 * nt]; }
+    }
+    auto dz_frags = [&](int s, float (&r)[2][2][8]) {
+        const int pb = p0 + 32 * s;
+        const size_t co = (size_t)(pb >> 6) * g.N + n0 + q;
+#pragma unroll
+        for (int nt = 0; nt < 2; ++nt) {
+            const float sdv = g.dsd[co + 32 * nt];
+            const int av = g.darg[co + 32 * nt];
+#pragma unroll
+            for (int ks = 0; ks < 2; ++ks)
+#pragma unroll
+                for (int e = 0; e < 8; ++e) {
+                    const int rr = 16 * ks + 8 * h + e;
+                    r[ks][nt][e] = fmaf(r[ks][nt][e], dzb[nt], dza[nt]) + (av == (pb & 63) + rr ? sdv : 0.f);
+                }
+        }
+    };
+
     float* const dimg = stg_base + wave * WSTG_F;
     const float* dsrc4 = g.dy + n0 + 4 * (lane & 15);
     auto load_raw = [&](int s, float4 (&r)[8]) {
@@ -576,7 +633,7 @@
             const int p = p0 + 32 * s + 4 * i + (lane >> 4);
             const bool in = p < p1;
             const float4 v = *reinterpret_cast<const float4*>(dsrc4 + (size_t)(in ? p : p1 - 1) * g.N);
-            r[i] = in ? v : make_float4(0.f, 0.f, 0.f, 0.f);
+            r[i] = (DZ || in) ? v : make_float4(0.f, 0.f, 0.f, 0.f);
         }
     };
     auto raw_to_frags = [&](const float4 (&r)[8], float (&f)[2][2][8]) {
@@ -591,6 +648,17 @@
 #pragma unroll
                 for (int nt = 0; nt < 2; ++nt) f[ks][nt][e] = dimg[(16 * ks + 8 * h + e) * WG_TP + 32 * nt + q];
     };
+    float* const dzl = stg_base + WG_WAVES * WSTG_F + wave * 384;
+    struct DzRoute { float sd; int arg; };
+    auto load_route = [&](int s) -> DzRoute {
+        const unsigned co = (unsigned)((p0 + 32 * s) >> 6) * (unsigned)g.N + (unsigned)(n0 + lane);
+        return {g.dsd[co], g.darg[co]};
+    };
+    auto park_route = [&](int s, const DzRoute& rt) {
+        dzl[128 + 128 * (s & 1) + lane] = rt.sd;
+        reinterpret_cast<int*>(dzl)[128 + 128 * (s & 1) + 64 + lane] = rt.arg;
+    };
+    if (DZ && WIDE) { dzl[lane] = g.dzc[n0 + lane]; dzl[64 + lane] = g.dzc[g.N + n0 + lane]; }
 
     f32x16 acc[2][4];
 #pragma unroll
@@ -604,16 +672,23 @@
 
     float rb[8], ra[2][2][8];
     float4 raw[8];
+    DzRoute route = {};
     load_b(0, rb);
-    if (WIDE) { load_raw(0, raw); raw_to_frags(raw, ra); }
-    else load_a(0, ra);
+    if (WIDE) {
+        load_raw(0, raw);
+        if (DZ) park_route(0, load_route(0));
+        raw_to_frags(raw, ra);
+    } else {
+        load_a(0, ra);
+        if (DZ) dz_frags(0, ra);
+    }
     store_b(0, rb);
     if (nst > 1) load_b(1, rb);
     __syncthreads();
     for (int s = 0; s < nst; ++s) {
         float ran[2][2][8];
         if (s + 1 < nst) {
-            if (WIDE) load_raw(s + 1, raw);
+            if (WIDE) { load_raw(s + 1, raw); if (DZ) route = load_route(s + 1); }
             else load_a(s + 1, ran);
         }
         const uint4* bs = &bring[s & 1][lane];
@@ -621,6 +696,13 @@
 #pragma unroll
             for (int nt = 0; nt < 2; ++nt) {
                 unsigned hi[4], mi[4], lo[4];
+                if (DZ && WIDE) {
+                    const int c = 32 * nt + q, rb0 = ((p0 + 32 * s) & 63) + 16 * ks + 8 * h;
+                    const float a = dzl[c], b = dzl[64 + c], sdv = dzl[128 + 128 * (s & 1) + c];
+                    const int av = reinterpret_cast<const int*>(dzl)[128 + 128 * (s & 1) + 64 + c] - rb0;
+#pragma unroll
+                    for (int e = 0; e < 8; ++e) ra[ks][nt][e] = fmaf(ra[ks][nt][e], b, a) + (av == e ? sdv : 0.f);
+                }
                 if (H3) {
 #pragma unroll
                     for (int e = 0; e < 4; ++e) split_pair_h(ra[ks][nt][2 * e] * sD, ra[ks][nt][2 * e + 1] * sD, hi[e], mi[e]);
@@ -659,7 +741,10 @@
             split_a(0, af0);
             mfma_ks(0, af0);
             split_a(1, af1);
-            if (WIDE && s + 1 < nst) raw_to_frags(raw, ra);
+            if (WIDE && s + 1 < nst) {
+                if (DZ) park_route(s + 1, route);
+                raw_to_frags(raw, ra);
+            }
             mfma_ks(1, af1);
         }
         if (s + 1 < nst) {
@@ -672,6 +757,7 @@
                     for (int nt = 0; nt < 2; ++nt)
 #pragma unroll
                         for (int e = 0; e < 8; ++e) ra[ks][nt][e] = ran[ks][nt][e];
+                if (DZ) dz_frags(s + 1, ra);
             }
         }
         __syncthreads();
@@ -700,10 +786,10 @@
         }
 }
 
-template <bool PRO, bool H3, bool WIDE>
+template <bool PRO, bool H3, bool WIDE, bool DZ = false>
 int wg_launch_k(const WgArgs& g, dim3 grid, hipStream_t st) {
-    constexpr int lds = 2 * (2 * 4 * (H3 ? 2 : 3) * 64) * 16 + WG_WAVES * 32 * (WIDE ? WG_TP : 32) * 4;
-    return facl_launch_dynamic_lds<k_wgrad_rs<PRO, H3, WIDE>>(grid, dim3(64 * WG_WAVES), lds, st, g);
+    constexpr int lds = 2 * (2 * 4 * (H3 ? 2 : 3) * 64) * 16 + WG_WAVES * 32 * (WIDE ? WG_TP : 32) * 4 + (DZ && WIDE ? WG_WAVES * 384 * 4 : 0);
+    return facl_launch_dynamic_lds<k_wgrad_rs<PRO, H3, WIDE, DZ>>(grid, dim3(64 * WG_WAVES), lds, st, g);
 }
 
 constexpr int RS_LDS8 = RS_LDS_W + 8 * RS_ASLOT + 2 * RS_KPRO * 4 + 8 * 6144;
@@ -713,10 +799,11 @@
     return (h3 && w8) ? 8 : RS_WAVES;
 }
 
-template <bool PRO, bool SEG, bool BST, bool H3, int WV>
+template <bool PRO, bool SEG, bool BST, bool H3, int WV, bool DZ = false>
 int rs_launch_k(const RsArgs& g, hipStream_t st) {
     const dim3 grid(g.N / 256, (g.M + 32 * WV - 1) / (32 * WV));
-    return facl_launch_dynamic_lds<k_gemm_rs<PRO, SEG, BST, H3, WV>>(grid, dim3(64 * WV), WV == 8 ? RS_LDS8 : RS_LDS, st, g);
+    return facl_launch_dynamic_lds<k_gemm_rs<PRO, SEG, BST, H3, WV, DZ>>(grid, dim3(64 * WV), DZ ? RS_LDS_DZ : WV == 8 ? RS_LDS8 : RS_LDS,
+                                                                     st, g);
 }
 template <bool H3, int WV>
 int rs_launch_form(const RsArgs& g, hipStream_t st) {
@@ -735,6 +822,7 @@
         g.first_round = 512;
         g.phase_ticks = (per_ks > 0 && wgs > g.first_round && rs_waves(g.h3) == RS_WAVES) ? per_ks * (g.K >> 4) + 500 : 0;
     }
+    if (g.dzc) return rs_launch_k<false, false, true, true, RS_WAVES, true>(g, st);
     if (rs_waves(g.h3) == 8) return rs_launch_form<true, 8>(g, st);
     return g.h3 ? rs_launch_form<true, RS_WAVES>(g, st) : rs_launch_form<false, RS_WAVES>(g, st);
 }
@@ -852,6 +940,26 @@
     return facl_reduce_rows((const double*)ws, prow, 2 * K, sums, st);
 }
 
+extern "C" int facl_gemm_rs_dgrad_dz3_bnstats(const float* y3, int64_t M, int N, const void* planes, const uint32_t* amax,
+                                              const float* dzc, const float* sd, const int32_t* arg, int K, float* da,
+                                              const float* y, const float* bnc, double* sums, void* ws, void* stream) {
+    if (!y3 || !planes || !da || !y || !bnc || !sums || !ws || !amax || !dzc || !sd || !arg) return FACL_E_NULL;
+    if (!facl_gemm_rs_supported(M, N, K) || (M & 63) || N > RS_KDZ) return FACL_E_SHAPE;
+    if (((uintptr_t)y3 | (uintptr_t)planes) & 15) return FACL_E_ALIGN;
+    const int prow = (int)((M + 32 * RS_WAVES - 1) / (32 * RS_WAVES));
+    if ((size_t)prow * K * 2 * sizeof(double) > ((size_t)facl_ws_bytes() - FACL_WS_TICKET_BYTES)) return FACL_E_SHAPE;
+    hipStream_t st = (hipStream_t)stream;
+    const int* wse = (const int*)((const char*)planes + rs_planes_only_bytes(K, N, 0));
+    RsArgs g{y3, N, (int)M, N, (const uint4*)planes, K / 32, K};
+    g.C = da; g.ldc = K;
+    g.part = (double*)ws; g.by = y; g.bbnc = bnc;
+    g.h3 = 1; g.amax = amax; g.wse = wse;
+    g.dzc = dzc; g.dsd = sd; g.darg = arg;
+    int rc = rs_launch(g, st);
+    if (rc) return rc;
+    return facl_reduce_rows((const double*)ws, prow, 2 * K, sums, st);
+}
+
 extern "C" int facl_gemm_rs_wgrad_slices(int64_t M, int N, int K) {
     if (M < 4096 || N < 512 || (N & 511) || K < 128 || (K & 127)) return 0;
     const int tiles = (N / 512) * (K / 128);
@@ -862,9 +970,9 @@
     rps = (rps + 31) / 32 * 32;
     return (int)((M + rps - 1) / rps);
 }
-extern "C" int facl_gemm_rs_wgrad(const float* dy, const float* y, int64_t M, int N, int K, const float* pscale,
-                                  const float* pshift, const uint32_t* amax, const uint32_t* amax_b, float* dW, float* slices,
-                                  void* stream) {
+static int rs_wgrad(const float* dy, const float* y, int64_t M, int N, int K, const float* pscale, const float* pshift,
+                    const uint32_t* amax, const uint32_t* amax_b, const float* dzc, const float* sd, const int32_t* arg,
+                    float* dW, float* slices, void* stream) {
     if (!dy || !y || !dW || !slices || (amax && !amax_b)) return FACL_E_NULL;
     if ((pscale == nullptr) != (pshift == nullptr)) return FACL_E_NULL;
     if (M > 0x7fffffff) return FACL_E_SHAPE;
@@ -878,11 +986,14 @@
     rps = (rps + 31) / 32 * 32;
     hipStream_t st = (hipStream_t)stream;
     WgArgs g{dy, y, (int)M, N, K, pscale, pshift, slices, rps, amax, amax_b};
+    g.dzc = dzc; g.dsd = sd; g.darg = arg;
     const dim3 grid(K / 128, N / 512, nz);
     static const int wide_env = facl_env_int("FACL_WGRAD_WIDE", 1);
-    const int wide = wide_env && !(((uintptr_t)dy) & 15);
+    const int wide = wide_env && !(((uintptr_t)dy | (uintptr_t)dzc | (uintptr_t)sd | (uintptr_t)arg) & 15);
     int rc;
-    if (pscale && amax && wide) rc = wg_launch_k<true, true, true>(g, grid, st);
+    if (dzc && pscale) rc = wide ? wg_launch_k<true, true, true, true>(g, grid, st) : wg_launch_k<true, true, false, true>(g, grid, st);
+    else if (dzc) rc = wide ? wg_launch_k<false, true, true, true>(g, grid, st) : wg_launch_k<false, true, false, true>(g, grid, st);
+    else if (pscale && amax && wide) rc = wg_launch_k<true, true, true>(g, grid, st);
     else if (amax && wide) rc = wg_launch_k<false, true, true>(g, grid, st);
     else if (pscale && amax) rc = wg_launch_k<true, true, false>(g, grid, st);
     else if (pscale) rc = wg_launch_k<true, false, false>(g, grid, st);
@@ -891,3 +1002,15 @@
     if (rc) return rc;
     return facl_sum_slices(slices, nz, (long long)N * K / 4, dW, false, st);
 }
+extern "C" int facl_gemm_rs_wgrad(const float* dy, const float* y, int64_t M, int N, int K, const float* pscale,
+                                  const float* pshift, const uint32_t* amax, const uint32_t* amax_b, float* dW, float* slices,
+                                  void* stream) {
+    return rs_wgrad(dy, y, M, N, K, pscale, pshift, amax, amax_b, nullptr, nullptr, nullptr, dW, slices, stream);
+}
+extern "C" int facl_gemm_rs_wgrad_dz3(const float* y3, const float* y, int64_t M, int N, int K, const float* pscale,
+                                      const float* pshift, const uint32_t* amax, const uint32_t* amax_b, const float* dzc,
+                                      const float* sd, const int32_t* arg, float* dW, float* slices, void* stream) {
+    if (!amax || !dzc || !sd || !arg) return FACL_E_NULL;
+    if ((M & 63) || N < 1 || (M >> 6) * (int64_t)N > 0x7fffffff) return FACL_E_SHAPE;
+    return rs_wgrad(y3, y, M, N, K, pscale, pshift, amax, amax_b, dzc, sd, arg, dW, slices, stream);
+}
diff --git a/facl_amd/csrc/rows.hip b/facl_amd/csrc/rows.hip
--- a/facl_amd/csrc/rows.hip
+++ b/facl_amd/csrc/rows.hip
@@ -141,21 +141,29 @@
 __global__ __launch_bounds__(256) void k_segmax_bwd_stats_ymax(const float* __restrict__ dxpre, const float* __restrict__ xpre,
                                                                const float* __restrict__ ymax, int Mrows, int C,
                                                                const float* __restrict__ bnc, double* __restrict__ part,
-                                                               unsigned* __restrict__ zamax, int zwords) {
+                                                               unsigned* __restrict__ zamax, int zwords,
+                                                               unsigned* __restrict__ dmax) {
     if (zamax && blockIdx.x == 0 && blockIdx.y == 0)
         for (int i = threadIdx.x; i < zwords; i += 256) zamax[i] = 0u;
     const int c = blockIdx.x * 256 + threadIdx.x;
     if (c >= C) return;
     const float mean = bnc[c], inv = bnc[C + c], sg = bnc[4 * C + c];
     double s = 0, g = 0;
+    unsigned mx = 0u;
     for (int m = blockIdx.y; m < Mrows; m += gridDim.y) {
         const size_t o = (size_t)m * C + c;
         const float d = xpre[o] > 0.f ? dxpre[o] : 0.f;
         s += (double)d;
         g += (double)d * (double)bn_yhat(sg * ymax[o], mean, inv);
+        const unsigned b = __float_as_uint(d) & 0x7fffffffu;
+        mx = mx > b ? mx : b;
     }
     part[(size_t)blockIdx.y * 2 * C + 2 * c] = s;
     part[(size_t)blockIdx.y * 2 * C + 2 * c + 1] = g;
+    if (dmax) {
+        unsigned* const slot = abs_max_slot(dmax);
+        publish_abs_max(slot, *slot, __uint_as_float(mx));
+    }
 }
 
 template <int W>
@@ -447,7 +455,16 @@
     if (!dxpre || !xpre || !ymax || !bnc || !sums || !ws) return FACL_E_NULL;
     if (M < 1 || M > 0x7fffffff || C < 1 || 2 * C > 4608 || zwords < 0) return FACL_E_SHAPE;
     return launch_partials(k_segmax_bwd_stats_ymax, rows_grid(M, C), 2 * C, sums, ws, (hipStream_t)stream, dxpre, xpre, ymax, (int)M,
-                           C, bnc, (double*)ws, zamax, zwords);
+                           C, bnc, (double*)ws, zamax, zwords, (unsigned*)nullptr);
+}
+
+extern "C" int facl_segmax_bwd_stats_ymax_dmax(const float* dxpre, const float* xpre, const float* ymax, int64_t M, int C,
+                                               const float* bnc, double* sums, void* ws, uint32_t* zamax, int zwords,
+                                               uint32_t* dmax, void* stream) {
+    if (!dxpre || !xpre || !ymax || !bnc || !sums || !ws || !dmax) return FACL_E_NULL;
+    if (M < 1 || M > 0x7fffffff || C < 1 || 2 * C > 4608 || zwords < 0) return FACL_E_SHAPE;
+    return launch_partials(k_segmax_bwd_stats_ymax, rows_grid(M, C), 2 * C, sums, ws, (hipStream_t)stream, dxpre, xpre, ymax, (int)M,
+                           C, bnc, (double*)ws, zamax, zwords, dmax);
 }
 
 extern "C" int facl_segmax_bwd_apply(const float* dxpre, const float* xpre, const float* y, const int32_t* arg,
diff --git a/facl_amd/tail.py b/facl_amd/tail.py
--- a/facl_amd/tail.py
+++ b/facl_amd/tail.py
@@ -162,7 +162,7 @@
     return torch.cat((dWc.float(), dWh), dim=1)
 
 
-def _forward_bn_consts(y, bn, training, reduce_fn, ws, sums=None, aamax=None):
+def _forward_bn_consts(y, bn, training, reduce_fn, ws, sums=None, aamax=None, zamax=None):
     R, C = y.shape
     if not training:
         bnc = _bn_eval(C, bn.weight.detach(), bn.bias.detach(), bn.running_mean, bn.running_var)
@@ -175,7 +175,8 @@
     if reduce_fn is not None:
         reduce_fn(sums)
         count = count * reduce_fn.world_size
-    bnc = _bn_finalize(sums, C, count, bn.weight.detach(), bn.bias.detach(), bn.running_mean, bn.running_var, aamax=aamax)
+    bnc = _bn_finalize(sums, C, count, bn.weight.detach(), bn.bias.detach(), bn.running_mean, bn.running_var, aamax=aamax,
+                       zamax=zamax)
     bn.count_batch()
     return bnc, count
 
@@ -588,7 +589,7 @@
 _FUSE_BNSTATS = _env_on("FACL_RS_BNSTATS")
 
 
-def _rs_dgrad(dy, W, prec, planes=None, bn_y=None, bn_c=None, ws=None, amax=None):
+def _rs_dgrad(dy, W, prec, planes=None, bn_y=None, bn_c=None, ws=None, amax=None, dz3=None):
     if prec != "f32":
         return gemm_dgrad(dy, W, prec=prec), None
     lib = _lib.load_library()
@@ -600,7 +601,13 @@
     da = _lib.empty((M, K), dtype=torch.float32, device=dy.device)
     sums = None
     with _lib.timed("facl_gemm_rs_dgrad %dx%dx%d%s" % (M, N, K, " h3" if half else "")):
-        if bn_y is not None and _FUSE_BNSTATS:
+        if dz3 is not None:
+            sums = _lib.empty((K, 2), dtype=torch.float64, device=dy.device)
+            _lib.check(lib.facl_gemm_rs_dgrad_dz3_bnstats(_lib.ptr(dy), M, N, _lib.ptr(planes), _lib.ptr(amax), _lib.ptr(dz3[0]),
+                                                          _lib.ptr(dz3[1]), _lib.ptr(dz3[2]), K, _lib.ptr(da), _lib.ptr(bn_y),
+                                                          _lib.ptr(bn_c), _lib.ptr(sums), _lib.ptr(ws), _lib.stream()),
+                       "facl_gemm_rs_dgrad_dz3_bnstats")
+        elif bn_y is not None and _FUSE_BNSTATS:
             sums = _lib.empty((K, 2), dtype=torch.float64, device=dy.device)
             _lib.check(lib.facl_gemm_rs_dgrad_bnstats(_lib.ptr(dy), M, N, _lib.ptr(planes), half, _lib.ptr(amax), K, _lib.ptr(da),
                                                       _lib.ptr(bn_y), _lib.ptr(bn_c), _lib.ptr(sums), _lib.ptr(ws), _lib.stream()),
@@ -612,14 +619,28 @@
 
 
 _WGRAD_RS = _env_on("FACL_WGRAD_RS")
-
-
-def _wgrad_pro(dy, y, bnc, prec, amax=None, amax_b=None):
+_TAIL_DZ3 = _env_on("FACL_TAIL_DZ3", "0")
+
+
+def _wgrad_rs_slices(M, N, K, y, prec):
+    lib = _lib.load_library()
+    return lib.facl_gemm_rs_wgrad_slices(M, N, K) if (prec == "f32" and _WGRAD_RS and y.is_contiguous()) else 0
+
+
+def _wgrad_pro(dy, y, bnc, prec, amax=None, amax_b=None, dz3=None):
     lib = _lib.load_library()
     M, N = dy.shape
     K = y.shape[1]
     dW = _lib.empty((N, K), dtype=torch.float32, device=dy.device)
-    nzr = lib.facl_gemm_rs_wgrad_slices(M, N, K) if (prec == "f32" and _WGRAD_RS and y.is_contiguous()) else 0
+    nzr = _wgrad_rs_slices(M, N, K, y, prec)
+    if dz3 is not None:
+        slices = _lib.empty(nzr * N * K, dtype=torch.float32, device=dy.device)
+        with _lib.timed("facl_gemm_rs_wgrad %dx%dx%d h3 dz3" % (M, N, K)):
+            _lib.check(lib.facl_gemm_rs_wgrad_dz3(_lib.ptr(dy), _lib.ptr(y), M, N, K, _lib.ptr(bnc[2]), _lib.ptr(bnc[3]),
+                                                  _lib.ptr(amax), _lib.ptr(amax_b), _lib.ptr(dz3[0]), _lib.ptr(dz3[1]),
+                                                  _lib.ptr(dz3[2]), _lib.ptr(dW), _lib.ptr(slices), _lib.stream()),
+                       "facl_gemm_rs_wgrad_dz3")
+        return dW
     if nzr > 0:
         slices = _lib.empty(nzr * N * K, dtype=torch.float32, device=dy.device)
         with _lib.timed("facl_gemm_rs_wgrad %dx%dx%d%s" % (M, N, K, "" if amax is None else " h3")):
@@ -684,7 +705,10 @@
         bnc2, _ = _forward_bn_consts(y2, bns[1], training, reduce_fn, ws, sums2, aamax=amax[2])
         y3, sums3, ymax, arg = _rs_fwd(y2, pl[2], W3.shape[0], b3, bnc2, None, training, g3.detach(), ws, h3, amax[2])
         ctx.act_amax = (a0, amax[1], amax[2])
-        bnc3, _ = _forward_bn_consts(y3, bns[2], training, reduce_fn, ws, sums3)
+        ctx.dmax = None
+        if _TAIL_DZ3 and training and ctx.bwd_h3 and W3.shape[0] <= 1024:
+            ctx.dmax = _lib.empty(_lib.AMAX_WORDS, dtype=torch.int32, device=pooled.device)
+        bnc3, _ = _forward_bn_consts(y3, bns[2], training, reduce_fn, ws, sums3, zamax=ctx.dmax)
         M, C = P // S, W3.shape[0]
         xpre = _lib.empty((M, C), dtype=torch.float32, device=pooled.device)
         _lib.check(lib.facl_sa_pool(_lib.ptr(ymax), M, C, _lib.ptr(bnc3[2]), _lib.ptr(bnc3[3]), _lib.ptr(xpre), None, _lib.stream()),
@@ -712,19 +736,37 @@
         sums = _lib.empty((C3, 2), **f64)
         h3 = ctx.bwd_h3 and bp == "f32"
         amax = _lib.empty((3, _lib.AMAX_WORDS), dtype=torch.int32, device=y1.device) if h3 else None
-        _lib.check(lib.facl_segmax_bwd_stats_ymax(_lib.ptr(dxpre), _lib.ptr(xpre), _lib.ptr(ymax), M, C3, _lib.ptr(bnc3),
-                                                  _lib.ptr(sums), _lib.ptr(ws), _lib.ptr(amax), 3 * _lib.AMAX_WORDS if h3 else 0, st),
-                   "facl_segmax_bwd_stats")
-        dbe3, dga3, kk, db3 = _bn_bwd_consts_mode(sums, bnc3, C3, ctx.count, ctx.reduce_fn, ctx.training)
-        dy = _lib.empty_like(y3)
         am = (lambda i: amax[i]) if h3 else (lambda i: None)
-        _lib.check(lib.facl_segmax_bwd_apply_amax(_lib.ptr(dxpre), _lib.ptr(xpre), _lib.ptr(y3), _lib.ptr(arg), M, S, C3,
-                                                  _lib.ptr(bnc3), _lib.ptr(kk), _lib.ptr(dy), _lib.ptr(am(0)), st),
-                   "facl_segmax_bwd_apply")
         bpl = ctx.bwd_planes if ctx.bwd_planes is not None else (None, None, None)
         a0b, a1b, a2b = ctx.act_amax
-        dW3 = _wgrad_pro(dy, y2, bnc2, bp, am(0), a2b)
-        da, sums = _rs_dgrad(dy, W3, bp, bpl[0], y2, bnc2, ws, am(0))
+        dz3 = None
+        if (ctx.dmax is not None and h3 and ctx.training and S == 64 and _FUSE_BNSTATS
+                and _wgrad_rs_slices(P, C3, y2.shape[1], y2, bp) > 0):
+            _lib.check(lib.facl_segmax_bwd_stats_ymax_dmax(_lib.ptr(dxpre), _lib.ptr(xpre), _lib.ptr(ymax), M, C3, _lib.ptr(bnc3),
+                                                           _lib.ptr(sums), _lib.ptr(ws), _lib.ptr(amax), 3 * _lib.AMAX_WORDS,
+                                                           _lib.ptr(ctx.dmax), st), "facl_segmax_bwd_stats")
+            f32 = dict(dtype=torch.float32, device=y1.device)
+            dbe3, dga3, kk = _lib.empty(C3, **f32), _lib.empty(C3, **f32), _lib.empty((2, C3), **f32)
+            dzc, sd = _lib.empty((2, C3), **f32), _lib.empty((M, C3), **f32)
+            sums_g = ctx.reduce_fn(sums.clone()) if ctx.reduce_fn is not None else sums
+            _lib.check(lib.facl_bn_bwd_consts_dz3(_lib.ptr(sums), _lib.ptr(sums_g), C3, float(ctx.count), _lib.ptr(dbe3),
+                                                  _lib.ptr(dga3), _lib.ptr(kk), _lib.ptr(bnc3), _lib.ptr(dxpre), _lib.ptr(xpre), M,
+                                                  _lib.ptr(ctx.dmax), _lib.ptr(dzc), _lib.ptr(sd), _lib.ptr(am(0)), st),
+                       "facl_bn_bwd_consts_dz3")
+            db3 = None
+            dz3 = (dzc, sd, arg)
+            dy = y3
+        else:
+            _lib.check(lib.facl_segmax_bwd_stats_ymax(_lib.ptr(dxpre), _lib.ptr(xpre), _lib.ptr(ymax), M, C3, _lib.ptr(bnc3),
+                                                      _lib.ptr(sums), _lib.ptr(ws), _lib.ptr(amax), 3 * _lib.AMAX_WORDS if h3 else 0, st),
+                       "facl_segmax_bwd_stats")
+            dbe3, dga3, kk, db3 = _bn_bwd_consts_mode(sums, bnc3, C3, ctx.count, ctx.reduce_fn, ctx.training)
+            dy = _lib.empty_like(y3)
+            _lib.check(lib.facl_segmax_bwd_apply_amax(_lib.ptr(dxpre), _lib.ptr(xpre), _lib.ptr(y3), _lib.ptr(arg), M, S, C3,
+                                                      _lib.ptr(bnc3), _lib.ptr(kk), _lib.ptr(dy), _lib.ptr(am(0)), st),
+                       "facl_segmax_bwd_apply")
+        dW3 = _wgrad_pro(dy, y2, bnc2, bp, am(0), a2b, dz3=dz3)
+        da, sums = _rs_dgrad(dy, W3, bp, bpl[0], y2, bnc2, ws, am(0), dz3=dz3)
         grads = []
         for li, (y, bnc, yin, bnc_in, W) in enumerate(((y2, bnc2, y1, bnc1, W2), (y1, bnc1, None, None, W1)), 1):
             dy, dga, dbe, db = _bn_relu_backward(da, y, bnc, ctx.count, ctx.reduce_fn, ws, sums, am(li), training=ctx.training)
diff --git a/include/facl_hip.h b/include/facl_hip.h
--- a/include/facl_hip.h
+++ b/include/facl_hip.h
@@ -82,6 +82,9 @@
                  const uint32_t* a1amax, void* stream);
 int facl_bn_bwd_consts(const double* sums_local, const double* sums_global, int C, double P, float* dbeta,
                        float* dgamma, float* kk, void* stream);
+int facl_bn_bwd_consts_dz3(const double* sums_local, const double* sums_global, int C, double P, float* dbeta, float* dgamma,
+                           float* kk, const float* bnc, const float* dxpre, const float* xpre, int64_t M, const uint32_t* dmax,
+                           float* dzc, float* sd, uint32_t* amax, void* stream);
 int facl_sa_bwd_consts3(const double* sums0, const float* bnc3, const float* W3, const float* b3, double P,
                         float* G3, float* h3, void* stream);
 int facl_sa_bwd_consts2(const double* sums1, const float* bnc2, double P, float* bw2, void* stream);
@@ -129,6 +132,9 @@
                           int64_t M, int S, int C, const float* bnc, double* sums, void* ws, void* stream);
 int facl_segmax_bwd_stats_ymax(const float* dxpre, const float* xpre, const float* ymax, int64_t M, int C,
                                const float* bnc, double* sums, void* ws, uint32_t* zamax, int zwords, void* stream);
+int facl_segmax_bwd_stats_ymax_dmax(const float* dxpre, const float* xpre, const float* ymax, int64_t M, int C,
+                                    const float* bnc, double* sums, void* ws, uint32_t* zamax, int zwords, uint32_t* dmax,
+                                    void* stream);
 int facl_segmax_bwd_apply(const float* dxpre, const float* xpre, const float* y, const int32_t* arg,
                           int64_t M, int S, int C, const float* bnc, const float* kk, float* dy, void* stream);
 #define FACL_AMAX_WORDS 2048
@@ -168,6 +174,9 @@
 int facl_gemm_rs_wgrad_slices(int64_t M, int N, int K);
 int facl_gemm_rs_wgrad(const float* dy, const float* y, int64_t M, int N, int K, const float* pscale, const float* pshift,
                        const uint32_t* amax, const uint32_t* amax_b, float* dW, float* slices, void* stream);
+int facl_gemm_rs_wgrad_dz3(const float* y3, const float* y, int64_t M, int N, int K, const float* pscale, const float* pshift,
+                           const uint32_t* amax, const uint32_t* amax_b, const float* dzc, const float* sd, const int32_t* arg,
+                           float* dW, float* slices, void* stream);
 int64_t facl_gemm_rs_planes_bytes(int N, int K, int with_centers);
 int facl_gemm_rs_planes(const float* W, int ldw, int N, int K, int transposed, const float* Wc, int ldwc, int half,
                         void* planes, void* stream);
@@ -183,6 +192,9 @@
                        float* da, void* stream);
 int facl_gemm_rs_dgrad_bnstats(const float* dy, int64_t M, int N, const void* planes, int half, const uint32_t* amax, int K,
                                float* da, const float* y, const float* bnc, double* sums, void* ws, void* stream);
+int facl_gemm_rs_dgrad_dz3_bnstats(const float* y3, int64_t M, int N, const void* planes, const uint32_t* amax, const float* dzc,
+                                   const float* sd, const int32_t* arg, int K, float* da, const float* y, const float* bnc,
+                                   double* sums, void* ws, void* stream);
 int facl_gemm_fwd_x3(const float* a, int64_t M, int K, const float* W, int ldw, int N, const float* bias,
                      const float* pscale, const float* pshift, const float* centers, const float* Wc, int ldwc,
                      float* y, double* sums, void* ws, void* stream);
```

Measured after the change: 10840. 0.988x the previous value.
